# JakobHavtorn/benchmarking-lvms

Hardware: AMD Instinct MI355X
Metric: audio frames/sec training (VRNN, 16 kHz mu-law) (higher is better)
Workload: dtype f32

## Files before the change

benchmarking-lvms_amd/blvm/models/vrnn.py:

```python
import math
from types import SimpleNamespace
from typing import Optional, Union

import torch
import torch.nn as nn
import torch.nn.init as init

from blvm import _hip, ops
from blvm.data.transforms import StackTensor
from blvm.evaluation import BitsPerDimMetric, DeferredScalars, KLMetric, LatestMeanMetric, LLMetric, LossMetric
from blvm.models.base_model import BaseModel
from blvm.modules.convenience import View
from blvm.modules.distributions import (DiagonalGaussianDense, DiagonalGaussianMixtureDense,
                                        DiscretizedLogisticMixtureDense, mlp_log_prob)

LIKELIHOOD_HEADS = (DiscretizedLogisticMixtureDense, DiagonalGaussianMixtureDense, DiagonalGaussianDense)


class LazyNamespace(SimpleNamespace):

    def __init__(self, _lazy=None, **kwargs):
        super().__init__(**kwargs)
        object.__setattr__(self, "_lazy", dict(_lazy or {}))

# ... 121 lines not shown
            and self.condition_x_on_h
            and all(isinstance(m, (nn.Linear, nn.LeakyReLU, View, StackTensor)) for m in list(enc) + list(dec))
            and isinstance(dec[-2], nn.LeakyReLU)
        )
        if not ok:
            raise NotImplementedError(
                "libblvm_hip accelerates the VRNNAudio(likelihood='DMoL') structure (stacked-frame MLP encoder, MLP "
                "decoder, DMoL head, condition_h_on_x = condition_x_on_h = True); other compositions are not built yet"
            )
        return stack.n_frames, _linears(enc), _linears(dec), lik

    def forward(self, x: torch.Tensor, x_sl: torch.Tensor, beta: float = 1, free_nats: float = 0,
                h0: Optional[torch.Tensor] = None, eps: Optional[torch.Tensor] = None):
        S, enc_lin, dec_lin, lik = self._plan()
        if x.ndim == 3:
            x = x.squeeze(-1)
        dev = x.device
        B, T = x.shape
        x_sl_host = x_sl.detach().cpu().to(torch.int64)
        x_sl_dev = ops.upload_i32(x_sl_host, dev)
        y = x.detach().to(torch.float32).contiguous()
        Tp = (T + S - 1) // S
        stride = math.ceil(T / Tp)
        H, Z, R = self.h_dim, self.z_dim, self.r_dim

        xs = torch.nn.functional.pad(y, (0, Tp * S - T)) if Tp * S != T else y
        xs = xs.view(B, Tp, S).transpose(0, 1).contiguous().view(Tp * B, S)
        enc = ops.mlp(xs, enc_lin, ops.ACT_LEAKY, ops.LEAKY_SLOPE).view(Tp, B, -1)

        if eps is None:
            eps = torch.randn(Tp, B, Z, device=dev, dtype=torch.float32)
        widths = [(lin.in_features, lin.out_features) for lin in dec_lin]
        chained = len(dec_lin) == 3 and widths[0] == (H + R, widths[1][0]) and widths[1][1] == widths[1][0] == widths[2][0]
        fold = ops.DecoderFold(dec_lin, ops.LEAKY_SLOPE) if chained and all(lin.bias is not None for lin in dec_lin) else None
        decin, kld, kld_fn, mu_q, sd_q, mu_p, sd_p, z = self.vrnn_cell.sequence(enc, h0, eps, x_sl_dev, stride, free_nats, decoder=fold)
        given = fold.given if fold is not None else None

        dec, log_prob = mlp_log_prob(lik, decin[:Tp].view(Tp * B, H + R), dec_lin, ops.ACT_LEAKY, ops.LEAKY_SLOPE, y, x_sl_dev,
                                     ops.LAYOUT_TIME_MAJOR, B, T, Tp, S, given=given)

        n_frames = float(x_sl_host.sum())
        loss, elbo, sums4 = ops.elbo_assemble(log_prob, kld, kld_fn, beta, n_frames)
        kl = kld_fn

        sums = DeferredScalars(sums4)
        ln2 = math.log(2)
        metrics = [
            LossMetric(sums[0], weight_by=B),
            LLMetric(sums[1], name="elbo", reduce_by=B),
            LLMetric(sums[2], name="rec", reduce_by=B),
            KLMetric(sums[3], reduce_by=B),
            KLMetric(sums[3] / ln2, name="kl (bpt)", reduce_by=n_frames),
            BitsPerDimMetric(sums[1], reduce_by=n_frames),
            LatestMeanMetric(beta, name="beta"),
            LatestMeanMetric(free_nats, name="free_nats"),
        ]

        max_len = int(x_sl_host.max())
        F = lik.out_features

        def parameters():
            d = dec.detach().view(Tp, B, S, F).permute(1, 0, 2, 3).reshape(B, Tp * S, F)[:, :max_len]
            return lik(d.contiguous())

        lazy = dict(
            reconstructions_parameters=parameters,
            reconstructions=lambda ns: lik.sample(ns.reconstructions_parameters),
            reconstructions_mode=lambda ns: lik.mode(ns.reconstructions_parameters),
            seq_mask=lambda: (torch.arange(max_len, device=dev).unsqueeze(0) < x_sl_dev.unsqueeze(1)).to(torch.float64),
        )
        outputs = LazyNamespace(
            lazy,
# ... 141 lines not shown
```

benchmarking-lvms_amd/blvm/modules/distributions.py:

```python
import math

import torch
import torch.nn as nn

from .. import ops
from .convenience import AddConstant


class ConditionalDistribution(nn.Module):
    def reset_parameters(self):
        pass


class DiagonalGaussianDense(ConditionalDistribution):
    def __init__(self, x_dim, y_dim, initial_sd: float = 1, epsilon: float = 1e-6):
        super().__init__()
        self.x_dim, self.y_dim, self.initial_sd, self.epsilon = x_dim, y_dim, initial_sd, epsilon
        self.out_features = 2 * y_dim
        self.params = nn.Linear(x_dim, 2 * y_dim)
        beta = math.log(2) / (initial_sd - epsilon)
        self.sd_activation = nn.Sequential(nn.Softplus(beta=beta), AddConstant(epsilon)) if epsilon > 0 else nn.Softplus(beta=beta)
        self.reset_parameters()

    @property
# ... 11 lines not shown
        lead = x.shape[:-1]
        p = ops.mlp(x.reshape(-1, x.shape[-1]), [self.params], act=ops.ACT_NONE)
        mu, raw = p.view(*lead, -1).chunk(2, dim=-1)
        return mu, self.sd_activation(raw)

    def fused_log_prob(self, dec, y, x_sl_dev, layout, B, T, Tp, S, fused_linear: bool = True):
        if self.y_dim != 1:
            raise NotImplementedError("Gaussian likelihood head: y_dim must be 1 on the audio path")
        W, b = (self.params.weight, self.params.bias) if fused_linear else (None, None)
        return ops.gauss_log_prob(dec, W, b, y, x_sl_dev, layout, B, T, Tp, S, self.softplus_beta, self.epsilon)


class DiscretizedLogisticMixtureDense(ConditionalDistribution):
    def __init__(self, x_dim: int, y_dim: int, num_mix: int = 10, num_bins: int = 256, log_epsilon: float = -7.0):
        super().__init__()
        self.x_dim, self.y_dim, self.num_mix, self.num_bins, self.log_epsilon = x_dim, y_dim, num_mix, num_bins, log_epsilon
        self.out_features = num_mix * (2 * y_dim + 1)
        self.params = nn.Linear(x_dim, self.out_features)
        self.reset_parameters()

    def forward(self, x):
        if self.y_dim != 1:
            raise NotImplementedError("DMoL head: y_dim must be 1 on the audio path")
        lead = x.shape[:-1]
        p = ops.mlp(x.reshape(-1, x.shape[-1]), [self.params], act=ops.ACT_NONE).view(*lead, -1)
        logits = p[..., : self.num_mix]
        locs, log_scales = p[..., self.num_mix :].reshape(*lead, 1, 2 * self.num_mix).chunk(2, dim=-1)
        return logits, locs, log_scales.clamp(min=self.log_epsilon)

    def fused_log_prob(self, dec, y, x_sl_dev, layout, B, T, Tp, S, fused_linear: bool = True):
        W, b = (self.params.weight, self.params.bias) if fused_linear else (None, None)
        return ops.dmol_log_prob(dec, W, b, y, x_sl_dev, layout, B, T, Tp, S, self.num_mix, self.num_bins, self.log_epsilon)

    def fused_mlp_log_prob(self, x2d, layers, act, slope, y, x_sl_dev, layout, B, T, Tp, S, given=None):
        return ops.mlp_dmol_log_prob(x2d, layers, self.params.weight, self.params.bias, y, x_sl_dev, layout, B, T, Tp, S, act, slope,
                                     self.num_mix, self.num_bins, self.log_epsilon, given)

    @staticmethod
    def _pack(params):
        return torch.cat([params[0], params[1].squeeze(-2), params[2].squeeze(-2)], -1).contiguous()

    @torch.no_grad()
    def mode(self, params):
        return ops.mix_sample(self._pack(params), None, None, 0, self.log_epsilon).unsqueeze(-1)

    @torch.no_grad()
    def sample(self, params, eps: float = 1e-5, uniforms=None):
        logits = params[0]
        u = torch.empty_like(logits).uniform_(eps, 1.0 - eps) if uniforms is None else uniforms[0].to(logits)
        u2 = torch.empty(*logits.shape[:-1], device=logits.device).uniform_(1e-8, 1.0 - 1e-8) if uniforms is None else uniforms[1].to(logits)
        return ops.mix_sample(self._pack(params), u, u2, 0, self.log_epsilon).unsqueeze(-1)


class DiagonalGaussianMixtureDense(ConditionalDistribution):

    def __init__(self, x_dim, y_dim, num_mix: int, initial_sd: float = 1, epsilon: float = 1e-6):
        super().__init__()
        self.x_dim, self.y_dim, self.num_mix, self.initial_sd, self.epsilon = x_dim, y_dim, num_mix, initial_sd, epsilon
        self.out_features = num_mix * (2 * y_dim + 1)
        self.params = nn.Linear(x_dim, self.out_features)
        beta = self.softplus_beta
        self.sd_activation = nn.Sequential(nn.Softplus(beta=beta), AddConstant(epsilon)) if epsilon > 0 else nn.Softplus(beta=beta)
        self.reset_parameters()

    @property
    def softplus_beta(self) -> float:
        return math.log(2) / self.initial_sd if self.epsilon > 0 else math.log(2) / (self.initial_sd - self.epsilon)

    def forward(self, x):
# ... 27 lines not shown
    def __init__(self, x_dim, y_dim):
        super().__init__()
        ops.categorical_check_widths(x_dim, y_dim)
        self.x_dim, self.y_dim = x_dim, y_dim
        self.out_features = y_dim
        self.logits = nn.Linear(x_dim, y_dim)
        self.register_buffer("levels", torch.linspace(-1.0, 1.0, y_dim), persistent=False)
        self.reset_parameters()

    def forward(self, x):
        lead = x.shape[:-1]
        return ops.mlp(x.reshape(-1, x.shape[-1]), [self.logits], act=ops.ACT_NONE).view(*lead, -1)

    def fused_log_prob(self, dec, y, x_sl_dev, B, T, Tp, S):
        return ops.categorical_log_prob(dec, self.logits.weight, self.logits.bias, y, x_sl_dev, B, T, Tp, S)

    def log_prob(self, y, logits, reduce_dim=None):
        ll = (logits - logits.logsumexp(dim=-1, keepdim=True)).gather(-1, y.long().unsqueeze(-1)).squeeze(-1)
        return ll if reduce_dim is None else ll.sum(reduce_dim)

    @torch.no_grad()
    def mode(self, logits):
        return ops.categorical_sample(logits)

    @torch.no_grad()
    def sample(self, logits, uniforms=None):
        u = torch.rand(logits.shape[:-1], device=logits.device) if uniforms is None else uniforms
        return ops.categorical_sample(logits, u)

    def dequantize(self, k):
        return self.levels.to(k.device)[k.long()]


def mlp_log_prob(lik, x2d, layers, act, slope, y, x_sl_dev, layout, B, T, Tp, S, given=None):
    if isinstance(lik, DiscretizedLogisticMixtureDense):
        return lik.fused_mlp_log_prob(x2d, layers, act, slope, y, x_sl_dev, layout, B, T, Tp, S, given)
    dec = ops.mlp(x2d, layers, act, slope) if given is None else ops.mlp_given(x2d, layers, given, act, slope)
    return dec.detach(), lik.fused_log_prob(dec, y, x_sl_dev, layout, B, T, Tp, S)
```

benchmarking-lvms_amd/blvm/ops.py:

```python
import ctypes
from typing import List, Optional, Sequence

import torch

from . import _hip
from ._hip import VrnnWeights, check, load, ptr, stream_ptr

ACT_NONE, ACT_RELU, ACT_LEAKY = 0, 1, 2
LEAKY_SLOPE = 0.01

LAYOUT_BATCH_MAJOR, LAYOUT_TIME_MAJOR = 0, 1

seq_timer_hook = None


def _tick(tag):
    if seq_timer_hook is not None:
        seq_timer_hook(tag)


def _c_ints(v):
    return (ctypes.c_int * len(v))(*[int(i) for i in v])


# ... 265 lines not shown
            dW = torch.empty_like(W) if need_w else None
            db = torch.empty_like(b) if need_b else None
            ws = _dmol_workspace(dec.device, ws_floats) if (need_w or need_b) else None
            rc = lib.blvm_dmol_bwd_fused(ptr(dec), layout, ptr(W), ptr(b), ptr(y), ptr(x_sl_dev), ptr(g32), B, T, Tp, S, num_mix,
                                         num_bins, log_eps, act_slope, ptr(dz), ptr(dW), ptr(db), ptr(ws), stream_ptr())
            if rc == 0:
                return (dz if ctx.needs_input_grad[0] else None, dW, db) + (None,) * 11
            if rc != BLVM_NOT_APPLICABLE:
                check(rc, "blvm_dmol_bwd_fused")
        d_dec = torch.empty_like(dec)
        d_par = torch.empty_like(dec) if ctx.has_linear else None
        check(
            load().blvm_dmol_bwd(ptr(dec), layout, ptr(W), ptr(b), ptr(y), ptr(x_sl_dev), ptr(g32), B, T, Tp, S, num_mix,
                                 num_bins, log_eps, ptr(d_dec), ptr(d_par), stream_ptr()),
            "blvm_dmol_bwd",
        )
        n_frames = dec.numel() // F
        dW, db = _head_linear_grads(d_par, dec, W, b, F, n_frames, need_w, need_b)
        if act_slope >= 0.0 and ctx.needs_input_grad[0]:
            dz = torch.empty_like(d_dec)
            check(lib.blvm_act_bwd_f32(ptr(d_dec), ptr(dec), act_slope, ptr(dz), dz.numel(), stream_ptr()), "blvm_act_bwd_f32")
            d_dec = dz
        return (d_dec if ctx.needs_input_grad[0] else None, dW, db) + (None,) * 11


def mlp_given(x2d, layers, given, act: int = ACT_LEAKY, slope: float = LEAKY_SLOPE, head_gates: bool = False):
    params = []
    for lin in layers:
        params += [lin.weight, lin.bias]
    return _MLPGivenFunction.apply(x2d, act, slope, head_gates, tuple(given), *params)


def mlp_dmol_log_prob(x2d, layers, W, b, y, x_sl_dev, layout, B, T, Tp, S, act: int = ACT_LEAKY, slope: float = LEAKY_SLOPE,
                      num_mix=10, num_bins=256, log_eps=-7.0, given=None):
    if act == ACT_NONE or W is None:
        dec = mlp(x2d, layers, act, slope) if given is None else mlp_given(x2d, layers, given, act, slope)
        return dec.detach(), dmol_log_prob(dec, W, b, y, x_sl_dev, layout, B, T, Tp, S, num_mix, num_bins, log_eps)
    params = []
    for lin in layers:
        params += [lin.weight, lin.bias]
    dec = _MLPFunction.apply(x2d, act, slope, True, *params) if given is None else mlp_given(x2d, layers, given, act, slope, True)
    gate = slope if act == ACT_LEAKY else 0.0
    return dec.detach(), _DMoLFunction.apply(dec, W, b, y, x_sl_dev, layout, B, T, Tp, S, num_mix, num_bins, log_eps, gate)


def dmol_log_prob(dec, W, b, y, x_sl_dev, layout, B, T, Tp, S, num_mix=10, num_bins=256, log_eps=-7.0):
    return _DMoLFunction.apply(dec, W, b, y, x_sl_dev, layout, B, T, Tp, S, num_mix, num_bins, log_eps, -1.0)


class _GaussHeadFunction(torch.autograd.Function):

    @staticmethod
    def forward(ctx, dec, W, b, y, x_sl_dev, kind, layout, B, T, Tp, S, num_mix, sd_beta, sd_eps):
        dec, y = _f32c(dec), _f32c(y)
        W, b = (_f32c(W), _f32c(b)) if W is not None else (None, None)
        F = 3 * num_mix if kind == 1 else 2
        if dec.dim() != 2 or dec.shape[0] != B * Tp or dec.shape[1] != S * F:
            raise _hip.BlvmHipError(f"Gaussian head: activations must be [B*T'={B * Tp}, S*F={S * F}], got {tuple(dec.shape)}")
        if W is not None and tuple(W.shape) != (F, F):
            raise _hip.BlvmHipError(f"Gaussian head: fused head weight must be [{F},{F}], got {tuple(W.shape)}")
        if tuple(y.shape) != (B, T) or Tp * S < T:
            raise _hip.BlvmHipError(f"Gaussian head: targets must be [B={B}, T={T}] with T <= T'*S={Tp * S}, got {tuple(y.shape)}")
        log_prob = torch.zeros(B, device=dec.device, dtype=torch.float64)
        lib = load()
        if kind == 1:
            rc = lib.blvm_gmm_fwd(ptr(dec), layout, ptr(W), ptr(b), ptr(y), ptr(x_sl_dev), B, T, Tp, S, num_mix, sd_beta, sd_eps,
                                  ptr(log_prob), None, stream_ptr())
# ... 325 lines not shown
    keep = _decode_weight_ptrs(w, "enc", enc_lin, dec_lin, lik_lin)
    w.cell = ctypes.pointer(cw)
    x0, eps = _f32c(x0), _f32c(eps)
    h0 = _f32c(h0) if h0 is not None else None
    u = _f32c(u) if u is not None else None
    v = _f32c(v) if v is not None else None
    if whole_chip is None:
        whole_chip = B <= lib.blvm_pchain_max_batch()
    x = torch.empty(B, T, S, device=dev, dtype=torch.float32)
    hn = torch.empty(B, R, device=dev, dtype=torch.float32)
    if whole_chip:

        def call(t0, t1, state, xc, scratch):
            xs, hs = (x0, h0) if state is None else state
            uc, vc = (None, None) if u is None else (u[t0:t1], v[t0:t1])
            check(lib.blvm_vrnn_generate(ctypes.byref(w), ptr(xs), ptr(hs), ptr(eps[t0:t1]), ptr(uc), ptr(vc), t1 - t0, B, S, H, Z, R, num_mix,
                                         sd_eps, slope, log_eps, ptr(xc), ptr(hn), ptr(scratch), stream_ptr()), "blvm_vrnn_generate")

        _rollout(lambda n: lib.blvm_vrnn_generate_scratch_floats(n, B, S, H, Z, R), T, max_scratch_floats, "vrnn_decode", x, call,
                 lambda xc, t1: (xc[:, -1].contiguous(), hn.clone()))
        return x, hn
    scratch = torch.empty(lib.blvm_vrnn_decode_scratch_floats(S, H, Z, R), device=dev, dtype=torch.float32)
    check(lib.blvm_vrnn_decode(ctypes.byref(w), ptr(x0), ptr(h0), ptr(eps), ptr(u), ptr(v), T, B, S, H, Z, R, num_mix, sd_eps, slope,
                               log_eps, ptr(x), ptr(hn), ptr(scratch), stream_ptr()), "blvm_vrnn_decode")
    return x, hn


class _VRNNSeqFunction(torch.autograd.Function):

    @staticmethod
    def forward(ctx, enc, h0, eps, x_sl_dev, cfg, dec, *params):
        Tp, B, X, H, Z, R, residual, sd_eps, stride, fn_floor = cfg
        enc, eps = _f32c(enc), _f32c(eps)
        params = tuple(_f32c(p) for p in params)
        dev = enc.device
        lib = load()
        f32 = dict(device=dev, dtype=torch.float32)
        decin = torch.empty(Tp + 1, B, H + R, **f32)
        mu_q, sd_q, mu_p, sd_p, z = (torch.empty(Tp, B, Z, **f32) for _ in range(5))
        w = _pack_weights(params)
        if dec is None:
            reserve = torch.empty(lib.blvm_vrnn_reserve_floats(Tp, B, X, H, Z, R), **f32)
            _tick("fwd_begin")
            check(
                lib.blvm_vrnn_seq_fwd(w, ptr(enc), ptr(_f32c(h0)) if h0 is not None else None, ptr(eps), Tp, B, X, H, Z, R,
                                      int(residual), sd_eps, ptr(decin), ptr(mu_q), ptr(sd_q), ptr(mu_p), ptr(sd_p), ptr(z),
                                      ptr(reserve), stream_ptr()),
                "blvm_vrnn_seq_fwd",
            )
        else:
            keep = [_f32c(t.detach()) for lin in dec.layers for t in (lin.weight, lin.bias)]
            DH, SF = keep[0].shape[0], keep[4].shape[0]
            ys = [torch.empty(Tp * B, n, **f32) for n in (DH, DH, SF)]
            three = ctypes.c_void_p * 3
            dw, db, dy = three(*(ptr(t) for t in keep[0::2])), three(*(ptr(t) for t in keep[1::2])), three(*(ptr(t) for t in ys))
            reserve = torch.empty(lib.blvm_vrnn_fwd_reserve_floats(Tp, B, X, H, Z, R, DH, SF), **f32)
            folded = ctypes.c_int(0)
            _tick("fwd_begin")
            check(
                lib.blvm_vrnn_seq_fwd_dec(w, ptr(enc), ptr(_f32c(h0)) if h0 is not None else None, ptr(eps), Tp, B, X, H, Z, R,
                                          int(residual), sd_eps, ptr(decin), ptr(mu_q), ptr(sd_q), ptr(mu_p), ptr(sd_p), ptr(z),
                                          ptr(reserve), dw, db, dy, DH, SF, dec.slope, ctypes.byref(folded), stream_ptr()),
                "blvm_vrnn_seq_fwd_dec",
            )
            dec.given = tuple(ys[: folded.value]) if folded.value else None
        _tick("fwd_end")
        kld = torch.zeros(B, device=dev, dtype=torch.float64)
        kld_fn = torch.zeros(B, device=dev, dtype=torch.float64)
        check(
            lib.blvm_kl_fwd(ptr(mu_q), ptr(sd_q), ptr(mu_p), ptr(sd_p), LAYOUT_TIME_MAJOR, ptr(x_sl_dev), B, Tp, Z, stride,
                            fn_floor, ptr(kld), ptr(kld_fn), stream_ptr()),
            "blvm_kl_fwd",
        )
        ctx.cfg = cfg
        ctx.has_h0 = h0 is not None
        ctx.save_for_backward(enc, eps, x_sl_dev, decin, mu_q, sd_q, mu_p, sd_p, z, reserve, *params)
        ctx.mark_non_differentiable(mu_q, sd_q, mu_p, sd_p, z)
        ctx.set_materialize_grads(False)
        return decin, kld, kld_fn, mu_q, sd_q, mu_p, sd_p, z

    @staticmethod
    def backward(ctx, d_decin, g_kld, g_kld_fn, *_unused):
        Tp, B, X, H, Z, R, residual, sd_eps, stride, fn_floor = ctx.cfg
        enc, eps, x_sl_dev, decin, mu_q, sd_q, mu_p, sd_p, z, reserve, *params = ctx.saved_tensors
        dev = enc.device
        lib = load()
        f32 = dict(device=dev, dtype=torch.float32)
        d_decin = _f32c(d_decin) if d_decin is not None else torch.zeros_like(decin)
        c_raw = _grad_f32(g_kld) if g_kld is not None else None
        c_fn = _grad_f32(g_kld_fn) if g_kld_fn is not None else None
        grads = _zeros_like_many(params)
        d_enc = torch.empty_like(enc)
        d_h0 = torch.empty(B, R, **f32) if ctx.has_h0 else None
        ws = torch.empty(lib.blvm_vrnn_bwd_workspace_floats(Tp, B, X, H, Z, R), **f32)
        w, g = _pack_weights(params), _pack_weights(grads, _hip.VrnnGrads)
        _tick("bwd_begin")
        check(
            lib.blvm_vrnn_seq_bwd(w, ptr(enc), ptr(eps), ptr(decin), ptr(mu_q), ptr(sd_q), ptr(mu_p), ptr(sd_p), ptr(z),
                                  ptr(reserve), ptr(d_decin), ptr(x_sl_dev), ptr(c_raw), ptr(c_fn), stride, fn_floor, Tp, B,
                                  X, H, Z, R, int(residual), sd_eps, ptr(d_enc), ptr(d_h0), g, ptr(ws), stream_ptr()),
            "blvm_vrnn_seq_bwd",
        )
        _tick("bwd_end")
        return (d_enc, d_h0, None, None, None, None, *grads)


def vrnn_sequence(enc, h0, eps, x_sl_dev, params: Sequence[torch.Tensor], X, H, Z, R, residual_posterior, stride,
                  free_nats=0.0, sd_eps=1e-6, decoder=None):
    Tp, B, _ = enc.shape
    fn_floor = float(free_nats) / Z if free_nats else 0.0
    cfg = (Tp, B, X, H, Z, R, int(residual_posterior), float(sd_eps), int(stride), fn_floor)
    if decoder is None:
        return _VRNNSeqFunction.apply(enc, h0, eps, x_sl_dev, cfg, None, *params)
    decoder.given = None
    return _VRNNSeqFunction.apply(enc, h0, eps, x_sl_dev, cfg, decoder, *params)


class DecoderFold:

    def __init__(self, layers, slope: float = LEAKY_SLOPE):
        self.layers, self.slope, self.given = list(layers), float(slope), None




class _LSTMSeqFunction(torch.autograd.Function):
    @staticmethod
    def forward(ctx, inp, h0, c0, lens_dev, Wih, Whh, bih, bhh):
        inp, Wih, Whh, bih, bhh = (_f32c(t) for t in (inp, Wih, Whh, bih, bhh))
        T, B, I = inp.shape
        H = Whh.shape[1]
        lib = load()
        f32 = dict(device=inp.device, dtype=torch.float32)
        out = torch.empty(T, B, H, **f32)
        hn, cn = torch.empty(B, H, **f32), torch.empty(B, H, **f32)
        reserve = torch.empty(lib.blvm_lstm_reserve_floats(T, B, H), **f32)
        check(
            lib.blvm_lstm_seq_fwd(ptr(Wih), ptr(Whh), ptr(bih), ptr(bhh), ptr(inp), ptr(_f32c(h0)) if h0 is not None else None,
                                  ptr(_f32c(c0)) if c0 is not None else None, ptr(lens_dev), T, B, I, H, ptr(out), ptr(hn), ptr(cn),
                                  ptr(reserve), stream_ptr()),
            "blvm_lstm_seq_fwd",
        )
        ctx.dims = (T, B, I, H)
        ctx.has_state = (h0 is not None, c0 is not None)
        ctx.save_for_backward(inp, Wih, Whh, reserve)
        ctx.mark_non_differentiable(hn, cn)
        return out, hn, cn

    @staticmethod
    def backward(ctx, d_out, _dhn, _dcn):
        T, B, I, H = ctx.dims
        inp, Wih, Whh, reserve = ctx.saved_tensors
        lib = load()
        f32 = dict(device=inp.device, dtype=torch.float32)
# ... 1273 lines not shown
```

benchmarking-lvms_amd/csrc/pchain.h:

```cpp
#pragma once
#include <algorithm>
#include <cstdlib>
#include <functional>

#include "common.h"
#include "decode_tiles.h"

namespace blvm {
namespace pchain {

constexpr unsigned SENTINEL = 0xFFFFFFFFu;
constexpr unsigned SPIN_LIMIT = 1u << 22;

typedef unsigned u32x4 __attribute__((ext_vector_type(4)));
typedef __amdgpu_buffer_rsrc_t rsrc_t;
constexpr int AUX_SC1 = 16;
#ifndef PCHAIN_POLL_AUX
#define PCHAIN_POLL_AUX AUX_SC1
#endif
#ifndef PCHAIN_STORE_AUX
#define PCHAIN_STORE_AUX AUX_SC1
#endif
__device__ __forceinline__ rsrc_t make_rsrc(const void* base) {
  const unsigned long long u = reinterpret_cast<unsigned long long>(base);
// ... 400 lines not shown
  int ld;
  bool rm_sc1;
  float* x16;
  int n16;
  float* x16b = nullptr;
  int n16b = 0;
};
__device__ __forceinline__ Out out_rm(float* p, int ld, bool sc1 = false) { return Out{p, ld, sc1, nullptr, 0}; }
__device__ __forceinline__ Out out_both(float* p, int ld, float* x16, int n16, bool sc1 = false) { return Out{p, ld, sc1, x16, n16}; }
__device__ __forceinline__ void put_rm(const Out& o, int row, int col, float x) {
  if (o.rm != nullptr) {
    if (o.rm_sc1) st_sc1(make_rsrc(o.rm), 4u * ((unsigned)row * (unsigned)o.ld + (unsigned)col), x);
    else o.rm[(size_t)row * o.ld + col] = x;
  }
}
__device__ __forceinline__ void put_t16(const Out& o, int r0, int c0, int row, int col, float x) {
  const int rr = row - r0, cc = col - c0;
  const unsigned in_block = (unsigned)((rr + 16 * ((cc & 15) >> 2)) * 4 + (cc & 3));
  if (o.x16 != nullptr) st_sc1(make_rsrc(o.x16), 4u * ((((unsigned)(r0 >> 4) * (unsigned)o.n16 + (unsigned)((c0 + cc) >> 4)) << 8) + in_block), x);
  if (o.x16b != nullptr) st_sc1(make_rsrc(o.x16b), 4u * ((((unsigned)(r0 >> 4) * (unsigned)o.n16b + (unsigned)((c0 + cc) >> 4)) << 8) + in_block), x);
}
__device__ __forceinline__ void put(const Out& o, int r0, int c0, int row, int col, float x) {
  put_t16(o, r0, c0, row, col, x);
  put_rm(o, row, col, x);
}


struct LinLate {
  const float *bias, *add, *gate;
  int ldadd, ldgate;
  bool add_polled, relu;
  float slope;
  Out out;
};
template <int NW, int OT, class Late, class WS = WMem, class PC = PaceOff>
__device__ __forceinline__ void tile_lin_late(const float* A, int lda, bool a_polled, const float* W, int K, Late& late, int r0, int c0, int B,
                                              float* red, Poll& pl, const float* A2 = nullptr, const float* A3 = nullptr, int w_width = 0,
                                              const WS& ws = WS(), const PC& pace = PC()) {
  const int t = threadIdx.x & 255;
  const int row = r0 + (t >> 4), col = c0 + (t & 15);
  const bool own = threadIdx.x < 256 && row < B;
  const int rowc = row < B ? row : r0;
#ifdef PCHAIN_TPROF
  const unsigned long long t0 = wall_clock64();
  pl.t_first = 0; pl.polls = 0;
#endif
  float e_bias = 0.f, e_gate = 1.f, e_add = 0.f;
  LinLate L;
  auto prefetch = [&]() {
    L = late();
    if (L.bias) e_bias = L.bias[col];
    if (L.gate) e_gate = L.gate[(size_t)rowc * L.ldgate + col];
    if (L.add && !L.add_polled) e_add = L.add[(size_t)rowc * L.ldadd + col];
  };
  f32x4 acc[1] = {{0.f, 0.f, 0.f, 0.f}};
  if (A2 != nullptr) {
    const float* const As[3] = {A, A2, A3};
    const float* const Ws[1] = {W};
    const int la[3] = {0, 0, 0}, cs[1] = {c0};
    tile_product<NW, OT, 3, 1, MapSum>(ws, As, la, true, r0, B, Ws, cs, K, acc, pl, prefetch, lda, w_width, pace);
  } else {
    const float* const As[1] = {A};
    const float* const Ws[1] = {W};
    const int la[1] = {lda}, cs[1] = {c0};
    tile_product<NW, OT, 1, 1, MapSame>(ws, As, la, a_polled, r0, B, Ws, cs, K, acc, pl, prefetch, a_polled ? lda : 0, w_width, pace);
  }
  float v[1];
  reduce_tiles<1, NW>(acc, red, v);
#ifdef PCHAIN_TPROF
  if (a_polled && pl.nap == 1) {
    const unsigned long long t3 = wall_clock64();
    pl.tp[0] += 1; pl.tp[1] += pl.t_first - t0; pl.tp[2] += pl.t_ok - pl.t_first; pl.tp[3] += t3 - pl.t_ok; pl.tp[4] += pl.polls;
    if (pl.t_end != 0) pl.tp[6] += t0 - pl.t_end;
  }
#endif
  if (threadIdx.x >= 256) return;
  if (L.add && L.add_polled) {
    const rsrc_t rs[1] = {make_rsrc(L.add)};
    const unsigned os[1] = {4u * ((unsigned)rowc * (unsigned)L.ldadd + (unsigned)col)};
    float ws[1];
    poll_words<1>(rs, os, ws, own, pl);
    e_add = ws[0];
  }
  if (!own) return;
  float x = v[0] + e_bias + e_add;
  if (L.relu) x = x > 0.f ? x : x * L.slope;
  if (L.gate) x = e_gate > 0.f ? x : x * L.slope;
  put(L.out, r0, c0, row, col, x);
#ifdef PCHAIN_TPROF
  if (a_polled && pl.nap == 1) { pl.t_end = wall_clock64(); pl.t_st = pl.t_end; }
#endif
}
template <int NW, int OT = OP_F32>
__device__ __forceinline__ void tile_lin(const float* A, int lda, bool a_polled, const float* W, int K, const float* bias,
                                         const float* add, int ldadd, bool add_polled, const float* gate, int ldgate, bool relu,
                                         float slope, const Out& out, int r0, int c0, int B, float* red, Poll& pl) {
  auto late = [&]() { return LinLate{bias, add, gate, ldadd, ldgate, add_polled, relu, slope, out}; };
  tile_lin_late<NW, OT>(A, lda, a_polled, W, K, late, r0, c0, B, red, pl);
}

struct HeadOut {
  float *mu_p, *sd_p, *mu_q, *sd_q, *raw_p, *raw_q, *muq_raw;
  Out z;
};
template <int NW, int OT = OP_F32, class WS = WMem, class PC = PaceOff>
__device__ __forceinline__ void tile_head(const float* P, const float* Q, bool polled, const float* Wp, const float* bp, const float* Wq,
                                          const float* bq, const float* eps, const HeadOut& o, int H, int Z, int residual, float beta,
                                          float inv_beta, float sd_eps, int r0, int c0, int B, float* red, Poll& pl, const WS& ws = WS(),
                                          const PC& pace = PC()) {
  const int t = threadIdx.x & 255;
  const int row = r0 + (t >> 4), col = c0 + (t & 15);
  const bool own = threadIdx.x < 256 && row < B;
  const size_t oc = (size_t)(row < B ? row : r0) * Z + col;
  float b0 = 0.f, b1 = 0.f, b2 = 0.f, b3 = 0.f, e = 0.f;
  auto prefetch = [&]() { b0 = bp[col]; b1 = bp[Z + col]; b2 = bq[col]; b3 = bq[Z + col]; e = eps[oc]; };
  f32x4 acc[4];
#pragma unroll
  for (int g = 0; g < 4; ++g) acc[g] = (f32x4){0.f, 0.f, 0.f, 0.f};
// ... 535 lines not shown
      }
#pragma unroll
      for (int j = 0; j < 4; ++j)
        if (wave * 4 + j < F) outp[lane * 32 + wave * 4 + j] = acc[j];
    }
  }
  __syncthreads();
  if (wave == 0) {
    const int rr = lane >> 2, ss = lane & 3, row = r0 + rr, smp = s0 + ss;
    if (row < B && smp < S) {
      const float* p = outp + lane * 32;
      const size_t f = (size_t)row * S + smp;
      const int best = mix_pick(p, num_mix, u != nullptr ? u + f * num_mix : nullptr);
      float x = p[num_mix + best];
      if (v != nullptr) x = logistic_draw(x, p[2 * num_mix + best], v[f], log_eps);
      put(xo, r0, s0 & ~15, row, smp, x);
    } else if (row < B) {
      put_t16(xo, r0, s0 & ~15, row, smp, 0.f);
    }
  }
  __syncthreads();
}

enum Kind : int { K_LIN = 0, K_HEAD = 1, K_GRU = 2, K_DZ = 3, K_GRUB = 4, K_DMOLS = 5, K_GRUS = 6, K_GRUSB = 7, K_LSTMS = 8, K_LSTMSB = 9, K_LINSEQ = 10, K_LSTM = 11 };
enum DescFlag : int {
  DF_RELU = 1,
  DF_A_PLAIN = 2,
  DF_ADD_POLLED = 4,
  DF_RM_SC1 = 8,
  DF_GENTLE = 16,
  DF_CANARY = 32,
  DF_A_SUM3 = 64,
  DF_SEQ_GATE = 128,
};
enum : int { LD_OUT = 3, N16_OUT = 0, N16_OUTB = 1 };
enum : int { LIN_A, LIN_W, LIN_BIAS, LIN_ADD, LIN_GATE, LIN_ORM, LIN_O16, LIN_O16B, LIN_A2, LIN_A3, LIN_LD_A = 0, LIN_LD_ADD = 1, LIN_LD_GATE = 2,
             LIN_I_W_WIDTH = 0, LIN_F_SLOPE = 0 };
enum : int { LINSEQ_A0 = 0, LINSEQ_W = 1, LINSEQ_AUX = 5, LINSEQ_ORM = 9, LINSEQ_O16 = 13, LINSEQ_ADD0 = 17, LINSEQ_LD_ORM = 0,
             LINSEQ_I_LD_ADD0 = 0, LINSEQ_I_N = 1, LINSEQ_I_LD_GATE = 2, LINSEQ_I_K0 = 3, LINSEQ_F_SLOPE = 0 };
enum : int { HEAD_P16, HEAD_Q16, HEAD_WP, HEAD_BP, HEAD_WQ, HEAD_BQ, HEAD_EPS, HEAD_MU_P, HEAD_SD_P, HEAD_MU_Q, HEAD_SD_Q, HEAD_RAW_P, HEAD_RAW_Q,
             HEAD_MUQ_RAW, HEAD_Z, HEAD_Z16, HEAD_Z16B, HEAD_I_Z = 0, HEAD_I_RESIDUAL = 1, HEAD_F_BETA = 0, HEAD_F_INV_BETA = 1, HEAD_F_SD_EPS = 2 };
enum : int { GRU_X16, GRU_WIH, GRU_XG, GRU_GH, GRU_HPREV, GRU_HRM, GRU_H16, GRU_RG, GRU_UG, GRU_NG, GRU_BIH, GRU_H16B, GRU_LD_HPREV = 0, GRU_I_R = 0 };
enum : int { DZ_D16, DZ_WT, DZ_D2_16, DZ_WT2, DZ_ADD, DZ_MU_Q, DZ_SD_Q, DZ_MU_P, DZ_SD_P, DZ_EPS, DZ_RAW_Q, DZ_RAW_P, DZ_MUQ_RAW, DZ_X_SL, DZ_C_RAW,
             DZ_C_FN, DZ_DQH, DZ_DQH16, DZ_DPH, DZ_DPH16, DZ_LD_ADD = 1, DZ_I_Z = 0, DZ_I_RESIDUAL = 1, DZ_I_STRIDE = 2, DZ_I_T0 = 3,
             DZ_F_FN_FLOOR = 0, DZ_F_BETA = 1, DZ_F_SD_EPS = 2, DZ_F_GEMM_FROM = 3 };
enum : int { GRUB_D0_16, GRUB_D1_16, GRUB_W0, GRUB_W1, GRUB_G_IN, GRUB_RG, GRUB_UG, GRUB_NG, GRUB_GH, GRUB_HPREV, GRUB_DD, GRUB_DGI, GRUB_DGI16,
             GRUB_DGH, GRUB_DGH16, GRUB_GA, GRUB_G_OUT, GRUB_G_ADD, GRUB_LD_H = 0, GRUB_LD_GADD = 1, GRUB_I_R = 0, GRUB_I_GEMM_FROM = 1,
             GRUB_I_GATES_TO = 2, GRUB_I_GIN_FROM = 3 };
enum : int { DMOLS_DEC, DMOLS_W, DMOLS_B, DMOLS_U, DMOLS_V, DMOLS_X, DMOLS_X16, DMOLS_LD_DEC = 0, DMOLS_I_S = 0, DMOLS_I_F = 1, DMOLS_I_NMIX = 2,
             DMOLS_F_LOG_EPS = 0 };
enum : int { GRUS_H16, GRUS_WHH, GRUS_BHH, GRUS_XG, GRUS_LENS, GRUS_HPREV, GRUS_HNEXT, GRUS_HNEXT16, GRUS_OUT, GRUS_RG, GRUS_UG, GRUS_NG, GRUS_GHN,
             GRUS_I_R = 0, GRUS_I_REVERSE = 1, GRUS_I_OUT_TS = 2, GRUS_I_OUT_LD = 3 };
enum : int { GRUSB_DGH16_IN, GRUSB_WHHT, GRUSB_DOUT, GRUSB_RG, GRUSB_UG, GRUSB_NG, GRUSB_GHN, GRUSB_HPREV, GRUSB_LENS, GRUSB_G, GRUSB_DGI, GRUSB_DGH,
             GRUSB_DGH16, GRUSB_DH0, GRUSB_N16_T = 1, GRUSB_I_R = 0, GRUSB_I_REVERSE = 1, GRUSB_I_OUT_TS = 2, GRUSB_I_OUT_LD = 3 };
enum : int { LSTMS_H16, LSTMS_WHH, LSTMS_BHH, LSTMS_XG, LSTMS_LENS, LSTMS_HPREV, LSTMS_HNEXT, LSTMS_HNEXT16, LSTMS_CPREV, LSTMS_CNEXT, LSTMS_OUT,
             LSTMS_GATES, LSTMS_I_H = 0 };
enum : int { LSTMSB_DG16_IN, LSTMSB_WHHT, LSTMSB_DOUT, LSTMSB_GATES, LSTMSB_CS, LSTMSB_DC, LSTMSB_DG, LSTMSB_DG16, LSTMSB_DH0, LSTMSB_N16_T = 1, LSTMSB_I_H = 0 };
enum : int { LSTM_X16, LSTM_WIH, LSTM_BIH, LSTM_GH, LSTM_CPREV, LSTM_CNEXT, LSTM_HRM, LSTM_H16, LSTM_H16B, LSTM_I_H = 0 };
constexpr int kMaxDesc = 24, kMaxPtr = 20;
struct Desc {
  int kind, ct, wg0, nwg, flags, K, s_begin, s_end;
  int ld[4];
  int n16[2];
  int i[4];
  float f[4];
  unsigned char sidx[kMaxPtr];
  const float* p[kMaxPtr];
};
struct Program {
  int ot = OP_F32;
// ... 129 lines not shown
```

benchmarking-lvms_amd/csrc/pchain.hip:

```cpp
#include <algorithm>
#include <mutex>

#include "common.h"
#include "pchain.h"
#include "pchain_rt.h"

namespace blvm {
namespace {
using namespace pchain;

constexpr int kDescWords = 128;
enum { RD_KIND = 0, RD_CT, RD_WG0, RD_NWG, RD_FLAGS, RD_K, RD_SBEGIN, RD_SEND, RD_LD = 8, RD_N16 = 12, RD_I = 14, RD_F = 18, RD_P = 24, RD_ST = 64,
       RD_NT = 84, RD_TILE = 85 };
constexpr int kMaxTilesPerWg = kDescWords - RD_TILE;
struct Hdr {
  int ndesc, s0, S, B, xcd, prof_wg, lds_products;
  Ctl ctl;
  unsigned long long* prof;
};

constexpr int kResolveChunk = 12;
struct ProgramPart {
  int ndesc, first;
  long stride[16];
// ... 115 lines not shown
  for (int s = a.s0; s < a.S; ++s) {
    for (unsigned m = mine; m != 0; m &= m - 1) {
      const int i = __builtin_ctz(m);
#ifdef PCHAIN_TPROF2
      const unsigned long long tq0 = wall_clock64();
      if (tq_end) tq[2] += tq0 - tq_end;
#endif
      const unsigned rest = m & (m - 1);
      const int nx_i = __builtin_ctz(rest != 0 ? rest : mine), nx_s = rest != 0 ? s : s + 1;
      const int kind = d.w<RD_KIND>(), flags = d.w<RD_FLAGS>(), K = d.w<RD_K>();
      const bool active = s >= d.w<RD_SBEGIN>() && s < d.w<RD_SEND>();
#ifdef PCHAIN_TPROF2
      const unsigned long long tqa = wall_clock64();
      tq[3] += tqa - tq0;
#endif
      if (!active || (kind != K_LIN && kind != K_LINSEQ)) nx.fetch(ltab, nx_i, nx_s);
      if (active) {
        const int nt = d.w<RD_NT>();
        pl.nap = (flags & DF_GENTLE) ? 16 : 1;
        pl.code = ((unsigned)s << 4) | (unsigned)i;
        switch (kind) {
          case K_LIN: {
            const bool a_polled = !(flags & DF_A_PLAIN);
            const float *A = d.p<LIN_A>(s), *W = d.base<LIN_W>();
            const float *A2 = (flags & DF_A_SUM3) ? d.p<LIN_A2>(s) : nullptr, *A3 = (flags & DF_A_SUM3) ? d.p<LIN_A3>(s) : nullptr;
            const int ld0 = d.w<RD_LD + LIN_LD_A>(), w_width = d.w<RD_I + LIN_I_W_WIDTH>();
#ifdef PCHAIN_TPROF2
            const unsigned long long tqb = wall_clock64();
            tq[4] += tqb - tqa;
#endif
            auto late = [&]() {
              __builtin_amdgcn_sched_barrier(0);
              nx.fetch(ltab, nx_i, nx_s);
              return LinLate{d.base<LIN_BIAS>(), d.p<LIN_ADD>(s), d.p<LIN_GATE>(s), d.w<RD_LD + LIN_LD_ADD>(), d.w<RD_LD + LIN_LD_GATE>(), (flags & DF_ADD_POLLED) != 0,
                             (flags & DF_RELU) != 0, d.f<LIN_F_SLOPE>(), Out{d.m<LIN_ORM>(s), d.w<RD_LD + LD_OUT>(), (flags & DF_RM_SC1) != 0, d.m<LIN_O16>(s),
                                                                             d.w<RD_N16 + N16_OUT>(), d.m<LIN_O16B>(s), d.w<RD_N16 + N16_OUTB>()}};
            };
            for (int tk = 0; tk < nt; ++tk) {
              const int trc = d.tile(tk), tr0 = trc & 0xffff, tc0 = (trc >> 16) * 16;
              if ((flags & DF_CANARY) && a_polled) canary_wait(A, tr0, K, pl, ld0);
#ifdef PCHAIN_TPROF2
              const unsigned long long tq1 = wall_clock64();
              tq[0] += tq1 - tq0;
#endif
              tile_lin_late<NW, OT>(A, ld0, a_polled, W, K, late, tr0, tc0, B, red(), pl, A2, A3, w_width);
#ifdef PCHAIN_TPROF2
              tq_end = wall_clock64();
              tq[1] += tq_end - tq1;
#endif
            }
            if (nt == 0) nx.fetch(ltab, nx_i, nx_s);
          } break;
          case K_LINSEQ: {
            const int n = d.w<RD_I + LINSEQ_I_N>();
            const bool gated = (flags & DF_SEQ_GATE) != 0;
            const float* A = d.p<LINSEQ_A0>(s);
            const int K0 = d.w<RD_I + LINSEQ_I_K0>();
            for (int lq = 0; lq < n; ++lq) {
              int li = lq;
              asm volatile("" : "+s"(li));
              pl.code = ((unsigned)s << 4) | (unsigned)i | ((unsigned)li << 28);
              const float* W = d.basedyn(LINSEQ_W + li);
              const int Kl = (li == 0 && K0 != 0) ? K0 : K;
              auto late = [&]() {
                __builtin_amdgcn_sched_barrier(0);
                if (li == 0) nx.fetch(ltab, nx_i, nx_s);
                const float* aux = d.pdyn(LINSEQ_AUX + li);
                const float* add0 = li == 0 ? d.p<LINSEQ_ADD0>(s) : nullptr;
                return LinLate{gated ? nullptr : aux, add0, gated ? aux : nullptr, d.w<RD_I + LINSEQ_I_LD_ADD0>(), d.w<RD_I + LINSEQ_I_LD_GATE>(), false,
// ... 381 lines not shown
  Hdr h{prog.ndesc, prog.s_first, prog.S, prog.B, prog.xcd, prog.prof_wg, prog.lds_products, prog.ctl, prog.prof};
  const int nw = prog.rt_group > 1 ? 8 : 16;
  const size_t lds_fixed = sizeof(int) * kDescWords * pchain::kMaxDesc + 32 * sizeof(unsigned long long);
  const size_t lds = lds_fixed + sizeof(float) * 2 * (size_t)prog.lds_products * nw * 256;
  constexpr int kMaxProducts = 8;
  static std::mutex attr_mu;
  static int attr_dev[7] = {-1, -1, -1, -1, -1, -1, -1};
  static int occ_blocks[7][kMaxProducts + 1];
  const size_t lds_max = lds_fixed + sizeof(float) * 2 * (prog.rt_group > 1 ? 8 : 4) * (size_t)nw * 256;
  BLVM_REQUIRE(prog.lds_products >= 1 && lds <= lds_max, "pchain: %d products per tile do not fit the reduction scratch", prog.lds_products);
  auto go = [&](auto kernel, int slot, int threads) -> int {
    {
      std::lock_guard<std::mutex> lock(attr_mu);
      int* const occ = occ_blocks[slot];
      if (attr_dev[slot] != dev) {
        BLVM_HIP(hipFuncSetAttribute(reinterpret_cast<const void*>(kernel), hipFuncAttributeMaxDynamicSharedMemorySize, (int)lds_max));
        attr_dev[slot] = dev;
        std::fill(occ, occ + kMaxProducts + 1, 0);
      }
      if (occ[prog.lds_products] == 0) BLVM_HIP(hipOccupancyMaxActiveBlocksPerMultiprocessor(&occ[prog.lds_products], kernel, threads, lds));
      BLVM_REQUIRE((long)occ[prog.lds_products] * cus >= grid,
                   "pchain: %d workgroups of %d threads + %zu B LDS are not co-resident (%d per CU x %d CUs)", grid, threads, lds, occ[prog.lds_products], cus);
    }
    hipLaunchKernelGGL(kernel, dim3(grid), dim3(threads), lds, stream, (const int*)tab, h);
    return BLVM_OK;
  };
  BLVM_REQUIRE(prog.rt_group == 1 || prog.rt_group == 2, "pchain: row groups of %d row tiles are not built", prog.rt_group);
  if (prog.rt_group > 1) {
    for (int i = 0; i < prog.ndesc; ++i) {
      const int k = prog.d[i].kind;
      BLVM_REQUIRE(k == pchain::K_LIN || k == pchain::K_LINSEQ || k == pchain::K_HEAD || k == pchain::K_GRU || k == pchain::K_DZ || k == pchain::K_GRUB,
                   "pchain: tile kind %d has no row-group form", k);
      BLVM_REQUIRE(k != pchain::K_DZ || prog.d[i].p[2] == nullptr, "pchain: the row-group dz tile is the single-product form");
    }
    BLVM_REQUIRE(prog.ot == OP_F32, "pchain: row groups multiply fp32 operands only");
    BLVM_TRY(go(&pchain_rt_kernel<8, OP_F32, 2>, 2, 512));
    BLVM_CHECK_LAUNCH("pchain_launch (row groups)");
    return BLVM_OK;
  }
  bool roll = false;
  for (int i = 0; i < prog.ndesc; ++i) roll |= prog.d[i].kind == pchain::K_LSTM;
  if (roll) {
    for (int i = 0; i < prog.ndesc; ++i) {
      const int k = prog.d[i].kind;
      BLVM_REQUIRE(k == pchain::K_LIN || k == pchain::K_LINSEQ || k == pchain::K_LSTM || k == pchain::K_DMOLS, "pchain: tile kind %d is not part of the roll-out kernel", k);
    }
    BLVM_TRY(prog.ot == OP_BF16  ? go(&pchain_kernel<16, OP_BF16, true>, 5, 1024)
             : prog.ot == OP_F16 ? go(&pchain_kernel<16, OP_F16, true>, 6, 1024)
                                 : go(&pchain_kernel<16, OP_F32, true>, 4, 1024));
    BLVM_CHECK_LAUNCH("pchain_launch (roll-out)");
    return BLVM_OK;
  }
  BLVM_TRY(prog.ot == OP_BF16  ? go(&pchain_kernel<16, OP_BF16>, 1, 1024)
           : prog.ot == OP_F16 ? go(&pchain_kernel<16, OP_F16>, 3, 1024)
                               : go(&pchain_kernel<16, OP_F32>, 0, 1024));
  BLVM_CHECK_LAUNCH("pchain_launch");
  return BLVM_OK;
}

}

extern "C" int blvm_pchain_chain_probe(const float* W16, const float* bias, float* x16, float* xs, int B, int N, int L, int nwg, void* stream_) {
  using namespace blvm;
  using namespace blvm::pchain;
  hipStream_t s = static_cast<hipStream_t>(stream_);
  BLVM_REQUIRE(W16 && bias && x16 && xs && B > 0 && N > 0 && N % 16 == 0 && L > 0, "pchain_chain_probe: bad arguments");
  const int rt = (B + 15) / 16;
  const long x = (long)rt * 16 * N, sN = (long)B * N;
  Builder bld;
  bld.begin(OP_F32, L, B, 1, false, 1);
  static const int run = [] { const char* e = getenv("BLVM_PCHAIN_PROBE_RUN"); return e ? atoi(e) : 1; }();
  const int nw = nwg > 0 ? nwg : range_for((N / 16) * rt, device_cus() & ~7);
  if (run >= 2 && run <= 4 && L % run == 0) {
    bld.p.S = L / run;
// ... 16 lines not shown
```

benchmarking-lvms_amd/csrc/vrnn.hip:

```cpp
#include <vector>
#include <stdlib.h>

#include <algorithm>

#include "common.h"
#include "pchain.h"
#include "vrnn_static.h"

namespace blvm {
namespace {

#include "stages.h"


template <int NW>
__global__ __launch_bounds__(NW * 64) void gru_stage_kernel(const float* decin_t, const float* Wih, const float* xg,
                                                            const float* gh, int B, int H, int R, float* decin_next,
                                                            float* rg, float* ug, float* ng) {
  __shared__ float red[3 * NW * 256];
  const int r0 = blockIdx.y * 16, c0 = blockIdx.x * 16, wave = threadIdx.x >> 6;
  const int ldd = H + R;
  const int t = threadIdx.x & 255;
  const int row = r0 + (t >> 4), col = c0 + (t & 15);
  const bool own = threadIdx.x < 256 && row < B;
// ... 123 lines not shown
  tmp.XQ = ar.take(n * H);
  tmp.XG = ar.take(n * 3 * R);
  tmp.RAWQ = ar.take(n * Z); tmp.RAWP = ar.take(n * Z);
  tmp.Wp[0] = ar.take((size_t)H * R); tmp.Wq[0] = ar.take((size_t)H * R);
  for (int i = 1; i < 3; ++i) { tmp.Wp[i] = ar.take((size_t)H * H); tmp.Wq[i] = ar.take((size_t)H * H); }
  tmp.Wph = ar.take((size_t)2 * Z * H); tmp.Wqh = ar.take((size_t)2 * Z * H);
  tmp.Wf[0] = ar.take((size_t)H * Z);
  for (int i = 1; i < 4; ++i) tmp.Wf[i] = ar.take((size_t)H * H);
  tmp.Wih = ar.take((size_t)3 * R * H); tmp.Whh = ar.take((size_t)3 * R * R);
  tmp.H16 = nullptr;
  if (B <= kPchainCarveMaxB || B <= vrnn_rt_max_b()) {
    const size_t rows = (size_t)((B + 15) / 16) * 16, m = (size_t)Tp * rows;
    tmp.H16 = ar.take((m + rows) * R);
    for (int i = 0; i < 3; ++i) tmp.P16[i] = ar.take(m * H);
    for (int i = 0; i < 3; ++i) tmp.Q16[i] = ar.take(m * H);
    tmp.Z16 = ar.take(m * Z);
    for (int i = 0; i < 3; ++i) tmp.FZ16[i] = ar.take(m * H);
    tmp.PHI16 = ar.take(m * H);
    tmp.Y116 = tmp.Y216 = tmp.Y1P = nullptr;
    if (SF > 0) { tmp.Y116 = ar.take(m * H); tmp.Y216 = ar.take(m * H); tmp.Y1P = ar.take(n * H); }
    tmp.x16_bytes = ar.bytes_from(tmp.H16);
    if (SF > 0) { tmp.Wd[0] = ar.take((size_t)H * (H + R)); tmp.Wd[1] = ar.take((size_t)H * H); tmp.Wd[2] = ar.take((size_t)SF * H); }
  }
  if (r) *r = tmp;
  return ar.floats();
}

struct BwdWs {
  float *pT[3], *phT, *qT[3], *qhT, *fT[4], *wihT, *whhT;
  float *DGI, *DGH, *DPHI[4], *DQH, *DPH, *DP[3], *DQ[3], *G;
  float *GA, *GB, *DP16[3], *DQ16[3], *DGI16, *DGH16, *DPHI16[4], *DPH16, *DQH16, *DPHI16b, *DPHI16c;
  size_t x16_bytes;
  float *DPHI3b, *DPHI3c;
};

size_t carve_ws(float* base, int Tp, int B, int X, int H, int Z, int R, BwdWs* w) {
  (void)X;
  const size_t n = (size_t)Tp * B;
  Arena ar{base};
  BwdWs t;
  t.pT[0] = ar.take((size_t)R * H); t.pT[1] = ar.take((size_t)H * H); t.pT[2] = ar.take((size_t)H * H);
  t.phT = ar.take((size_t)H * 2 * Z);
  t.qT[0] = ar.take((size_t)R * H); t.qT[1] = ar.take((size_t)H * H); t.qT[2] = ar.take((size_t)H * H);
  t.qhT = ar.take((size_t)H * 2 * Z);
  t.fT[0] = ar.take((size_t)Z * H);
  for (int i = 1; i < 4; ++i) t.fT[i] = ar.take((size_t)H * H);
  t.wihT = ar.take((size_t)H * 3 * R);
  t.whhT = ar.take((size_t)R * 3 * R);
  t.DGI = ar.take(n * 3 * R); t.DGH = ar.take(n * 3 * R);
  for (int i = 0; i < 4; ++i) t.DPHI[i] = ar.take(n * H);
  t.DQH = ar.take(n * 2 * Z); t.DPH = ar.take(n * 2 * Z);
  for (int i = 0; i < 3; ++i) t.DP[i] = ar.take(n * H);
  for (int i = 0; i < 3; ++i) t.DQ[i] = ar.take(n * H);
  t.G = ar.take((size_t)B * R);
  t.GA = nullptr;
  if (B <= kPchainCarveMaxB || B <= vrnn_rt_max_b()) {
    const size_t m = (size_t)Tp * ((B + 15) / 16) * 16;
    t.GA = ar.take(n * R); t.GB = ar.take(n * R);
    for (int i = 0; i < 3; ++i) { t.DP16[i] = ar.take(m * H); t.DQ16[i] = ar.take(m * H); }
    t.DGI16 = ar.take(m * 3 * R); t.DGH16 = ar.take(m * 3 * R);
    for (int i = 0; i < 4; ++i) t.DPHI16[i] = ar.take(m * H);
    t.DPH16 = ar.take(m * 2 * Z); t.DQH16 = ar.take(m * 2 * Z);
    t.DPHI16b = ar.take(m * H); t.DPHI16c = ar.take(m * H);
    t.x16_bytes = ar.bytes_from(t.GA);
    t.DPHI3b = ar.take(n * H); t.DPHI3c = ar.take(n * H);
  }
  if (w) *w = t;
  return ar.floats();
}

__global__ __launch_bounds__(256) void add3_kernel(float4* __restrict__ a, const float4* __restrict__ b, const float4* __restrict__ c, size_t n4) {
  for (size_t i = (size_t)blockIdx.x * 256 + threadIdx.x; i < n4; i += (size_t)gridDim.x * 256) {
    float4 x = a[i];
    const float4 y = b[i], z = c[i];
    x.x += y.x + z.x; x.y += y.y + z.y; x.z += y.z + z.z; x.w += y.w + z.w;
    a[i] = x;
  }
}

inline bool pchain_split3() {
  static int v = [] {
    const char* e = getenv("BLVM_PCHAIN_SPLIT3");
    return e ? atoi(e) : 1;
  }();
  return v != 0;
}

struct VrnnDecoder {
  const float *w[3], *b[3];
  float* y[3];
};
int g_dec_fold = [] { const char* e = getenv("BLVM_VRNN_DEC_FOLD"); const int v = e ? atoi(e) : 1; return v >= 0 && v <= 2 ? v : 1; }();
long g_dec_folded = 0;
int dec_ct(int layers, int SF) { return layers == 3 ? SF / 16 : layers == 2 ? 1 : 0; }
int vrnn_dec_folds(int B, int H, int Z, int R, int DH, int SF) {
  if (!g_dec_fold || !vrnn_persistent(B) || device_cus() < 32 || operand_16bit() || pchain_optype(B) != OP_F32) return 0;
  if (B > 64 || vrnn_row_groups(B) || Z != H || DH != H || SF <= 0 || SF % 16 != 0) return 0;
  const int tl = (B + 15) / 16, layers = g_dec_fold == 2 ? 2 : 3;
  const bool fits = pchain::vrnn_fwd_deal(H / 16, Z / 16, R / 16, tl, device_cus() & ~7, vrnn_shared_deal(false, tl), dec_ct(layers, SF)).dec[0].nwg > 0;
  return fits ? layers : 0;
}

int check_dims(int Tp, int B, int X, int H, int Z, int R) {
  BLVM_REQUIRE(Tp > 0 && B > 0, "vrnn: bad Tp=%d B=%d", Tp, B);
  BLVM_REQUIRE(X > 0 && H > 0 && Z > 0 && R > 0 && X % 16 == 0 && H % 16 == 0 && Z % 16 == 0 && R % 16 == 0,
               "vrnn: X,H,Z,R must be positive multiples of 16 (got %d,%d,%d,%d)", X, H, Z, R);
  BLVM_REQUIRE(B < 65536 && H < 65536 && R < 65536, "vrnn: B, H and R must be below 65536 (packed kernel arguments)");
  return BLVM_OK;
}

}
}

using namespace blvm;

extern "C" size_t blvm_vrnn_reserve_floats(int Tp, int B, int X, int H, int Z, int R) {
  (void)X;
  return carve_reserve(nullptr, Tp, B, H, Z, R, nullptr);
}
extern "C" size_t blvm_vrnn_fwd_reserve_floats(int Tp, int B, int X, int H, int Z, int R, int DH, int SF) {
  (void)X;
  return carve_reserve(nullptr, Tp, B, H, Z, R, nullptr, vrnn_dec_folds(B, H, Z, R, DH, SF) ? SF : 0);
}
extern "C" int blvm_vrnn_dec_fold(int mode) {
  if (mode == -2) return (int)std::min<long>(g_dec_folded, 0x7fffffffL);
  const int was = g_dec_fold;
  if (mode >= 0) g_dec_fold = mode <= 2 ? mode : 1;
  return was;
}

extern "C" size_t blvm_vrnn_bwd_workspace_floats(int Tp, int B, int X, int H, int Z, int R) {
  return carve_ws(nullptr, Tp, B, X, H, Z, R, nullptr);
}

static int vrnn_seq_fwd_impl(const BlvmVrnnWeights* w, const float* enc, const float* h0, const float* eps,
                             int Tp, int B, int X, int H, int Z, int R, int residual_posterior, float sd_eps,
                             float* decin, float* mu_q, float* sd_q, float* mu_p, float* sd_p, float* z,
                             float* reserve, hipStream_t s, const VrnnDecoder* dec = nullptr, int DH = 0, int SF = 0,
                             float dec_slope = 0.f, int* folded = nullptr) {
  BLVM_TRY(check_dims(Tp, B, X, H, Z, R));
  BLVM_REQUIRE(w && enc && eps && decin && mu_q && sd_q && mu_p && sd_p && z && reserve, "vrnn_fwd: null pointer");
  BLVM_REQUIRE(aligned16(enc) && aligned16(decin) && aligned16(reserve) && aligned16(z),
               "vrnn_fwd: buffers must be 16-byte aligned");
  if (folded) *folded = 0;
  const int fold = dec != nullptr ? vrnn_dec_folds(B, H, Z, R, DH, SF) : 0;
  Reserve rs;
  carve_reserve(reserve, Tp, B, H, Z, R, &rs, fold ? SF : 0);
  const size_t n = (size_t)Tp * B;
  const int ldd = H + R;
  const float beta = softplus_beta_of(sd_eps);

  BLVM_TRY(gemm_f32(0, 0, (int)n, H, X, enc, X, w->post_w[0] + R, R + X, rs.XQ, H, w->post_b[0], 0, 0.f, nullptr, 0, 0, 1, s));
  BLVM_TRY(gemm_f32(0, 0, (int)n, 3 * R, X, enc, X, w->gru_wih, X + H, rs.XG, 3 * R, w->gru_bih, 0, 0.f, nullptr, 0, 0, 1, s));

  T16PackScope pack_scope(pchain_optype(B), s);
  BLVM_TRY(t16_pack_rows(w->prior_w[0], R, H, R, rs.Wp[0], s));
  BLVM_TRY(t16_pack_rows(w->post_w[0], R + X, H, R, rs.Wq[0], s));
  for (int l = 1; l < 3; ++l) {
    BLVM_TRY(t16_pack_rows(w->prior_w[l], H, H, H, rs.Wp[l], s));
    BLVM_TRY(t16_pack_rows(w->post_w[l], H, H, H, rs.Wq[l], s));
  }
  BLVM_TRY(t16_pack_rows(w->prior_hw, H, 2 * Z, H, rs.Wph, s));
  BLVM_TRY(t16_pack_rows(w->post_hw, H, 2 * Z, H, rs.Wqh, s));
  BLVM_TRY(t16_pack_rows(w->phi_w[0], Z, H, Z, rs.Wf[0], s));
  for (int l = 1; l < 4; ++l) BLVM_TRY(t16_pack_rows(w->phi_w[l], H, H, H, rs.Wf[l], s));
// ... 155 lines not shown
  BLVM_CHECK_LAUNCH("vrnn_seq_fwd");
  return BLVM_OK;
}

extern "C" int blvm_vrnn_seq_fwd(const BlvmVrnnWeights* w, const float* enc, const float* h0, const float* eps,
                                 int Tp, int B, int X, int H, int Z, int R, int residual_posterior, float sd_eps,
                                 float* decin, float* mu_q, float* sd_q, float* mu_p, float* sd_p, float* z,
                                 float* reserve, void* stream_) {
  return vrnn_seq_fwd_impl(w, enc, h0, eps, Tp, B, X, H, Z, R, residual_posterior, sd_eps, decin, mu_q, sd_q, mu_p, sd_p, z, reserve,
                           static_cast<hipStream_t>(stream_));
}

extern "C" int blvm_vrnn_seq_fwd_dec(const BlvmVrnnWeights* w, const float* enc, const float* h0, const float* eps,
                                     int Tp, int B, int X, int H, int Z, int R, int residual_posterior, float sd_eps,
                                     float* decin, float* mu_q, float* sd_q, float* mu_p, float* sd_p, float* z,
                                     float* reserve, const float* const* dec_w, const float* const* dec_b, float* const* dec_y,
                                     int DH, int SF, float slope, int* folded, void* stream_) {
  BLVM_REQUIRE(dec_w && dec_b && dec_y && folded, "vrnn_seq_fwd_dec: null pointer");
  VrnnDecoder d;
  for (int l = 0; l < 3; ++l) {
    d.w[l] = dec_w[l]; d.b[l] = dec_b[l]; d.y[l] = dec_y[l];
    BLVM_REQUIRE(d.w[l] && d.b[l] && d.y[l] && aligned16(d.y[l]), "vrnn_seq_fwd_dec: decoder layer %d: null or unaligned pointer", l);
  }
  BLVM_REQUIRE(DH > 0 && SF > 0, "vrnn_seq_fwd_dec: bad decoder widths %d, %d", DH, SF);
  return vrnn_seq_fwd_impl(w, enc, h0, eps, Tp, B, X, H, Z, R, residual_posterior, sd_eps, decin, mu_q, sd_q, mu_p, sd_p, z, reserve,
                           static_cast<hipStream_t>(stream_), &d, DH, SF, slope, folded);
}

static int vrnn_seq_bwd_impl(const BlvmVrnnWeights* w, const float* enc, const float* eps, const float* decin,
                             const float* mu_q, const float* sd_q, const float* mu_p, const float* sd_p,
                             const float* z, const float* reserve, const float* d_decin, const int32_t* x_sl,
                             const float* c_raw, const float* c_fn, int stride, float fn_floor, int Tp, int B, int X, int H, int Z,
                             int R, int residual_posterior, float sd_eps, float* d_enc, float* d_h0,
                             const BlvmVrnnGrads* gr, float* workspace, hipStream_t s) {
  BLVM_TRY(check_dims(Tp, B, X, H, Z, R));
  BLVM_REQUIRE(w && enc && eps && decin && mu_q && sd_q && mu_p && sd_p && z && reserve && d_decin && workspace && gr,
               "vrnn_bwd: null pointer");
  BLVM_REQUIRE((c_fn == nullptr && c_raw == nullptr) || x_sl != nullptr, "vrnn_bwd: KL coefficients need x_sl");
  BLVM_REQUIRE(aligned16(workspace) && aligned16(reserve) && aligned16(d_decin), "vrnn_bwd: buffers must be 16-byte aligned");
  Reserve rs;
  carve_reserve(const_cast<float*>(reserve), Tp, B, H, Z, R, &rs);
  BwdWs ws;
  carve_ws(workspace, Tp, B, X, H, Z, R, &ws);
  const size_t n = (size_t)Tp * B;
  const int ldd = H + R;
  const float beta = softplus_beta_of(sd_eps);

  T16PackScope pack_scope(pchain_optype(B), s);
  BLVM_TRY(t16_pack_transposed(w->prior_w[0], R, H, R, ws.pT[0], s));
  BLVM_TRY(t16_pack_transposed(w->prior_w[1], H, H, H, ws.pT[1], s));
  BLVM_TRY(t16_pack_transposed(w->prior_w[2], H, H, H, ws.pT[2], s));
  BLVM_TRY(t16_pack_transposed(w->prior_hw, H, 2 * Z, H, ws.phT, s));
  BLVM_TRY(t16_pack_transposed(w->post_w[0], R + X, H, R, ws.qT[0], s));
  BLVM_TRY(t16_pack_transposed(w->post_w[1], H, H, H, ws.qT[1], s));
  BLVM_TRY(t16_pack_transposed(w->post_w[2], H, H, H, ws.qT[2], s));
  BLVM_TRY(t16_pack_transposed(w->post_hw, H, 2 * Z, H, ws.qhT, s));
  BLVM_TRY(t16_pack_transposed(w->phi_w[0], Z, H, Z, ws.fT[0], s));
  for (int i = 1; i < 4; ++i) BLVM_TRY(t16_pack_transposed(w->phi_w[i], H, H, H, ws.fT[i], s));
  BLVM_TRY(t16_pack_transposed(w->gru_wih + X, X + H, 3 * R, H, ws.wihT, s));
  BLVM_TRY(t16_pack_transposed(w->gru_whh, R, 3 * R, R, ws.whhT, s));
  BLVM_TRY(pack_scope.flush());

  BLVM_HIP(hipMemsetAsync(ws.G, 0, sizeof(float) * (size_t)B * R, s));
  const int rt = (B + 15) / 16;

  auto launch_dh = [&](int t_gemm, int s_gates) {
    DhArgs d;
    d.has_gemm = t_gemm >= 0; d.has_gates = s_gates >= 0;
    d.DP0 = d.has_gemm ? ws.DP[0] + (size_t)t_gemm * B * H : nullptr;
    d.DQ0 = d.has_gemm ? ws.DQ[0] + (size_t)t_gemm * B * H : nullptr;
    d.WpT = ws.pT[0]; d.WqT = ws.qT[0]; d.G = ws.G;
    const size_t sg = d.has_gates ? (size_t)s_gates : 0;
    d.rg = rs.RG + sg * B * R; d.ug = rs.UG + sg * B * R; d.ng = rs.NG + sg * B * R;
    d.gh = rs.GHb + sg * B * 3 * R;
    d.decin_s = decin + sg * B * ldd; d.ddecin_s = d_decin + sg * B * ldd;
    d.dgi = ws.DGI + sg * B * 3 * R; d.dgh = ws.DGH + sg * B * 3 * R;
    d.B = B; d.H = H; d.R = R;
    {
      const int nw = pick_nw(H, 2);
      const dim3 grid(R / 16, rt);
      const unsigned b_h = (unsigned)B | ((unsigned)H << 16), has = (d.has_gemm ? 1u : 0u) | (d.has_gates ? 2u : 0u);
      LAUNCH_NW(dh_stage_kernel<NW_>, nw, grid, s, d.DP0, d.DQ0, d.WpT, d.WqT, d.G, b_h, R, has, d);
    }
  };

  const float* hprev_all = decin + H;
  auto batched = [&]() -> int {
    if (d_enc) {
      BLVM_TRY(gemm_f32(0, 1, (int)n, X, H, ws.DQ[0], H, w->post_w[0] + R, R + X, d_enc, X, nullptr, 0, 0.f, nullptr, 0, 0, 1, s));
      BLVM_TRY(gemm_f32(0, 1, (int)n, X, 3 * R, ws.DGI, 3 * R, w->gru_wih, X + H, d_enc, X, nullptr, 0, 0.f, nullptr, 0, 1, 1, s));
    }
    {
      WgradGroup grp;
      auto job = [&](const float* D, int ldd_, int n_out, const float* Act, int lda, int k_in, float* dW, int ldw, float* db = nullptr) {
        grp.add(D, ldd_, n_out, Act, lda, k_in, dW, ldw, db);
      };
      job(ws.DGI, 3 * R, 3 * R, enc, X, X, gr->gru_wih, X + H, gr->gru_bih);
      job(ws.DGI, 3 * R, 3 * R, decin, ldd, H, gr->gru_wih ? gr->gru_wih + X : nullptr, X + H);
      job(ws.DGH, 3 * R, 3 * R, hprev_all, ldd, R, gr->gru_whh, R, gr->gru_bhh);
      job(ws.DPHI[0], H, H, z, Z, Z, gr->phi_w[0], Z, gr->phi_b[0]);
      for (int l = 1; l < 4; ++l) job(ws.DPHI[l], H, H, rs.FZ[l - 1], H, H, gr->phi_w[l], H, gr->phi_b[l]);
      job(ws.DPH, 2 * Z, 2 * Z, rs.P[2], H, H, gr->prior_hw, H, gr->prior_hb);
      job(ws.DQH, 2 * Z, 2 * Z, rs.Q[2], H, H, gr->post_hw, H, gr->post_hb);
      for (int l = 2; l >= 1; --l) {
        job(ws.DP[l], H, H, rs.P[l - 1], H, H, gr->prior_w[l], H, gr->prior_b[l]);
        job(ws.DQ[l], H, H, rs.Q[l - 1], H, H, gr->post_w[l], H, gr->post_b[l]);
      }
      job(ws.DP[0], H, H, hprev_all, ldd, R, gr->prior_w[0], R, gr->prior_b[0]);
      job(ws.DQ[0], H, H, hprev_all, ldd, R, gr->post_w[0], R + X);
      job(ws.DQ[0], H, H, enc, X, X, gr->post_w[0] ? gr->post_w[0] + R : nullptr, R + X, gr->post_b[0]);
      BLVM_TRY(grp.run(n, s));
    }
    return BLVM_OK;
  };
  if (vrnn_persistent(B) && device_cus() >= 32) {
    using namespace pchain;
    const int ctH = H / 16, ctZ = Z / 16, ctR = R / 16, cus = device_cus() & ~7, T = Tp;
    const long sH = (long)B * H, sZ = (long)B * Z, sR = (long)B * R, s3R = 3 * sR, s2Z = 2 * sZ, sD = (long)B * ldd;
    const long xH = (long)rt * 16 * H, x2Z = (long)rt * 16 * 2 * Z, x3R = (long)rt * 16 * 3 * R;
    const bool groups = vrnn_row_groups(B);
    const int RTG = groups ? vrnn_rt(B) : 1;
    const int tl = (rt + RTG - 1) / RTG;
    const bool shared = vrnn_shared_deal(groups, tl);
    const VrnnBwdDeal dl = vrnn_bwd_deal(ctH, ctZ, ctR, tl, cus, shared, pchain_split3());
    Builder bld;
    bld.begin(pchain_optype(B), T + 1, B, groups ? 8 : 2, true, dl.g);
    bld.p.rt_group = RTG;
    auto last = [&](const float* base, long step) { return rev(base, step, T - 1); };
    {
      Operands o;
      o.p[GRUB_D0_16] = rev(ws.DP16[0], xH, T); o.p[GRUB_D1_16] = rev(ws.DQ16[0], xH, T); o.p[GRUB_W0] = ws.pT[0]; o.p[GRUB_W1] = ws.qT[0];
      o.p[GRUB_G_IN] = rev(ws.GB, sR, T); o.p[GRUB_RG] = last(rs.RG, sR); o.p[GRUB_UG] = last(rs.UG, sR); o.p[GRUB_NG] = last(rs.NG, sR);
      o.p[GRUB_GH] = last(rs.GHb, s3R); o.p[GRUB_HPREV] = last(decin + H, sD); o.p[GRUB_DD] = last(d_decin + H, sD); o.p[GRUB_DGI] = last(ws.DGI, s3R);
      o.p[GRUB_DGI16] = last(ws.DGI16, x3R); o.p[GRUB_DGH] = last(ws.DGH, s3R); o.p[GRUB_DGH16] = last(ws.DGH16, x3R); o.p[GRUB_GA] = last(ws.GA, sR);
      o.p[GRUB_G_OUT] = d_h0 ? d_h0 : ws.G; o.ld[GRUB_LD_H] = ldd; o.ld[LD_OUT] = 3 * R; o.n16[N16_OUT] = 3 * ctR; o.i[GRUB_I_R] = R; o.i[GRUB_I_GEMM_FROM] = 1;
      o.i[GRUB_I_GATES_TO] = T; o.i[GRUB_I_GIN_FROM] = 1;
      add_desc(bld, K_GRUB, ctR, dl.grub.wg0, dl.grub.nwg, H, 0, 0, T + 1, o);
    }
    const bool split3 = dl.split3;
    Operands o;
    o.p[LIN_GATE] = last(decin, sD); o.ld[LIN_LD_ADD] = ldd; o.ld[LIN_LD_GATE] = ldd; o.ld[LD_OUT] = H; o.n16[N16_OUT] = ctH;
    if (split3) {
      const size_t wthird = (size_t)ctR * 256 / (bld.p.ot != OP_F32 ? 2 : 1);
      float* const orm[3] = {ws.DPHI[3], ws.DPHI3b, ws.DPHI3c};
      float* const o16[3] = {ws.DPHI16[3], ws.DPHI16b, ws.DPHI16c};
      o.ld[LIN_LD_A] = 3 * R; o.i[LIN_I_W_WIDTH] = 3 * R;
      for (int part = 0; part < 3; ++part) {
        o.p[LIN_A] = last(ws.DGI16 + (size_t)part * ctR * 256, x3R); o.p[LIN_W] = ws.wihT + part * wthird; o.p[LIN_ADD] = part == 0 ? last(d_decin, sD) : Ptr();
        o.p[LIN_ORM] = last(orm[part], sH); o.p[LIN_O16] = last(o16[part], xH);
        add_desc(bld, K_LIN, ctH, dl.part[part].wg0, dl.part[part].nwg, R, 0, 0, T, o);
      }
    } else {
      o.p[LIN_A] = last(ws.DGI16, x3R); o.p[LIN_W] = ws.wihT; o.p[LIN_ADD] = last(d_decin, sD); o.p[LIN_ORM] = last(ws.DPHI[3], sH);
      o.p[LIN_O16] = last(ws.DPHI16[3], xH);
      add_desc(bld, K_LIN, ctH, dl.dphi.wg0, dl.dphi.nwg, 3 * R, 0, 0, T, o);
    }
    Operands gb;
    gb.p[LIN_A] = last(ws.DGH16, x3R); gb.p[LIN_W] = ws.whhT; gb.p[LIN_ADD] = last(ws.GA, sR); gb.ld[LIN_LD_ADD] = R; gb.p[LIN_ORM] = last(ws.GB, sR); gb.ld[LD_OUT] = R;
    add_desc(bld, K_LIN, ctR, dl.gb.wg0, dl.gb.nwg, 3 * R, DF_ADD_POLLED | DF_RM_SC1 | DF_GENTLE | ((pchain_tune() & 16) ? DF_CANARY : 0), 0, T, gb);
    auto blink = [&](const float* W, const float* gate, float* orm, float* o16) { return rev_link(W, gate, orm, o16, T - 1, sH, H, xH); };
    const SeqLink lf[3] = {blink(ws.fT[3], rs.FZ[2], ws.DPHI[2], ws.DPHI16[2]), blink(ws.fT[2], rs.FZ[1], ws.DPHI[1], ws.DPHI16[1]),
                           blink(ws.fT[1], rs.FZ[0], ws.DPHI[0], ws.DPHI16[0])};
    if (split3) {
      Operands o3;
      o3.p[LIN_A] = last(ws.DPHI16[3], xH); o3.p[LIN_W] = ws.fT[3]; o3.p[LIN_GATE] = last(rs.FZ[2], sH); o3.ld[LIN_LD_GATE] = H; o3.p[LIN_ORM] = last(ws.DPHI[2], sH);
      o3.ld[LD_OUT] = H; o3.p[LIN_O16] = last(ws.DPHI16[2], xH); o3.n16[N16_OUT] = ctH; o3.p[LIN_A2] = last(ws.DPHI16b, xH); o3.p[LIN_A3] = last(ws.DPHI16c, xH);
      add_desc(bld, K_LIN, ctH, dl.wide_h.wg0, dl.wide_h.nwg, H, DF_A_SUM3, 0, T, o3);
    }
    add_linseq(bld, ctH, dl.wide_h.wg0, dl.wide_h.nwg, H, false, true, 0, T, last(ws.DPHI16[split3 ? 2 : 3], xH), split3 ? 2 : 3, lf + (split3 ? 1 : 0), -sH,
               -xH, ctH, 0.f, H);
    {
      Operands z;
      z.p[DZ_D16] = last(ws.DPHI16[0], xH); z.p[DZ_WT] = ws.fT[0]; z.p[DZ_MU_Q] = last(mu_q, sZ); z.p[DZ_SD_Q] = last(sd_q, sZ); z.p[DZ_MU_P] = last(mu_p, sZ);
      z.p[DZ_SD_P] = last(sd_p, sZ); z.p[DZ_EPS] = last(eps, sZ); z.p[DZ_RAW_Q] = last(rs.RAWQ, sZ); z.p[DZ_RAW_P] = last(rs.RAWP, sZ); z.p[DZ_X_SL] = x_sl;
      z.p[DZ_C_RAW] = c_raw; z.p[DZ_C_FN] = c_fn; z.p[DZ_DQH] = last(ws.DQH, s2Z); z.p[DZ_DQH16] = last(ws.DQH16, x2Z); z.p[DZ_DPH] = last(ws.DPH, s2Z);
      z.p[DZ_DPH16] = last(ws.DPH16, x2Z); z.ld[LD_OUT] = 2 * Z; z.n16[N16_OUT] = 2 * ctZ; z.i[DZ_I_Z] = Z; z.i[DZ_I_RESIDUAL] = residual_posterior;
      z.i[DZ_I_STRIDE] = stride; z.i[DZ_I_T0] = T - 1; z.f[DZ_F_FN_FLOOR] = fn_floor; z.f[DZ_F_BETA] = beta; z.f[DZ_F_SD_EPS] = sd_eps;
      add_desc(bld, K_DZ, ctZ, dl.dz.wg0, dl.dz.nwg, H, 0, 0, T, z);
    }
    {
      const SeqLink lp[3] = {blink(ws.phT, rs.P[2], ws.DP[2], ws.DP16[2]), blink(ws.pT[2], rs.P[1], ws.DP[1], ws.DP16[1]), blink(ws.pT[1], rs.P[0], ws.DP[0], ws.DP16[0])};
      const SeqLink lq[3] = {blink(ws.qhT, rs.Q[2], ws.DQ[2], ws.DQ16[2]), blink(ws.qT[2], rs.Q[1], ws.DQ[1], ws.DQ16[1]), blink(ws.qT[1], rs.Q[0], ws.DQ[0], ws.DQ16[0])};
      add_linseq(bld, ctH, dl.prior.wg0, dl.prior.nwg, H, false, true, 0, T, last(ws.DPH16, x2Z), 3, lp, -sH, -xH, ctH, 0.f, H, 2 * Z);
      add_linseq(bld, ctH, dl.post.wg0, dl.post.nwg, H, false, true, 0, T, last(ws.DQH16, x2Z), 3, lq, -sH, -xH, ctH, 0.f, H, 2 * Z);
    }
    ArmPlan plan;
    plan.fill(ws.GA, ws.x16_bytes);
    if (!groups) {
      plan.add(arm_rm(ws.GA, R, B, T, true)); plan.add(arm_rm(ws.GB, R, B, T, true));
      for (int i = 0; i < 3; ++i) { plan.add(arm_t16(ws.DP16[i], H, rt, T, true)); plan.add(arm_t16(ws.DQ16[i], H, rt, T, true)); }
      plan.add(arm_t16(ws.DGI16, 3 * R, rt, T, true)); plan.add(arm_t16(ws.DGH16, 3 * R, rt, T, true));
      for (int i = 0; i < 4; ++i) plan.add(arm_t16(ws.DPHI16[i], H, rt, T, true));
      plan.add(arm_t16(ws.DPH16, 2 * Z, rt, T, true)); plan.add(arm_t16(ws.DQH16, 2 * Z, rt, T, true));
      plan.add(arm_t16(ws.DPHI16b, H, rt, T, true)); plan.add(arm_t16(ws.DPHI16c, H, rt, T, true));
    }
    BLVM_TRY(vrnn_launch(bld, false, "vrnn_bwd", s, plan, []() -> int { return BLVM_OK; }));
    if (split3) {
      const size_t n4 = n * H / 4;
      hipLaunchKernelGGL(add3_kernel, dim3((unsigned)std::min<size_t>((n4 + 255) / 256, 2048)), dim3(256), 0, s, reinterpret_cast<float4*>(ws.DPHI[3]),
                         reinterpret_cast<const float4*>(ws.DPHI3b), reinterpret_cast<const float4*>(ws.DPHI3c), n4);
    }
    return batched();
  }

  launch_dh(-1, Tp - 1);
  for (int t = Tp - 1; t >= 0; --t) {
    const size_t oH = (size_t)t * B * H, oZ = (size_t)t * B * Z, o3R = (size_t)t * B * 3 * R, o2Z = (size_t)t * B * 2 * Z;
    const float* dec_t = decin + (size_t)t * B * ldd;
    const float* ddec_t = d_decin + (size_t)t * B * ldd;
    LinLaunch a;
    a.B = B;
    a.nseg = 2;
    a.seg[0] = seg(ws.DGI + o3R, 3 * R, ws.wihT, 3 * R, nullptr, ddec_t, ldd, dec_t, ldd, ws.DPHI[3] + oH, H, H, 3 * R, 0);
    a.seg[1] = seg(ws.DGH + o3R, 3 * R, ws.whhT, 3 * R, nullptr, ws.G, R, nullptr, 0, ws.G, R, R, 3 * R, 0);
    launch_lin(a, s);
    a.nseg = 1;
    for (int l = 3; l >= 1; --l) {
      a.seg[0] = seg(ws.DPHI[l] + oH, H, ws.fT[l], H, nullptr, nullptr, 0, rs.FZ[l - 1] + oH, H, ws.DPHI[l - 1] + oH, H, H, H, 0);
      launch_lin(a, s);
    }
    DzArgs d;
    d.D = ws.DPHI[0] + oH; d.WT = ws.fT[0]; d.D2 = nullptr; d.WT2 = nullptr; d.dz_add = nullptr; d.ld_add = 0; d.has_gemm = 1;
    d.mu_q = mu_q + oZ; d.sd_q = sd_q + oZ; d.mu_p = mu_p + oZ; d.sd_p = sd_p + oZ; d.eps = eps + oZ;
    d.raw_q = rs.RAWQ + oZ; d.raw_p = rs.RAWP + oZ;
    d.x_sl = x_sl; d.c_raw = c_raw; d.c_fn = c_fn;
    d.dqh = ws.DQH + o2Z; d.dph = ws.DPH + o2Z;
    d.B = B; d.H = H; d.Z = Z; d.residual = residual_posterior; d.t = t; d.stride = stride;
    d.fn_floor = fn_floor; d.beta = beta; d.sd_eps = sd_eps; d.muq_raw = nullptr;
    launch_dz(d, pick_nw(H, 1), dim3(Z / 16, rt), s);
    a.nseg = 2;
    a.seg[0] = seg(ws.DPH + o2Z, 2 * Z, ws.phT, 2 * Z, nullptr, nullptr, 0, rs.P[2] + oH, H, ws.DP[2] + oH, H, H, 2 * Z, 0);
    a.seg[1] = seg(ws.DQH + o2Z, 2 * Z, ws.qhT, 2 * Z, nullptr, nullptr, 0, rs.Q[2] + oH, H, ws.DQ[2] + oH, H, H, 2 * Z, 0);
    launch_lin(a, s);
    for (int l = 2; l >= 1; --l) {
      a.seg[0] = seg(ws.DP[l] + oH, H, ws.pT[l], H, nullptr, nullptr, 0, rs.P[l - 1] + oH, H, ws.DP[l - 1] + oH, H, H, H, 0);
      a.seg[1] = seg(ws.DQ[l] + oH, H, ws.qT[l], H, nullptr, nullptr, 0, rs.Q[l - 1] + oH, H, ws.DQ[l - 1] + oH, H, H, H, 0);
      launch_lin(a, s);
    }
    launch_dh(t, t - 1);
  }
  BLVM_CHECK_LAUNCH("vrnn_seq_bwd");
  if (d_h0) BLVM_HIP(hipMemcpyAsync(d_h0, ws.G, sizeof(float) * (size_t)B * R, hipMemcpyDeviceToDevice, s));

  return batched();
}

extern "C" int blvm_vrnn_seq_bwd(const BlvmVrnnWeights* w, const float* enc, const float* eps, const float* decin,
                                 const float* mu_q, const float* sd_q, const float* mu_p, const float* sd_p,
                                 const float* z, const float* reserve, const float* d_decin, const int32_t* x_sl,
                                 const float* c_raw, const float* c_fn, int stride, float fn_floor, int Tp, int B, int X, int H, int Z,
                                 int R, int residual_posterior, float sd_eps, float* d_enc, float* d_h0,
                                 const BlvmVrnnGrads* gr, float* workspace, void* stream_) {
  return vrnn_seq_bwd_impl(w, enc, eps, decin, mu_q, sd_q, mu_p, sd_p, z, reserve, d_decin, x_sl, c_raw, c_fn, stride, fn_floor, Tp, B, X,
                           H, Z, R, residual_posterior, sd_eps, d_enc, d_h0, gr, workspace, static_cast<hipStream_t>(stream_));
}
```

benchmarking-lvms_amd/csrc/vrnn_static.h:

```cpp
#pragma once
#include <algorithm>
#include <initializer_list>

#include "pchain.h"

namespace blvm {
namespace pchain {

struct LinkRange {
  int ct, wg0, nwg;
};
constexpr int kMaxTiles = 8;
struct VrnnFwdDeal {
  int def_n, half, g, spare;
  LinkRange hproj, prior, post, head, phi, gru, dec[4];
};
inline VrnnFwdDeal vrnn_fwd_deal(int ctH, int ctZ, int ctR, int tl, int cus, bool shared, int ctD = 0) {
  VrnnFwdDeal d;
  d.def_n = shared ? 0 : range_for(3 * ctR * tl, std::min(cus / 4, 64));
  d.half = range_for(ctH * tl, (cus - d.def_n) / 2);
  d.g = 2 * d.half;
  const int wide = shared ? d.half : d.g;
  d.hproj = shared ? LinkRange{3 * ctR, d.half, d.half} : LinkRange{3 * ctR, d.g, d.def_n};
  d.prior = LinkRange{ctH, 0, d.half};
  d.post = LinkRange{ctH, d.half, d.half};
  d.head = LinkRange{ctZ, 0, range_for(ctZ * tl, wide)};
  d.phi = LinkRange{ctH, 0, range_for(ctH * tl, wide)};
  d.gru = LinkRange{ctR, 0, range_for(ctR * tl, d.g)};
  d.spare = shared ? 0 : cus - d.g - d.def_n;
  for (LinkRange& r : d.dec) r = LinkRange{0, 0, 0};
  if (ctD > 0 && d.spare >= 8) {
    const int w0 = d.g + d.def_n, n12 = range_for(ctH * tl, d.spare), n3 = range_for(ctD * tl, d.spare);
    bool fits = true;
    for (bool xcd : {false, true})
      fits = fits && tiles_per_workgroup(tl, ctH, n12, xcd) <= 1 && tiles_per_workgroup(tl, ctD, n3, xcd) <= kMaxTiles;
    if (fits) {
      d.dec[0] = d.dec[1] = d.dec[2] = LinkRange{ctH, w0, n12};
      d.dec[3] = LinkRange{ctD, w0, n3};
    }
  }
  return d;
}
struct VrnnBwdDeal {
  int def_n, half, g, spare;
  bool split3;
  LinkRange grub, part[3], dphi, gb, wide_h, dz, prior, post;
};
inline VrnnBwdDeal vrnn_bwd_deal(int ctH, int ctZ, int ctR, int tl, int cus, bool shared, bool allow_split3) {
  VrnnBwdDeal d;
  d.def_n = shared ? 0 : range_for(ctR * tl, std::min(cus / 4, 64));
  d.half = range_for(ctH * tl, (cus - d.def_n) / 2);
  d.g = 2 * d.half;
  const int wide = shared ? d.half : d.g;
  d.spare = cus - d.g - d.def_n;
  d.split3 = !shared && d.spare >= 8 && d.half >= 8 && allow_split3;
  d.grub = LinkRange{ctR, 0, range_for(ctR * tl, d.g)};
  d.part[0] = LinkRange{ctH, 0, range_for(ctH * tl, d.half)};
  d.part[1] = LinkRange{ctH, d.half, range_for(ctH * tl, d.half)};
  d.part[2] = LinkRange{ctH, d.g + d.def_n, d.split3 ? range_for(ctH * tl, d.spare) : 0};
  d.dphi = LinkRange{ctH, 0, range_for(ctH * tl, wide)};
  d.gb = shared ? LinkRange{ctR, d.half, d.half} : LinkRange{ctR, d.g, d.def_n};
  d.wide_h = LinkRange{ctH, 0, range_for(ctH * tl, wide)};
  d.dz = LinkRange{ctZ, 0, range_for(ctZ * tl, wide)};
  d.prior = LinkRange{ctH, 0, d.half};
  d.post = LinkRange{ctH, d.half, d.half};
  return d;
}

constexpr std::initializer_list<int> kFwdResident = {1, 2, 3, 4, 5};
constexpr std::initializer_list<int> kBwdResident = {0, 1, 2, 3, 5, 6, 7, 8, 9};
constexpr int kFwdDesc = 6, kFwdDecDesc = 10;
constexpr std::initializer_list<int> kFwdDecResident = {6, 7, 8};
inline bool one_tile_each(const Program& p, std::initializer_list<int> links, bool xcd) {
  for (int i : links)
    if (tiles_per_workgroup((p.B + 15) / 16, p.d[i].ct, p.d[i].nwg, xcd) > 1) return false;
  return true;
}
inline bool one_tile_each(const Program& p, std::initializer_list<int> links) { return one_tile_each(p, links, p.xcd != 0); }

enum Place {
  kPlaceProgram = 0,
  kPlacePlain = 1,
  kPlaceLocal = 2,
};
constexpr int kPlaceSpan = 128;
__host__ __device__ __forceinline__ int place_wg(int p) { return p < kPlaceSpan ? 64 * ((p & 7) >> 2) + 4 * (p >> 3) + (p & 3) : p; }
inline bool place_local_applies(const Program& p, int prior, int post, int grid) {
  if ((p.B + 15) / 16 != 4 || grid < kPlaceSpan) return false;
  if (p.d[prior].wg0 != 0 || p.d[prior].nwg != 64 || p.d[post].wg0 != 64 || p.d[post].nwg != 64) return false;
  for (int i = 0; i < p.ndesc; ++i) {
    const int lo = p.d[i].wg0, hi = lo + p.d[i].nwg;
    const bool kept = (lo == 0 && (hi == 64 || hi == kPlaceSpan)) || (lo == 64 && hi == kPlaceSpan) || lo >= kPlaceSpan;
    if (!kept) return false;
  }
  return true;
}
inline int place_for(int want, int fallback, const Program& p, int prior, int post, int grid) {
  if (want == kPlaceLocal) return place_local_applies(p, prior, post, grid) ? kPlaceLocal : (fallback == kPlacePlain ? kPlacePlain : kPlaceProgram);
  return want == kPlacePlain ? kPlacePlain : kPlaceProgram;
}
inline bool place_xcd(int place, const Program& p) { return place == kPlaceProgram && p.xcd != 0; }
inline int grid_of(const Program& p) {
  int g = 0;
  for (int i = 0; i < p.ndesc; ++i) g = std::max(g, p.d[i].wg0 + p.d[i].nwg);
  return g;
// ... 39 lines not shown
  for (int c = cand0; c < cand0 + ncand; ++c) {
    TileIter it(c, d.wg0, d.nwg, rt, d.ct, xcd);
    if (!it.valid() || it.r0() != mine.r0()) continue;
    ++*n;
    if (c < w) ++*k;
  }
  return true;
}
inline int arm_operand_slot(int kind) {
  switch (kind) {
    case K_LIN: return LIN_A;
    case K_LINSEQ: return LINSEQ_A0;
    case K_HEAD: return HEAD_P16;
    case K_GRU: return GRU_X16;
    case K_GRUB: return GRUB_D0_16;
    case K_DZ: return DZ_D16;
    default: return -1;
  }
}
inline bool arm_applies(const Program& p, const ArmTable& t, int link, std::initializer_list<int> idle, int cand0, int ncand, bool xcd) {
  const int rt = (p.B + 15) / 16;
  if (t.n <= 0 || t.n > kArmMax || ncand <= 0 || ncand > kArmCandidates || p.S <= kArmAhead || p.rt_group != 1) return false;
  for (int i = 0; i < t.n; ++i) {
    const ArmEntry& e = t.e[i];
    const long span = e.step < 0 ? -(long)e.step : e.step;
    if (e.base == nullptr || (reinterpret_cast<unsigned long long>(e.base) & 15) != 0 || e.step % 4 != 0 || e.tile % 4 != 0) return false;
    if (e.n4 <= 0 || e.n4_last <= 0 || e.n4_last > e.n4 || 4L * e.n4 > e.tile || (long)(rt - 1) * e.tile + 4L * e.n4_last > span) return false;
    if (e.nslabs < p.S - 1 || e.nslabs > p.S + 1) return false;
  }
  for (int i = 0; i < p.ndesc; ++i) {
    const Desc& d = p.d[i];
    const int slot = arm_operand_slot(d.kind);
    if (slot < 0 || d.p[slot] == nullptr || p.stride[d.sidx[slot]] == 0) return false;
    bool inside = false;
    for (int k = 0; k < t.n && !inside; ++k) {
      const ArmEntry& e = t.e[k];
      const long span = e.step < 0 ? -(long)e.step : e.step;
      const float* lo = e.step < 0 ? e.base - (long)(e.nslabs - 1) * span : e.base;
      inside = d.p[slot] >= lo && d.p[slot] <= lo + (long)e.nslabs * span;
    }
    if (!inside) return false;
  }
  const Desc& d = p.d[link];
  int armers[4] = {0, 0, 0, 0};
  if (rt > 4) return false;
  for (int w = cand0; w < cand0 + ncand; ++w) {
    int tiles = 0, r = 0;
    for (TileIter it(w, d.wg0, d.nwg, rt, d.ct, xcd); it.valid(); it.next()) { ++tiles; r = it.r0() / 16; }
    if (tiles > 1) return false;
    if (tiles == 1) ++armers[r];
    for (int i : idle)
      if (TileIter(w, p.d[i].wg0, p.d[i].nwg, rt, p.d[i].ct, xcd).valid()) return false;
  }
  for (int r = 0; r < rt; ++r)
    if (armers[r] == 0 || (armers[r] & (armers[r] - 1)) != 0) return false;
  return true;
}

}
}
```

benchmarking-lvms_amd/csrc/vrnn_static.hip:

```cpp
#include <algorithm>
#include <mutex>

#include "common.h"
#include "pchain.h"
#include "vrnn_static.h"

namespace blvm {
namespace {
using namespace pchain;

struct SPtr {
  float* base;
  int stride;
  __device__ __forceinline__ float* at(int s) const { return base + (long)s * stride; }
};

__device__ __forceinline__ int placed_wg(int place) { return place == kPlaceLocal ? place_wg((int)blockIdx.x) : (int)blockIdx.x; }
__device__ __forceinline__ int tile_lanes(int w, int wg0, int nwg, int rt, int ct, bool xcd) {
  TileIter it(w, wg0, nwg, rt, ct, xcd);
  const int lane = threadIdx.x & 63;
  it.j += lane * it.step;
  return (lane < kMaxTiles && it.valid()) ? (it.r0() | (it.c() << 16)) : -1;
}
__device__ __forceinline__ int tile_count(int lanes) { return __popcll(__ballot(lanes >= 0)); }

constexpr int kAnatBase = 128, kAnatRole = 512, kAnatSlots = 48;
#ifdef PCHAIN_TPROF
__device__ __forceinline__ void anat_begin(unsigned* tab) {
  for (int i = threadIdx.x; i < kAnatSlots * 8; i += blockDim.x) tab[i] = 0u;
  __syncthreads();
}
__device__ __forceinline__ void anat_arm(Poll& pl) { pl.rpolls = 0; pl.t_st = 0; }
__device__ __forceinline__ void anat_note(unsigned* tab, int slot, const Poll& pl) {
  const unsigned long long now = wall_clock64();
  if ((threadIdx.x & 63) == 0 && pl.rpolls != 0) {
    unsigned* q = tab + (slot * 2 + (threadIdx.x < 256 ? 0 : 1)) * 4;
    atomicAdd(q, 1u); atomicAdd(q + 1, pl.rpolls); atomicAdd(q + 2, (unsigned)(pl.t_ok - pl.t_issue));
    atomicAdd(q + 3, (unsigned)((pl.t_st != 0 ? pl.t_st : now) - pl.t_ok));
  }
}
__device__ __forceinline__ void anat_end(const unsigned* tab, unsigned long long* prof, int role, bool chosen) {
  __syncthreads();
  if (prof != nullptr && chosen)
    for (int i = threadIdx.x; i < kAnatSlots * 8; i += blockDim.x) prof[kAnatBase + role * kAnatRole + i] = tab[i];
}
#define ANAT(x) x
#else
#define ANAT(x)
#endif

struct LinChainArgs {
  SPtr a16, orm, o16;
  const float *W, *bias;
  int ldo, n16, B, s0, S, wg0, nwg, ct, xcd, place;
  Ctl ctl;
  int pace_early, pace_epi;
  ANAT(unsigned long long* prof;)
};
template <class PC>
// ... 121 lines not shown
template <int NW>
__device__ __forceinline__ void load_head(Res<kH, 4>& r, const HeadArgs& q, int tiles, int nt) {
  if (nt == 0) return;
  const int c0 = tile_c0(tiles);
  const float* const Ws[4] = {q.Wp, q.Wp, q.Wq, q.Wq};
  const int cs[4] = {c0, q.Z + c0, c0, q.Z + c0};
  load_w<NW, OP_F32, 4, 1>(r.w, Ws, cs, kH);
}
template <int NW>
__device__ __forceinline__ void load_gru(Res<kH, 3>& r, const GruArgs& q, int tiles, int nt) {
  if (nt == 0) return;
  const int c0 = tile_c0(tiles);
  const float* const Ws[3] = {q.Wih, q.Wih, q.Wih};
  const int cs[3] = {c0, q.R + c0, 2 * q.R + c0};
  load_w<NW, OP_F32, 3, 1>(r.w, Ws, cs, kH);
}
template <int NW>
__device__ __forceinline__ void load_grub(Res<kH, 2>& r, const GrubArgs& q, int tiles, int nt) {
  if (nt == 0) return;
  const int c0 = tile_c0(tiles);
  const float* const Ws[2] = {q.W0, q.W1};
  const int cs[2] = {c0, c0};
  load_w<NW, OP_F32, 2, 1>(r.w, Ws, cs, kH);
}

#ifndef VRNN_PACE_EARLY
#define VRNN_PACE_EARLY 8
#endif
#ifndef VRNN_PACE_EPI
#define VRNN_PACE_EPI 4
#endif
typedef PaceK<VRNN_PACE_EARLY, VRNN_PACE_EPI> Paced;

template <int NW, int K, int FLAGS, class PC = PaceOff, bool ROW_ONCE = false, class WS>
__device__ __forceinline__ void visit_lin(const LinArgs& q, const Deal& d, int s, int tiles, int nt, Walk& wk, const WS& ws) {
  if (nt == 0 || s < d.s_begin || s >= d.s_end) return;
  constexpr bool sum3 = (FLAGS & DF_A_SUM3) != 0;
  wk.at(d, s, (FLAGS & DF_GENTLE) != 0);
  const float* A = q.a.at(s);
  const float* A2 = sum3 ? q.a2.at(s) : nullptr;
  const float* A3 = sum3 ? q.a3.at(s) : nullptr;
  auto late = [&]() {
    return LinLate{q.bias, q.add.at(s), q.gate.at(s), q.ld1, q.ld2, (FLAGS & DF_ADD_POLLED) != 0, (FLAGS & DF_RELU) != 0, q.slope,
                   Out{q.orm.at(s), q.ld3, (FLAGS & DF_RM_SC1) != 0, q.o16.at(s), q.n16, q.o16b.at(s), q.n16b}};
  };
  int seen_r0 = -1;
  for (int tk = 0; tk < (WS::resident ? 1 : nt); ++tk) {
    const int trc = __builtin_amdgcn_readlane(tiles, tk), tr0 = trc & 0xffff, tc0 = (trc >> 16) * 16;
    if constexpr ((FLAGS & DF_CANARY) != 0) {
      if (!ROW_ONCE || tr0 != seen_r0) canary_wait(A, tr0, K, wk.pl, q.ld0);
      seen_r0 = tr0;
    }
    ANAT(anat_arm(wk.pl);)
    tile_lin_late<NW, OP_F32>(A, q.ld0, true, q.W, K, late, tr0, tc0, wk.B, wk.red(), wk.pl, A2, A3, q.w_width, ws, PC());
    ANAT(anat_note(wk.anat, 4 * d.idx, wk.pl);)
  }
}

template <int NW, int N, int K0, int K, bool GATED, class P0 = PaceOff>
__device__ __forceinline__ void visit_run(const SeqArgs& q, const Deal& d, int s, int tiles, int nt, Walk& wk, const RunRes<N, K0, K>& rr) {
  if (nt == 0 || s < d.s_begin || s >= d.s_end) return;
  const int trc = __builtin_amdgcn_readlane(tiles, 0), tr0 = trc & 0xffff, tc0 = (trc >> 16) * 16;
  const float* A = q.a0.at(s);
#pragma unroll
  for (int li = 0; li < N; ++li) {
    wk.at(d, s, false, (unsigned)li);
    auto late = [&]() {
      const float* aux = q.aux[li].at(s);
      return LinLate{GATED ? nullptr : aux, li == 0 ? q.add0.at(s) : nullptr, GATED ? aux : nullptr, q.ldadd0, q.ldgate, false, !GATED, q.slope,
                     Out{q.orm[li].at(s), q.ld[li], false, q.o16[li].at(s), q.n16}};
    };
    ANAT(anat_arm(wk.pl);)
    if (li == 0) tile_lin_late<NW, OP_F32>(A, 0, true, q.W[li], K0, late, tr0, tc0, wk.B, wk.red(), wk.pl, nullptr, nullptr, 0, rr.first, P0());
    else tile_lin_late<NW, OP_F32>(A, 0, true, q.W[li], K, late, tr0, tc0, wk.B, wk.red(), wk.pl, nullptr, nullptr, 0, rr.rest[li > 0 ? li - 1 : 0], Paced());
    ANAT(anat_note(wk.anat, 4 * d.idx + li, wk.pl);)
    A = q.o16[li].at(s);
  }
}

template <int NW, class PC = PaceOff>
__device__ __forceinline__ void visit_head(const HeadArgs& q, const Deal& d, int s, int tiles, int nt, Walk& wk, const Res<kH, 4>& ws) {
  if (nt == 0 || s < d.s_begin || s >= d.s_end) return;
  wk.at(d, s, false);
  const HeadOut o{q.mu_p.at(s), q.sd_p.at(s), q.mu_q.at(s), q.sd_q.at(s), q.raw_p.at(s), q.raw_q.at(s), q.muq_raw.at(s),
                  Out{q.z.at(s), q.ld3, false, q.z16.at(s), q.n16, q.z16b.at(s), q.n16b}};
  const int trc = __builtin_amdgcn_readlane(tiles, 0);
  ANAT(anat_arm(wk.pl);)
// ... 161 lines not shown
    visit_lin<NW, kH, kDecFlags>(kargs<FwdArgs>().dec[2], kargs<FwdArgs>().deal[8], s, t8, n8, wk, w2);
    visit_lin<NW, kH, kDecFlags, PaceOff, true>(kargs<FwdArgs>().dec[3], kargs<FwdArgs>().deal[9], s, t9, n9, wk, WMem());
  }
}

template <int NW>
__global__ __launch_bounds__(NW * 64, 1) void vrnn_static_fwd_kernel(FwdArgs a) {
  extern __shared__ __attribute__((aligned(16))) float lds_red[];
  const int w = placed_wg(a.place), rt = (a.B + 15) / 16;
  const bool xcd = a.place == kPlaceProgram && a.xcd != 0;
  Walk wk{lds_red, lds_red + kFwdProducts * NW * 256, 0, a.B, Poll{a.ctl, 0u, false, 1}};
  ANAT(__shared__ unsigned anat[kAnatSlots * 8]; anat_begin(anat); wk.anat = anat;)
  if (a.ndec != 0 && w >= a.deal[6].wg0) {
    fwd_dec<NW>(a, w, rt, xcd, wk);
    return;
  }
  if (w >= a.deal[0].wg0) {
    const int t0 = tile_lanes(w, a.deal[0].wg0, a.deal[0].nwg, rt, a.deal[0].ct, xcd), n0 = tile_count(t0);
    if (n0 == 0) return;
    for (int s = a.s0; s < a.S; ++s) visit_lin<NW, kR, DF_RM_SC1 | DF_GENTLE | DF_CANARY>(kargs<FwdArgs>().hproj, kargs<FwdArgs>().deal[0], s, t0, n0, wk, WMem());
    return;
  }
  if (w < a.deal[2].wg0) fwd_half<NW, 0>(a, w, rt, xcd, wk);
  else if (a.arm.n != 0) fwd_post_arming<NW>(a, w, rt, xcd, wk);
  else fwd_half<NW, 1>(a, w, rt, xcd, wk);
}

struct BwdArgs {
  GrubArgs grub;
  LinArgs part[3], gb, sum;
  SeqArgs phi;
  DzArgs dz;
  SeqArgs run[2];
  Deal deal[10];
  int B, s0, S, xcd, place;
  Ctl ctl;
  ArmTable arm;
  ANAT(unsigned long long* prof;)
};

template <int NW, int HALF>
__device__ __forceinline__ void bwd_half(const BwdArgs& a, int w, int rt, bool xcd, Walk& wk) {
  const int t0 = tile_lanes(w, a.deal[0].wg0, a.deal[0].nwg, rt, a.deal[0].ct, xcd), n0 = tile_count(t0);
  const int t1 = tile_lanes(w, a.deal[1 + HALF].wg0, a.deal[1 + HALF].nwg, rt, a.deal[1 + HALF].ct, xcd), n1 = tile_count(t1);
  const int t5 = tile_lanes(w, a.deal[5].wg0, a.deal[5].nwg, rt, a.deal[5].ct, xcd), n5 = tile_count(t5);
  const int t6 = tile_lanes(w, a.deal[6].wg0, a.deal[6].nwg, rt, a.deal[6].ct, xcd), n6 = tile_count(t6);
  const int t7 = tile_lanes(w, a.deal[7].wg0, a.deal[7].nwg, rt, a.deal[7].ct, xcd), n7 = tile_count(t7);
  const int t8 = tile_lanes(w, a.deal[8 + HALF].wg0, a.deal[8 + HALF].nwg, rt, a.deal[8 + HALF].ct, xcd), n8 = tile_count(t8);
  Res<kH, 2> grub;
  Res<kR> part;
  Res<kH> sum, dz;
  RunRes<2, kH, kH> phi;
  RunRes<3, 2 * kH, kH> run;
  load_grub<NW>(grub, kargs<BwdArgs>().grub, t0, n0);
  load_lin<NW, kR>(part, kargs<BwdArgs>().part[HALF].W, kargs<BwdArgs>().part[HALF].w_width, t1, n1);
  load_lin<NW, kH>(sum, kargs<BwdArgs>().sum.W, kH, t5, n5);
  load_run<NW>(phi, kargs<BwdArgs>().phi, t6, n6);
  load_lin<NW, kH>(dz, kargs<BwdArgs>().dz.WT, kH, t7, n7);
  load_run<NW>(run, kargs<BwdArgs>().run[HALF], t8, n8);
  for (int s = a.s0; s < a.S; ++s) {
    visit_grub<NW, Paced>(kargs<BwdArgs>().grub, kargs<BwdArgs>().deal[0], s, t0, n0, wk, grub);
    visit_lin<NW, kR, 0, Paced>(kargs<BwdArgs>().part[HALF], kargs<BwdArgs>().deal[1 + HALF], s, t1, n1, wk, part);
    visit_lin<NW, kH, DF_A_SUM3, Paced>(kargs<BwdArgs>().sum, kargs<BwdArgs>().deal[5], s, t5, n5, wk, sum);
    visit_run<NW, 2, kH, kH, true, Paced>(kargs<BwdArgs>().phi, kargs<BwdArgs>().deal[6], s, t6, n6, wk, phi);
    visit_dz<NW, Paced>(kargs<BwdArgs>().dz, kargs<BwdArgs>().deal[7], s, t7, n7, wk, dz);
    if constexpr (HALF == 0) visit_run<NW, 3, 2 * kH, kH, true, Paced>(kargs<BwdArgs>().run[HALF], kargs<BwdArgs>().deal[8 + HALF], s, t8, n8, wk, run);
    else visit_run<NW, 3, 2 * kH, kH, true>(kargs<BwdArgs>().run[HALF], kargs<BwdArgs>().deal[8 + HALF], s, t8, n8, wk, run);
  }
  ANAT(anat_end(wk.anat, kargs<BwdArgs>().prof, 2 + HALF, w == kargs<BwdArgs>().deal[1 + HALF].wg0);)
}

template <int NW>
__global__ __launch_bounds__(NW * 64, 1) void vrnn_static_bwd_kernel(BwdArgs a) {
  extern __shared__ __attribute__((aligned(16))) float lds_red[];
  const int w = placed_wg(a.place), rt = (a.B + 15) / 16;
  const bool xcd = a.place == kPlaceProgram && a.xcd != 0;
  Walk wk{lds_red, lds_red + kBwdProducts * NW * 256, 0, a.B, Poll{a.ctl, 0u, false, 1}};
  ANAT(__shared__ unsigned anat[kAnatSlots * 8]; anat_begin(anat); wk.anat = anat;)
  if (w >= a.deal[3].wg0) {
    const int t = tile_lanes(w, a.deal[3].wg0, a.deal[3].nwg, rt, a.deal[3].ct, xcd), n = tile_count(t);
    if (n == 0) return;
    Res<kR> part;
    load_lin<NW, kR>(part, kargs<BwdArgs>().part[2].W, kargs<BwdArgs>().part[2].w_width, t, n);
    const Armer armer = arm_rank_dev(w, a.deal[3], a.deal[3].wg0, a.deal[3].nwg, rt, xcd, t, n, a.arm.n);
    for (int s = a.s0; s < a.S; ++s) {
      visit_lin<NW, kR, 0>(kargs<BwdArgs>().part[2], kargs<BwdArgs>().deal[3], s, t, n, wk, part);
      arm_ahead<NW>(kargs<BwdArgs>().arm, s + kArmAhead, rt, armer);
    }
    ANAT(anat_end(wk.anat, kargs<BwdArgs>().prof, 4, w == kargs<BwdArgs>().deal[3].wg0);)
    return;
  }
  if (w >= a.deal[4].wg0) {
    const int t = tile_lanes(w, a.deal[4].wg0, a.deal[4].nwg, rt, a.deal[4].ct, xcd), n = tile_count(t);
    if (n == 0) return;
    for (int s = a.s0; s < a.S; ++s)
      visit_lin<NW, 3 * kR, DF_ADD_POLLED | DF_RM_SC1 | DF_GENTLE | DF_CANARY>(kargs<BwdArgs>().gb, kargs<BwdArgs>().deal[4], s, t, n, wk, WMem());
    return;
  }
  if (w < a.deal[2].wg0) bwd_half<NW, 0>(a, w, rt, xcd, wk);
  else bwd_half<NW, 1>(a, w, rt, xcd, wk);
}

int static_place_fallback() { return (pchain_tune() & 32) ? kPlacePlain : kPlaceProgram; }
int static_place_wanted() { return (pchain_tune() & 64) ? kPlaceLocal : static_place_fallback(); }

bool int_strides(const Program& p) {
  for (long v : p.stride)
    if (v < -2147483647L || v > 2147483647L) return false;
  return true;
}
SPtr sptr(const Program& p, const Desc& d, int k) { return SPtr{const_cast<float*>(d.p[k]), (int)p.stride[d.sidx[k]]}; }

template <class Kern>
int static_go(Kern kernel, int slot, int grid, size_t lds, const char* what) {
  static std::mutex mu;
  static int attr_dev[3] = {-1, -1, -1}, occ[3] = {0, 0, 0};
  int dev = 0, cus = 0;
  BLVM_HIP(hipGetDevice(&dev));
  BLVM_HIP(hipDeviceGetAttribute(&cus, hipDeviceAttributeMultiprocessorCount, dev));
  {
    std::lock_guard<std::mutex> lock(mu);
    if (attr_dev[slot] != dev) {
      BLVM_HIP(hipFuncSetAttribute(reinterpret_cast<const void*>(kernel), hipFuncAttributeMaxDynamicSharedMemorySize, (int)lds));
      BLVM_HIP(hipOccupancyMaxActiveBlocksPerMultiprocessor(&occ[slot], kernel, 1024, lds));
      attr_dev[slot] = dev;
    }
    BLVM_REQUIRE((long)occ[slot] * cus >= grid, "%s: %d workgroups are not co-resident (%d per CU x %d CUs)", what, grid, occ[slot], cus);
  }
  return BLVM_OK;
// ... 119 lines not shown
    }
    if (!one_tile_each(p, kFwdDecResident, place_xcd(place, p))) return 1;
  }
  FwdArgs a{};
  a.hproj = lin_args(p, d[0]);
  a.run[0] = seq_args(p, d[1]); a.run[1] = seq_args(p, d[2]); a.phi = seq_args(p, d[4]);
  const Desc &h = d[3], &g = d[5];
  a.head = HeadArgs{sp(p, h, HEAD_P16), sp(p, h, HEAD_Q16), sp(p, h, HEAD_EPS), sp(p, h, HEAD_MU_P), sp(p, h, HEAD_SD_P), sp(p, h, HEAD_MU_Q),
                    sp(p, h, HEAD_SD_Q), sp(p, h, HEAD_RAW_P), sp(p, h, HEAD_RAW_Q), sp(p, h, HEAD_MUQ_RAW), sp(p, h, HEAD_Z), sp(p, h, HEAD_Z16),
                    sp(p, h, HEAD_Z16B), h.p[HEAD_WP], h.p[HEAD_BP], h.p[HEAD_WQ], h.p[HEAD_BQ], h.ld[LD_OUT], h.n16[N16_OUT], h.n16[N16_OUTB],
                    h.i[HEAD_I_Z], h.i[HEAD_I_RESIDUAL], h.f[HEAD_F_BETA], h.f[HEAD_F_INV_BETA], h.f[HEAD_F_SD_EPS]};
  a.gru = GruArgs{sp(p, g, GRU_X16), sp(p, g, GRU_XG), sp(p, g, GRU_GH), sp(p, g, GRU_HPREV), sp(p, g, GRU_HRM), sp(p, g, GRU_H16), sp(p, g, GRU_H16B),
                  sp(p, g, GRU_RG), sp(p, g, GRU_UG), sp(p, g, GRU_NG), g.p[GRU_WIH], g.p[GRU_BIH], g.ld[GRU_LD_HPREV], g.ld[LD_OUT], g.n16[N16_OUT],
                  g.n16[N16_OUTB], g.i[GRU_I_R]};
  a.ndec = dec ? p.ndesc - kFwdDesc : 0;
  for (int k = 0; k < a.ndec; ++k) a.dec[k] = lin_args(p, d[6 + k]);
  int grid = 0;
  for (int i = 0; i < p.ndesc; ++i) { a.deal[i] = deal_of(d[i], i); grid = std::max(grid, d[i].wg0 + d[i].nwg); }
  a.B = p.B; a.s0 = p.s_first; a.S = S; a.xcd = p.xcd; a.place = place; a.ctl = p.ctl;
  ANAT(a.prof = pchain_profile_buffer();)
  BLVM_TRY(arm_or_fill(p, plan, 5, {3, 4}, half, gentle - half, place_xcd(place, p), stream, &a.arm));
  BLVM_TRY(pre());
  const size_t lds = sizeof(float) * 2 * kFwdProducts * 16 * 256;
  BLVM_TRY(static_go(&vrnn_static_fwd_kernel<16>, 0, grid, lds, "vrnn_static_fwd"));
  hipLaunchKernelGGL(vrnn_static_fwd_kernel<16>, dim3(grid), dim3(1024), lds, stream, a);
  BLVM_CHECK_LAUNCH("vrnn_static_fwd");
  ++g_static_launches;
  if (a.arm.n != 0) ++g_armed_launches;
  return BLVM_OK;
}

int vrnn_static_bwd(const Program& p, hipStream_t stream, const ArmPlan& plan, const std::function<int()>& pre) {
  int place = kPlaceProgram;
  if (vrnn_static_check(p, 10, kBwdProducts, 8, 9, &place)) return 1;
  const Desc* d = p.d;
  const int S = p.S;
  for (int i = 0; i < 10; ++i)
    if (d[i].s_begin != 0 || d[i].s_end != (i == 0 ? S : S - 1)) return 1;
  if (!shaped(d[0], K_GRUB, 0, kH) || !shaped(d[1], K_LIN, 0, kR) || !shaped(d[2], K_LIN, 0, kR) || !shaped(d[3], K_LIN, 0, kR) ||
      !shaped(d[4], K_LIN, DF_ADD_POLLED | DF_RM_SC1 | DF_GENTLE | DF_CANARY, 3 * kR) || !shaped(d[5], K_LIN, DF_A_SUM3, kH) ||
      !shaped(d[6], K_LINSEQ, DF_SEQ_GATE, kH) || !shaped(d[7], K_DZ, 0, kH) || !shaped(d[8], K_LINSEQ, DF_SEQ_GATE, kH) ||
      !shaped(d[9], K_LINSEQ, DF_SEQ_GATE, kH))
    return 1;
  if (!run(d[6], 2, 0) || !run(d[8], 3, 2 * kH) || !run(d[9], 3, 2 * kH)) return 1;
  if (!one_tile_each(p, kBwdResident, place_xcd(place, p)) || d[7].p[DZ_D2_16] != nullptr) return 1;
  const int half = d[2].wg0, gentle = d[4].wg0, spare = d[3].wg0;
  if (!within(d[1], 0, half) || !within(d[8], 0, half) || !within(d[2], half, gentle) || !within(d[9], half, gentle) || !within(d[4], gentle, spare) ||
      d[3].nwg <= 0)
    return 1;
  for (int i : {0, 5, 6, 7})
    if (!within(d[i], 0, gentle)) return 1;
  BwdArgs a{};
  const Desc& g = d[0];
  a.grub = GrubArgs{sp(p, g, GRUB_D0_16), sp(p, g, GRUB_D1_16), sp(p, g, GRUB_G_IN), sp(p, g, GRUB_RG), sp(p, g, GRUB_UG), sp(p, g, GRUB_NG), sp(p, g, GRUB_GH),
                    sp(p, g, GRUB_HPREV), sp(p, g, GRUB_DD), sp(p, g, GRUB_DGI), sp(p, g, GRUB_DGI16), sp(p, g, GRUB_DGH), sp(p, g, GRUB_DGH16), sp(p, g, GRUB_GA),
                    sp(p, g, GRUB_G_ADD), g.p[GRUB_W0], g.p[GRUB_W1], g.p[GRUB_G_OUT], g.ld[GRUB_LD_H], g.ld[GRUB_LD_GADD], g.ld[LD_OUT], g.n16[N16_OUT],
                    g.i[GRUB_I_R], g.i[GRUB_I_GEMM_FROM], g.i[GRUB_I_GATES_TO], g.i[GRUB_I_GIN_FROM]};
  for (int k = 0; k < 3; ++k) a.part[k] = lin_args(p, d[1 + k]);
  a.gb = lin_args(p, d[4]); a.sum = lin_args(p, d[5]);
  a.phi = seq_args(p, d[6]); a.run[0] = seq_args(p, d[8]); a.run[1] = seq_args(p, d[9]);
  const Desc& z = d[7];
  a.dz = DzArgs{sp(p, z, DZ_D16), sp(p, z, DZ_ADD), sp(p, z, DZ_MU_Q), sp(p, z, DZ_SD_Q), sp(p, z, DZ_MU_P), sp(p, z, DZ_SD_P),
                sp(p, z, DZ_EPS), sp(p, z, DZ_RAW_Q), sp(p, z, DZ_RAW_P), sp(p, z, DZ_MUQ_RAW), sp(p, z, DZ_DQH), sp(p, z, DZ_DQH16), sp(p, z, DZ_DPH),
                sp(p, z, DZ_DPH16), z.p[DZ_WT], z.p[DZ_C_RAW], z.p[DZ_C_FN], reinterpret_cast<const int32_t*>(z.p[DZ_X_SL]), z.ld[DZ_LD_ADD],
                z.ld[LD_OUT], z.n16[N16_OUT], z.i[DZ_I_Z], z.i[DZ_I_RESIDUAL], z.i[DZ_I_STRIDE], z.i[DZ_I_T0], (int)z.f[DZ_F_GEMM_FROM], z.f[DZ_F_FN_FLOOR],
                z.f[DZ_F_BETA], z.f[DZ_F_SD_EPS]};
  int grid = 0;
  for (int i = 0; i < 10; ++i) { a.deal[i] = deal_of(d[i], i); grid = std::max(grid, d[i].wg0 + d[i].nwg); }
  a.B = p.B; a.s0 = p.s_first; a.S = S; a.xcd = p.xcd; a.place = place; a.ctl = p.ctl;
  ANAT(a.prof = pchain_profile_buffer();)
  BLVM_TRY(arm_or_fill(p, plan, 3, {}, spare, d[3].nwg, place_xcd(place, p), stream, &a.arm));
  BLVM_TRY(pre());
  const size_t lds = sizeof(float) * 2 * kBwdProducts * 16 * 256;
  BLVM_TRY(static_go(&vrnn_static_bwd_kernel<16>, 1, grid, lds, "vrnn_static_bwd"));
  hipLaunchKernelGGL(vrnn_static_bwd_kernel<16>, dim3(grid), dim3(1024), lds, stream, a);
  BLVM_CHECK_LAUNCH("vrnn_static_bwd");
  ++g_static_launches;
  if (a.arm.n != 0) ++g_armed_launches;
  return BLVM_OK;
}

}

int vrnn_launch(pchain::Builder& bld, bool forward, const char* who, hipStream_t stream, const pchain::ArmPlan& plan, const std::function<int()>& pre) {
  BLVM_TRY(pchain_prepare(bld, who));
  const int rc = forward ? vrnn_static_fwd(bld.p, stream, plan, pre) : vrnn_static_bwd(bld.p, stream, plan, pre);
  if (rc != 1) return rc;
  BLVM_TRY(full_fill(plan, stream));
  BLVM_TRY(pre());
  return pchain_run(bld.p, stream);
}

}

extern "C" int blvm_pchain_static(int mode) {
  if (mode == -2) return (int)std::min<long>(blvm::g_static_launches, 0x7fffffffL);
  if (mode == -3) return (int)std::min<long>(blvm::g_armed_launches, 0x7fffffffL);
  const int was = blvm::g_static;
  if (mode >= 0) blvm::g_static = mode != 0;
  return was;
}
// ... 35 lines not shown
```

include/blvm_hip.h:

```cpp
#ifndef BLVM_HIP_H
#define BLVM_HIP_H

#include <stddef.h>
#include <stdint.h>

#ifdef __cplusplus
extern "C" {
#endif

#define BLVM_OK 0
#define BLVM_EINVAL (-1)
#define BLVM_ELAUNCH (-2)
#define BLVM_ENOSUP (-3)
#define BLVM_NOT_APPLICABLE 1

int blvm_version(void);
const char* blvm_last_error(void);
int blvm_device_ok(void);
int blvm_async_errors(unsigned* last_code);
int blvm_async_errors_take(unsigned* last_code);
int blvm_pchain_configure(int max_batch, int waves);
int blvm_pchain_max_batch(void);
#define BLVM_DTYPE_F32 0
#define BLVM_DTYPE_BF16 1
// ... 129 lines not shown
} BlvmVrnnDecodeWeights;
size_t blvm_vrnn_decode_scratch_floats(int S, int H, int Z, int R);
int blvm_vrnn_decode(const BlvmVrnnDecodeWeights* w, const float* x0, const float* h0, const float* eps, const float* u,
                     const float* v, int T, int B, int S, int H, int Z, int R, int num_mix, float sd_eps, float slope,
                     float log_eps, float* x_out, float* h_out, float* scratch, void* stream);

size_t blvm_vrnn_generate_scratch_floats(int T, int B, int S, int H, int Z, int R);
int blvm_vrnn_generate(const BlvmVrnnDecodeWeights* w, const float* x0, const float* h0, const float* eps, const float* u,
                       const float* v, int T, int B, int S, int H, int Z, int R, int num_mix, float sd_eps, float slope,
                       float log_eps, float* x_out, float* h_out, float* scratch, void* stream);

size_t blvm_vrnn_reserve_floats(int Tp, int B, int X, int H, int Z, int R);
size_t blvm_vrnn_bwd_workspace_floats(int Tp, int B, int X, int H, int Z, int R);

int blvm_vrnn_seq_fwd(const BlvmVrnnWeights* w, const float* enc, const float* h0, const float* eps, int Tp, int B,
                      int X, int H, int Z, int R, int residual_posterior, float sd_eps, float* decin,
                      float* mu_q, float* sd_q, float* mu_p, float* sd_p, float* z, float* reserve, void* stream);

size_t blvm_vrnn_fwd_reserve_floats(int Tp, int B, int X, int H, int Z, int R, int DH, int SF);
int blvm_vrnn_seq_fwd_dec(const BlvmVrnnWeights* w, const float* enc, const float* h0, const float* eps, int Tp, int B,
                          int X, int H, int Z, int R, int residual_posterior, float sd_eps, float* decin,
                          float* mu_q, float* sd_q, float* mu_p, float* sd_p, float* z, float* reserve,
                          const float* const* dec_w, const float* const* dec_b, float* const* dec_y, int DH, int SF, float slope,
                          int* folded, void* stream);
int blvm_vrnn_dec_fold(int mode);

int blvm_vrnn_seq_bwd(const BlvmVrnnWeights* w, const float* enc, const float* eps, const float* decin,
                      const float* mu_q, const float* sd_q, const float* mu_p, const float* sd_p, const float* z,
                      const float* reserve, const float* d_decin, const int32_t* x_sl, const float* c_raw,
                      const float* c_fn, int stride, float fn_floor, int Tp, int B, int X, int H, int Z, int R,
                      int residual_posterior, float sd_eps, float* d_enc, float* d_h0, const BlvmVrnnGrads* grads,
                      float* workspace, void* stream);

size_t blvm_lstm_reserve_floats(int T, int B, int H);
size_t blvm_lstm_bwd_workspace_floats(int T, int B, int H);
int blvm_lstm_seq_fwd(const float* Wih, const float* Whh, const float* bih, const float* bhh, const float* in,
                      const float* h0, const float* c0, const int32_t* lens, int T, int B, int I, int H, float* out,
                      float* hn, float* cn, float* reserve, void* stream);
int blvm_lstm_seq_bwd(const float* Wih, const float* Whh, const float* in, const float* reserve, const float* d_out,
                      int T, int B, int I, int H, float* d_in, float* d_h0, float* d_c0, float* dWih, float* dWhh,
                      float* dbih, float* dbhh, float* workspace, void* stream);

size_t blvm_lstm_bidir_reserve_floats(int T, int B, int H);
size_t blvm_lstm_bidir_bwd_workspace_floats(int T, int B, int H);
int blvm_lstm_bidir_fwd(const float* Wih_f, const float* Whh_f, const float* bih_f, const float* bhh_f,
                        const float* Wih_r, const float* Whh_r, const float* bih_r, const float* bhh_r, const float* in,
                        const int32_t* lens, int T, int B, int I, int H, float* out, float* reserve, void* stream);
int blvm_lstm_bidir_bwd(const float* Wih_f, const float* Whh_f, const float* Wih_r, const float* Whh_r, const float* in,
                        const int32_t* lens, const float* reserve, const float* d_out, int T, int B, int I, int H,
                        float* d_in, float* dWih_f, float* dWhh_f, float* dbih_f, float* dbhh_f, float* dWih_r,
                        float* dWhh_r, float* dbih_r, float* dbhh_r, float* workspace, void* stream);
int blvm_lstm_bidir_applies(int T, int B, int H);
int blvm_lstm_bidir_path_counts(unsigned long long out[2]);

size_t blvm_gru_reserve_floats(int T, int B, int R);
size_t blvm_gru_bwd_workspace_floats(int T, int B, int R);
int blvm_gru_seq_fwd(const float* Wih, const float* Whh, const float* bih, const float* bhh, const float* in,
                     int ld_in, const float* h0, const int32_t* lens, int reverse, int T, int B, int I, int R,
                     float* out, long long out_ts, int out_ld, float* hn, float* reserve, void* stream);
int blvm_gru_seq_bwd(const float* Wih, const float* Whh, const float* in, int ld_in, const int32_t* lens, int reverse,
                     const float* reserve, const float* d_out, long long out_ts, int out_ld, int T, int B, int I,
                     int R, float* d_in, int ld_din, int accumulate_din, float* d_h0, float* dWih, float* dWhh,
                     float* dbih, float* dbhh, float* workspace, void* stream);

typedef struct BlvmSrnnWeights {
  const float *prior_w[3], *prior_b[3];
// ... 178 lines not shown
```

Measured before the change: 92.89 million.

## Fold decoder MLP backward into persistent VRNN backward kernel via spare leader workgroups

The forward VRNN sequence now also returns the final decoder activation, so the DMoL head consumes it directly. The backward pass then runs the decoder-MLP input-gradient GEMMs inside the persistent VRNN backward chain on spare workgroups (bwd_spare_leader), feeding a second polled add into the gate-gradient linear. This overlaps the decoder backward with the recurrent backward instead of running separate GEMMs first. Weight gradients are computed afterwards in a grouped wgrad call. A fallback path issues the GEMMs separately when the fold is unavailable. The change adds considerable complexity and new polling paths, which risks stalls or mismatched descriptors.

```diff
diff --git a/benchmarking-lvms_amd/blvm/models/vrnn.py b/benchmarking-lvms_amd/blvm/models/vrnn.py
--- a/benchmarking-lvms_amd/blvm/models/vrnn.py
+++ b/benchmarking-lvms_amd/blvm/models/vrnn.py
@@ -177,12 +177,13 @@
             eps = torch.randn(Tp, B, Z, device=dev, dtype=torch.float32)
         widths = [(lin.in_features, lin.out_features) for lin in dec_lin]
         chained = len(dec_lin) == 3 and widths[0] == (H + R, widths[1][0]) and widths[1][1] == widths[1][0] == widths[2][0]
-        fold = ops.DecoderFold(dec_lin, ops.LEAKY_SLOPE) if chained and all(lin.bias is not None for lin in dec_lin) else None
+        gates = isinstance(lik, DiscretizedLogisticMixtureDense) and lik.params is not None
+        fold = ops.DecoderFold(dec_lin, ops.LEAKY_SLOPE, gates) if chained and all(lin.bias is not None for lin in dec_lin) else None
         decin, kld, kld_fn, mu_q, sd_q, mu_p, sd_p, z = self.vrnn_cell.sequence(enc, h0, eps, x_sl_dev, stride, free_nats, decoder=fold)
-        given = fold.given if fold is not None else None
+        given, dec_node = (fold.given, fold.dec) if fold is not None else (None, None)
 
         dec, log_prob = mlp_log_prob(lik, decin[:Tp].view(Tp * B, H + R), dec_lin, ops.ACT_LEAKY, ops.LEAKY_SLOPE, y, x_sl_dev,
-                                     ops.LAYOUT_TIME_MAJOR, B, T, Tp, S, given=given)
+                                     ops.LAYOUT_TIME_MAJOR, B, T, Tp, S, given=given, dec_node=dec_node)
 
         n_frames = float(x_sl_host.sum())
         loss, elbo, sums4 = ops.elbo_assemble(log_prob, kld, kld_fn, beta, n_frames)
diff --git a/benchmarking-lvms_amd/blvm/modules/distributions.py b/benchmarking-lvms_amd/blvm/modules/distributions.py
--- a/benchmarking-lvms_amd/blvm/modules/distributions.py
+++ b/benchmarking-lvms_amd/blvm/modules/distributions.py
@@ -67,9 +67,9 @@
         W, b = (self.params.weight, self.params.bias) if fused_linear else (None, None)
         return ops.dmol_log_prob(dec, W, b, y, x_sl_dev, layout, B, T, Tp, S, self.num_mix, self.num_bins, self.log_epsilon)
 
-    def fused_mlp_log_prob(self, x2d, layers, act, slope, y, x_sl_dev, layout, B, T, Tp, S, given=None):
+    def fused_mlp_log_prob(self, x2d, layers, act, slope, y, x_sl_dev, layout, B, T, Tp, S, given=None, dec_node=None):
         return ops.mlp_dmol_log_prob(x2d, layers, self.params.weight, self.params.bias, y, x_sl_dev, layout, B, T, Tp, S, act, slope,
-                                     self.num_mix, self.num_bins, self.log_epsilon, given)
+                                     self.num_mix, self.num_bins, self.log_epsilon, given, dec_node)
 
     @staticmethod
     def _pack(params):
@@ -163,8 +163,10 @@
         return self.levels.to(k.device)[k.long()]
 
 
-def mlp_log_prob(lik, x2d, layers, act, slope, y, x_sl_dev, layout, B, T, Tp, S, given=None):
+def mlp_log_prob(lik, x2d, layers, act, slope, y, x_sl_dev, layout, B, T, Tp, S, given=None, dec_node=None):
     if isinstance(lik, DiscretizedLogisticMixtureDense):
-        return lik.fused_mlp_log_prob(x2d, layers, act, slope, y, x_sl_dev, layout, B, T, Tp, S, given)
+        return lik.fused_mlp_log_prob(x2d, layers, act, slope, y, x_sl_dev, layout, B, T, Tp, S, given, dec_node)
+    if dec_node is not None:
+        raise ops._hip.BlvmHipError("mlp_log_prob: only the fused DMoL head takes a decoder output with head gates")
     dec = ops.mlp(x2d, layers, act, slope) if given is None else ops.mlp_given(x2d, layers, given, act, slope)
     return dec.detach(), lik.fused_log_prob(dec, y, x_sl_dev, layout, B, T, Tp, S)
diff --git a/benchmarking-lvms_amd/blvm/ops.py b/benchmarking-lvms_amd/blvm/ops.py
--- a/benchmarking-lvms_amd/blvm/ops.py
+++ b/benchmarking-lvms_amd/blvm/ops.py
@@ -321,7 +321,11 @@
 
 
 def mlp_dmol_log_prob(x2d, layers, W, b, y, x_sl_dev, layout, B, T, Tp, S, act: int = ACT_LEAKY, slope: float = LEAKY_SLOPE,
-                      num_mix=10, num_bins=256, log_eps=-7.0, given=None):
+                      num_mix=10, num_bins=256, log_eps=-7.0, given=None, dec_node=None):
+    if dec_node is not None:
+        if act != ACT_LEAKY or W is None:
+            raise _hip.BlvmHipError("mlp_dmol_log_prob: a decoder output with head gates needs the leaky ReLU and the fused head Linear")
+        return dec_node.detach(), _DMoLFunction.apply(dec_node, W, b, y, x_sl_dev, layout, B, T, Tp, S, num_mix, num_bins, log_eps, slope)
     if act == ACT_NONE or W is None:
         dec = mlp(x2d, layers, act, slope) if given is None else mlp_given(x2d, layers, given, act, slope)
         return dec.detach(), dmol_log_prob(dec, W, b, y, x_sl_dev, layout, B, T, Tp, S, num_mix, num_bins, log_eps)
@@ -713,7 +717,7 @@
     def forward(ctx, enc, h0, eps, x_sl_dev, cfg, dec, *params):
         Tp, B, X, H, Z, R, residual, sd_eps, stride, fn_floor = cfg
         enc, eps = _f32c(enc), _f32c(eps)
-        params = tuple(_f32c(p) for p in params)
+        params, dparams = tuple(_f32c(p) for p in params[:28]), tuple(_f32c(p) for p in params[28:])
         dev = enc.device
         lib = load()
         f32 = dict(device=dev, dtype=torch.float32)
@@ -745,6 +749,7 @@
                 "blvm_vrnn_seq_fwd_dec",
             )
             dec.given = tuple(ys[: folded.value]) if folded.value else None
+        joint = dec is not None and len(dparams) == 6 and dec.given is not None and len(dec.given) == 3
         _tick("fwd_end")
         kld = torch.zeros(B, device=dev, dtype=torch.float64)
         kld_fn = torch.zeros(B, device=dev, dtype=torch.float64)
@@ -755,21 +760,74 @@
         )
         ctx.cfg = cfg
         ctx.has_h0 = h0 is not None
-        ctx.save_for_backward(enc, eps, x_sl_dev, decin, mu_q, sd_q, mu_p, sd_p, z, reserve, *params)
+        ctx.joint, ctx.n_dpar, ctx.dec_slope = joint, len(dparams), dec.slope if joint else 0.0
+        ctx.save_for_backward(enc, eps, x_sl_dev, decin, mu_q, sd_q, mu_p, sd_p, z, reserve, *params, *((*dparams, ys[0], ys[1]) if joint else ()))
         ctx.mark_non_differentiable(mu_q, sd_q, mu_p, sd_p, z)
         ctx.set_materialize_grads(False)
-        return decin, kld, kld_fn, mu_q, sd_q, mu_p, sd_p, z
-
-    @staticmethod
-    def backward(ctx, d_decin, g_kld, g_kld_fn, *_unused):
+        return decin, kld, kld_fn, mu_q, sd_q, mu_p, sd_p, z, (ys[2] if joint else None)
+
+    @staticmethod
+    def backward(ctx, d_decin, g_kld, g_kld_fn, *rest):
         Tp, B, X, H, Z, R, residual, sd_eps, stride, fn_floor = ctx.cfg
         enc, eps, x_sl_dev, decin, mu_q, sd_q, mu_p, sd_p, z, reserve, *params = ctx.saved_tensors
         dev = enc.device
         lib = load()
         f32 = dict(device=dev, dtype=torch.float32)
-        d_decin = _f32c(d_decin) if d_decin is not None else torch.zeros_like(decin)
         c_raw = _grad_f32(g_kld) if g_kld is not None else None
         c_fn = _grad_f32(g_kld_fn) if g_kld_fn is not None else None
+        d_dec = rest[5] if ctx.joint else None
+        dgrads = (None,) * ctx.n_dpar
+        if d_dec is not None:
+            params, (W1, b1, W2, b2, W3, b3, y1, y2) = params[:28], params[28:]
+            dz3, M, DH, SF, slope = _f32c(d_dec), Tp * B, W2.shape[0], W3.shape[0], ctx.dec_slope
+            dy2, dy1 = torch.empty(M, DH, **f32), torch.empty(M, DH, **f32)
+            grads = _zeros_like_many(params)
+            d_enc = torch.empty_like(enc)
+            d_h0 = torch.empty(B, R, **f32) if ctx.has_h0 else None
+            w, g = _pack_weights(params), _pack_weights(grads, _hip.VrnnGrads)
+            folded = ctypes.c_int(0)
+            if d_decin is None:
+                ws = torch.empty(lib.blvm_vrnn_bwd_dec_workspace_floats(Tp, B, X, H, Z, R, DH, SF), **f32)
+                dw = (ctypes.c_void_p * 3)(ptr(W1), ptr(W2), ptr(W3))
+                _tick("bwd_begin")
+                check(
+                    lib.blvm_vrnn_seq_bwd_dec(w, ptr(enc), ptr(eps), ptr(decin), ptr(mu_q), ptr(sd_q), ptr(mu_p), ptr(sd_p), ptr(z),
+                                              ptr(reserve), ptr(x_sl_dev), ptr(c_raw), ptr(c_fn), stride, fn_floor, Tp, B, X, H, Z, R,
+                                              int(residual), sd_eps, ptr(d_enc), ptr(d_h0), g, ptr(ws), ptr(dz3), ptr(y1), ptr(y2), dw,
+                                              ptr(dy2), ptr(dy1), DH, SF, slope, ctypes.byref(folded), stream_ptr()),
+                    "blvm_vrnn_seq_bwd_dec",
+                )
+            if not folded.value:
+                gemm(0, 1, M, DH, SF, dz3, SF, W3, DH, dy2, DH, slope=slope, gate=y2, ldg=DH)
+                gemm(0, 1, M, DH, DH, dy2, DH, W2, DH, dy1, DH, slope=slope, gate=y1, ldg=DH)
+                dx = torch.empty(M, H + R, **f32)
+                gemm(0, 1, M, H + R, DH, dy1, DH, W1, H + R, dx, H + R, slope=slope)
+                dd = torch.zeros_like(decin)
+                dd[:Tp] = dx.view(Tp, B, H + R)
+                if d_decin is not None:
+                    dd = dd + _f32c(d_decin)
+                ws = torch.empty(lib.blvm_vrnn_bwd_workspace_floats(Tp, B, X, H, Z, R), **f32)
+                _tick("bwd_begin")
+                check(
+                    lib.blvm_vrnn_seq_bwd(w, ptr(enc), ptr(eps), ptr(decin), ptr(mu_q), ptr(sd_q), ptr(mu_p), ptr(sd_p), ptr(z),
+                                          ptr(reserve), ptr(dd), ptr(x_sl_dev), ptr(c_raw), ptr(c_fn), stride, fn_floor, Tp, B,
+                                          X, H, Z, R, int(residual), sd_eps, ptr(d_enc), ptr(d_h0), g, ptr(ws), stream_ptr()),
+                    "blvm_vrnn_seq_bwd",
+                )
+            _tick("bwd_end")
+            dpar = (W1, b1, W2, b2, W3, b3)
+            want = [ctx.needs_input_grad[6 + 28 + i] for i in range(6)]
+            sizes = [(dpar[i].numel() + 3) // 4 * 4 if want[i] else 0 for i in range(6)]
+            flat = torch.zeros(sum(sizes), **f32)
+            views, off = [], 0
+            for i in range(6):
+                views.append(flat[off : off + dpar[i].numel()].view(dpar[i].shape) if want[i] else None)
+                off += sizes[i]
+            x2d = decin[:Tp].view(M, H + R)
+            wgrad_group([(dz3, y2, views[4], views[5]), (dy2, y1, views[2], views[3]), (dy1, x2d, views[0], views[1])], M)
+            return (d_enc, d_h0, None, None, None, None, *grads, *views)
+        params = params[:28]
+        d_decin = _f32c(d_decin) if d_decin is not None else torch.zeros_like(decin)
         grads = _zeros_like_many(params)
         d_enc = torch.empty_like(enc)
         d_h0 = torch.empty(B, R, **f32) if ctx.has_h0 else None
@@ -783,7 +841,7 @@
             "blvm_vrnn_seq_bwd",
         )
         _tick("bwd_end")
-        return (d_enc, d_h0, None, None, None, None, *grads)
+        return (d_enc, d_h0, None, None, None, None, *grads, *dgrads)
 
 
 def vrnn_sequence(enc, h0, eps, x_sl_dev, params: Sequence[torch.Tensor], X, H, Z, R, residual_posterior, stride,
@@ -792,15 +850,19 @@
     fn_floor = float(free_nats) / Z if free_nats else 0.0
     cfg = (Tp, B, X, H, Z, R, int(residual_posterior), float(sd_eps), int(stride), fn_floor)
     if decoder is None:
-        return _VRNNSeqFunction.apply(enc, h0, eps, x_sl_dev, cfg, None, *params)
-    decoder.given = None
-    return _VRNNSeqFunction.apply(enc, h0, eps, x_sl_dev, cfg, decoder, *params)
+        return _VRNNSeqFunction.apply(enc, h0, eps, x_sl_dev, cfg, None, *params)[:8]
+    decoder.given = decoder.dec = None
+    dparams = ()
+    if decoder.head_gates and load().blvm_vrnn_dec_bwd_fold(-1):
+        dparams = tuple(t for lin in decoder.layers for t in (lin.weight, lin.bias))
+    *out, decoder.dec = _VRNNSeqFunction.apply(enc, h0, eps, x_sl_dev, cfg, decoder, *params, *dparams)
+    return tuple(out)
 
 
 class DecoderFold:
 
-    def __init__(self, layers, slope: float = LEAKY_SLOPE):
-        self.layers, self.slope, self.given = list(layers), float(slope), None
+    def __init__(self, layers, slope: float = LEAKY_SLOPE, head_gates: bool = False):
+        self.layers, self.slope, self.given, self.head_gates, self.dec = list(layers), float(slope), None, bool(head_gates), None
 
 
 
diff --git a/benchmarking-lvms_amd/csrc/pchain.h b/benchmarking-lvms_amd/csrc/pchain.h
--- a/benchmarking-lvms_amd/csrc/pchain.h
+++ b/benchmarking-lvms_amd/csrc/pchain.h
@@ -456,6 +456,9 @@
   bool add_polled, relu;
   float slope;
   Out out;
+  bool add_early = false;
+  const float* add2 = nullptr;
+  int ldadd2 = 0;
 };
 template <int NW, int OT, class Late, class WS = WMem, class PC = PaceOff>
 __device__ __forceinline__ void tile_lin_late(const float* A, int lda, bool a_polled, const float* W, int K, Late& late, int r0, int c0, int B,
@@ -476,6 +479,7 @@
     if (L.bias) e_bias = L.bias[col];
     if (L.gate) e_gate = L.gate[(size_t)rowc * L.ldgate + col];
     if (L.add && !L.add_polled) e_add = L.add[(size_t)rowc * L.ldadd + col];
+    if (L.add && L.add_polled && L.add_early) e_add = ld_sc1(make_rsrc(L.add), 4u * ((unsigned)rowc * (unsigned)L.ldadd + (unsigned)col));
   };
   f32x4 acc[1] = {{0.f, 0.f, 0.f, 0.f}};
   if (A2 != nullptr) {
@@ -499,15 +503,24 @@
   }
 #endif
   if (threadIdx.x >= 256) return;
-  if (L.add && L.add_polled) {
+  if (L.add && L.add_polled && (!L.add_early || __any(own && is_sentinel(e_add)))) {
     const rsrc_t rs[1] = {make_rsrc(L.add)};
     const unsigned os[1] = {4u * ((unsigned)rowc * (unsigned)L.ldadd + (unsigned)col)};
     float ws[1];
     poll_words<1>(rs, os, ws, own, pl);
     e_add = ws[0];
   }
+  float e_add2 = 0.f;
+  if (L.add2) {
+    const rsrc_t rs[1] = {make_rsrc(L.add2)};
+    const unsigned os[1] = {4u * ((unsigned)rowc * (unsigned)L.ldadd2 + (unsigned)col)};
+    float ws[1];
+    poll_words<1>(rs, os, ws, own, pl);
+    e_add2 = ws[0];
+  }
   if (!own) return;
   float x = v[0] + e_bias + e_add;
+  if (L.add2) x += e_add2;
   if (L.relu) x = x > 0.f ? x : x * L.slope;
   if (L.gate) x = e_gate > 0.f ? x : x * L.slope;
   put(L.out, r0, c0, row, col, x);
@@ -1109,10 +1122,12 @@
   DF_CANARY = 32,
   DF_A_SUM3 = 64,
   DF_SEQ_GATE = 128,
+  DF_ADD_EARLY = 256,
+  DF_ADD2_POLLED = 512,
 };
 enum : int { LD_OUT = 3, N16_OUT = 0, N16_OUTB = 1 };
-enum : int { LIN_A, LIN_W, LIN_BIAS, LIN_ADD, LIN_GATE, LIN_ORM, LIN_O16, LIN_O16B, LIN_A2, LIN_A3, LIN_LD_A = 0, LIN_LD_ADD = 1, LIN_LD_GATE = 2,
-             LIN_I_W_WIDTH = 0, LIN_F_SLOPE = 0 };
+enum : int { LIN_A, LIN_W, LIN_BIAS, LIN_ADD, LIN_GATE, LIN_ORM, LIN_O16, LIN_O16B, LIN_A2, LIN_A3, LIN_ADD2, LIN_LD_A = 0, LIN_LD_ADD = 1, LIN_LD_GATE = 2,
+             LIN_I_W_WIDTH = 0, LIN_I_LD_ADD2 = 1, LIN_F_SLOPE = 0 };
 enum : int { LINSEQ_A0 = 0, LINSEQ_W = 1, LINSEQ_AUX = 5, LINSEQ_ORM = 9, LINSEQ_O16 = 13, LINSEQ_ADD0 = 17, LINSEQ_LD_ORM = 0,
              LINSEQ_I_LD_ADD0 = 0, LINSEQ_I_N = 1, LINSEQ_I_LD_GATE = 2, LINSEQ_I_K0 = 3, LINSEQ_F_SLOPE = 0 };
 enum : int { HEAD_P16, HEAD_Q16, HEAD_WP, HEAD_BP, HEAD_WQ, HEAD_BQ, HEAD_EPS, HEAD_MU_P, HEAD_SD_P, HEAD_MU_Q, HEAD_SD_Q, HEAD_RAW_P, HEAD_RAW_Q,
diff --git a/benchmarking-lvms_amd/csrc/pchain.hip b/benchmarking-lvms_amd/csrc/pchain.hip
--- a/benchmarking-lvms_amd/csrc/pchain.hip
+++ b/benchmarking-lvms_amd/csrc/pchain.hip
@@ -171,9 +171,15 @@
             auto late = [&]() {
               __builtin_amdgcn_sched_barrier(0);
               nx.fetch(ltab, nx_i, nx_s);
-              return LinLate{d.base<LIN_BIAS>(), d.p<LIN_ADD>(s), d.p<LIN_GATE>(s), d.w<RD_LD + LIN_LD_ADD>(), d.w<RD_LD + LIN_LD_GATE>(), (flags & DF_ADD_POLLED) != 0,
-                             (flags & DF_RELU) != 0, d.f<LIN_F_SLOPE>(), Out{d.m<LIN_ORM>(s), d.w<RD_LD + LD_OUT>(), (flags & DF_RM_SC1) != 0, d.m<LIN_O16>(s),
-                                                                             d.w<RD_N16 + N16_OUT>(), d.m<LIN_O16B>(s), d.w<RD_N16 + N16_OUTB>()}};
+              if constexpr (OT == OP_F32 && !ROLL)
+                return LinLate{d.base<LIN_BIAS>(), d.p<LIN_ADD>(s), d.p<LIN_GATE>(s), d.w<RD_LD + LIN_LD_ADD>(), d.w<RD_LD + LIN_LD_GATE>(), (flags & DF_ADD_POLLED) != 0,
+                               (flags & DF_RELU) != 0, d.f<LIN_F_SLOPE>(), Out{d.m<LIN_ORM>(s), d.w<RD_LD + LD_OUT>(), (flags & DF_RM_SC1) != 0, d.m<LIN_O16>(s),
+                                                                               d.w<RD_N16 + N16_OUT>(), d.m<LIN_O16B>(s), d.w<RD_N16 + N16_OUTB>()},
+                               (flags & DF_ADD_EARLY) != 0, (flags & DF_ADD2_POLLED) ? d.p<LIN_ADD2>(s) : nullptr, d.w<RD_I + LIN_I_LD_ADD2>()};
+              else
+                return LinLate{d.base<LIN_BIAS>(), d.p<LIN_ADD>(s), d.p<LIN_GATE>(s), d.w<RD_LD + LIN_LD_ADD>(), d.w<RD_LD + LIN_LD_GATE>(), (flags & DF_ADD_POLLED) != 0,
+                               (flags & DF_RELU) != 0, d.f<LIN_F_SLOPE>(), Out{d.m<LIN_ORM>(s), d.w<RD_LD + LD_OUT>(), (flags & DF_RM_SC1) != 0, d.m<LIN_O16>(s),
+                                                                               d.w<RD_N16 + N16_OUT>(), d.m<LIN_O16B>(s), d.w<RD_N16 + N16_OUTB>()}};
             };
             for (int tk = 0; tk < nt; ++tk) {
               const int trc = d.tile(tk), tr0 = trc & 0xffff, tc0 = (trc >> 16) * 16;
@@ -621,6 +627,8 @@
       BLVM_REQUIRE(k == pchain::K_LIN || k == pchain::K_LINSEQ || k == pchain::K_HEAD || k == pchain::K_GRU || k == pchain::K_DZ || k == pchain::K_GRUB,
                    "pchain: tile kind %d has no row-group form", k);
       BLVM_REQUIRE(k != pchain::K_DZ || prog.d[i].p[2] == nullptr, "pchain: the row-group dz tile is the single-product form");
+      BLVM_REQUIRE(k != pchain::K_LIN || (prog.d[i].flags & (pchain::DF_ADD_EARLY | pchain::DF_ADD2_POLLED)) == 0,
+                   "pchain: the row-group linear tile has one addend, polled behind its product");
     }
     BLVM_REQUIRE(prog.ot == OP_F32, "pchain: row groups multiply fp32 operands only");
     BLVM_TRY(go(&pchain_rt_kernel<8, OP_F32, 2>, 2, 512));
@@ -629,6 +637,9 @@
   }
   bool roll = false;
   for (int i = 0; i < prog.ndesc; ++i) roll |= prog.d[i].kind == pchain::K_LSTM;
+  for (int i = 0; i < prog.ndesc; ++i)
+    BLVM_REQUIRE(prog.d[i].kind != pchain::K_LIN || (prog.d[i].flags & (pchain::DF_ADD_EARLY | pchain::DF_ADD2_POLLED)) == 0 || (prog.ot == OP_F32 && !roll),
+                 "pchain: an early or a second polled addend runs in the fp32 training kernel only");
   if (roll) {
     for (int i = 0; i < prog.ndesc; ++i) {
       const int k = prog.d[i].kind;
diff --git a/benchmarking-lvms_amd/csrc/vrnn.hip b/benchmarking-lvms_amd/csrc/vrnn.hip
--- a/benchmarking-lvms_amd/csrc/vrnn.hip
+++ b/benchmarking-lvms_amd/csrc/vrnn.hip
@@ -179,9 +179,10 @@
   float *GA, *GB, *DP16[3], *DQ16[3], *DGI16, *DGH16, *DPHI16[4], *DPH16, *DQH16, *DPHI16b, *DPHI16c;
   size_t x16_bytes;
   float *DPHI3b, *DPHI3c;
+  float *DY216, *DY116, *DD, *dT[3];
 };
 
-size_t carve_ws(float* base, int Tp, int B, int X, int H, int Z, int R, BwdWs* w) {
+size_t carve_ws(float* base, int Tp, int B, int X, int H, int Z, int R, BwdWs* w, int SF = 0) {
   (void)X;
   const size_t n = (size_t)Tp * B;
   Arena ar{base};
@@ -209,8 +210,11 @@
     for (int i = 0; i < 4; ++i) t.DPHI16[i] = ar.take(m * H);
     t.DPH16 = ar.take(m * 2 * Z); t.DQH16 = ar.take(m * 2 * Z);
     t.DPHI16b = ar.take(m * H); t.DPHI16c = ar.take(m * H);
+    t.DY216 = t.DY116 = t.DD = nullptr;
+    if (SF > 0) { t.DY216 = ar.take(m * H); t.DY116 = ar.take(m * H); t.DD = ar.take(n * (H + R)); }
     t.x16_bytes = ar.bytes_from(t.GA);
     t.DPHI3b = ar.take(n * H); t.DPHI3c = ar.take(n * H);
+    if (SF > 0) { t.dT[0] = ar.take((size_t)(H + R) * H); t.dT[1] = ar.take((size_t)H * H); t.dT[2] = ar.take((size_t)H * SF); }
   }
   if (w) *w = t;
   return ar.floats();
@@ -248,6 +252,24 @@
   return fits ? layers : 0;
 }
 
+struct VrnnDecBwd {
+  const float *dz3, *y1, *y2, *w[3];
+  float *dy2, *dy1;
+  int DH, SF;
+  float slope;
+};
+int g_dec_bwd_fold = [] { const char* e = getenv("BLVM_VRNN_DEC_BWD_FOLD"); return e ? (atoi(e) != 0 ? 1 : 0) : 1; }();
+long g_dec_bwd_folded = 0;
+bool vrnn_dec_bwd_folds(int Tp, int B, int H, int Z, int R, int DH, int SF) {
+  if (!g_dec_bwd_fold || !vrnn_persistent(B) || device_cus() < 32 || operand_16bit() || pchain_optype(B) != OP_F32) return false;
+  if (B > 64 || vrnn_row_groups(B) || Z != H || DH != H || H != 256 || R != 512 || SF <= 0 || SF % 16 != 0) return false;
+  if (Tp + 1 <= pchain::kArmAhead || Tp <= pchain::kBdecAhead) return false;
+  const int tl = (B + 15) / 16;
+  if (vrnn_shared_deal(false, tl)) return false;
+  const pchain::VrnnBwdDeal dl = pchain::vrnn_bwd_deal(H / 16, Z / 16, R / 16, tl, device_cus() & ~7, false, pchain_split3(), (H + R) / 16);
+  return dl.split3 && dl.bdec[0].nwg > 0;
+}
+
 int check_dims(int Tp, int B, int X, int H, int Z, int R) {
   BLVM_REQUIRE(Tp > 0 && B > 0, "vrnn: bad Tp=%d B=%d", Tp, B);
   BLVM_REQUIRE(X > 0 && H > 0 && Z > 0 && R > 0 && X % 16 == 0 && H % 16 == 0 && Z % 16 == 0 && R % 16 == 0,
@@ -278,6 +300,15 @@
 
 extern "C" size_t blvm_vrnn_bwd_workspace_floats(int Tp, int B, int X, int H, int Z, int R) {
   return carve_ws(nullptr, Tp, B, X, H, Z, R, nullptr);
+}
+extern "C" size_t blvm_vrnn_bwd_dec_workspace_floats(int Tp, int B, int X, int H, int Z, int R, int DH, int SF) {
+  return carve_ws(nullptr, Tp, B, X, H, Z, R, nullptr, vrnn_dec_bwd_folds(Tp, B, H, Z, R, DH, SF) ? SF : 0);
+}
+extern "C" int blvm_vrnn_dec_bwd_fold(int mode) {
+  if (mode == -2) return (int)std::min<long>(g_dec_bwd_folded, 0x7fffffffL);
+  const int was = g_dec_bwd_fold;
+  if (mode >= 0) g_dec_bwd_fold = mode != 0;
+  return was;
 }
 
 static int vrnn_seq_fwd_impl(const BlvmVrnnWeights* w, const float* enc, const float* h0, const float* eps,
@@ -499,16 +530,16 @@
                              const float* z, const float* reserve, const float* d_decin, const int32_t* x_sl,
                              const float* c_raw, const float* c_fn, int stride, float fn_floor, int Tp, int B, int X, int H, int Z,
                              int R, int residual_posterior, float sd_eps, float* d_enc, float* d_h0,
-                             const BlvmVrnnGrads* gr, float* workspace, hipStream_t s) {
+                             const BlvmVrnnGrads* gr, float* workspace, hipStream_t s, const VrnnDecBwd* dec = nullptr) {
   BLVM_TRY(check_dims(Tp, B, X, H, Z, R));
-  BLVM_REQUIRE(w && enc && eps && decin && mu_q && sd_q && mu_p && sd_p && z && reserve && d_decin && workspace && gr,
+  BLVM_REQUIRE(w && enc && eps && decin && mu_q && sd_q && mu_p && sd_p && z && reserve && (d_decin || dec) && workspace && gr,
                "vrnn_bwd: null pointer");
   BLVM_REQUIRE((c_fn == nullptr && c_raw == nullptr) || x_sl != nullptr, "vrnn_bwd: KL coefficients need x_sl");
   BLVM_REQUIRE(aligned16(workspace) && aligned16(reserve) && aligned16(d_decin), "vrnn_bwd: buffers must be 16-byte aligned");
   Reserve rs;
   carve_reserve(const_cast<float*>(reserve), Tp, B, H, Z, R, &rs);
   BwdWs ws;
-  carve_ws(workspace, Tp, B, X, H, Z, R, &ws);
+  carve_ws(workspace, Tp, B, X, H, Z, R, &ws, dec ? dec->SF : 0);
   const size_t n = (size_t)Tp * B;
   const int ldd = H + R;
   const float beta = softplus_beta_of(sd_eps);
@@ -526,6 +557,11 @@
   for (int i = 1; i < 4; ++i) BLVM_TRY(t16_pack_transposed(w->phi_w[i], H, H, H, ws.fT[i], s));
   BLVM_TRY(t16_pack_transposed(w->gru_wih + X, X + H, 3 * R, H, ws.wihT, s));
   BLVM_TRY(t16_pack_transposed(w->gru_whh, R, 3 * R, R, ws.whhT, s));
+  if (dec) {
+    BLVM_TRY(t16_pack_transposed(dec->w[0], H + R, H, H + R, ws.dT[0], s));
+    BLVM_TRY(t16_pack_transposed(dec->w[1], H, H, H, ws.dT[1], s));
+    BLVM_TRY(t16_pack_transposed(dec->w[2], H, dec->SF, H, ws.dT[2], s));
+  }
   BLVM_TRY(pack_scope.flush());
 
   BLVM_HIP(hipMemsetAsync(ws.G, 0, sizeof(float) * (size_t)B * R, s));
@@ -589,7 +625,8 @@
     const int RTG = groups ? vrnn_rt(B) : 1;
     const int tl = (rt + RTG - 1) / RTG;
     const bool shared = vrnn_shared_deal(groups, tl);
-    const VrnnBwdDeal dl = vrnn_bwd_deal(ctH, ctZ, ctR, tl, cus, shared, pchain_split3());
+    const VrnnBwdDeal dl = vrnn_bwd_deal(ctH, ctZ, ctR, tl, cus, shared, pchain_split3(), dec ? (H + R) / 16 : 0);
+    BLVM_REQUIRE(!dec || (dl.split3 && dl.bdec[0].nwg > 0 && !groups), "vrnn_bwd: the deal has no decoder leader range");
     Builder bld;
     bld.begin(pchain_optype(B), T + 1, B, groups ? 8 : 2, true, dl.g);
     bld.p.rt_group = RTG;
@@ -598,7 +635,7 @@
       Operands o;
       o.p[GRUB_D0_16] = rev(ws.DP16[0], xH, T); o.p[GRUB_D1_16] = rev(ws.DQ16[0], xH, T); o.p[GRUB_W0] = ws.pT[0]; o.p[GRUB_W1] = ws.qT[0];
       o.p[GRUB_G_IN] = rev(ws.GB, sR, T); o.p[GRUB_RG] = last(rs.RG, sR); o.p[GRUB_UG] = last(rs.UG, sR); o.p[GRUB_NG] = last(rs.NG, sR);
-      o.p[GRUB_GH] = last(rs.GHb, s3R); o.p[GRUB_HPREV] = last(decin + H, sD); o.p[GRUB_DD] = last(d_decin + H, sD); o.p[GRUB_DGI] = last(ws.DGI, s3R);
+      o.p[GRUB_GH] = last(rs.GHb, s3R); o.p[GRUB_HPREV] = last(decin + H, sD); o.p[GRUB_DD] = dec ? Ptr() : last(d_decin + H, sD); o.p[GRUB_DGI] = last(ws.DGI, s3R);
       o.p[GRUB_DGI16] = last(ws.DGI16, x3R); o.p[GRUB_DGH] = last(ws.DGH, s3R); o.p[GRUB_DGH16] = last(ws.DGH16, x3R); o.p[GRUB_GA] = last(ws.GA, sR);
       o.p[GRUB_G_OUT] = d_h0 ? d_h0 : ws.G; o.ld[GRUB_LD_H] = ldd; o.ld[LD_OUT] = 3 * R; o.n16[N16_OUT] = 3 * ctR; o.i[GRUB_I_R] = R; o.i[GRUB_I_GEMM_FROM] = 1;
       o.i[GRUB_I_GATES_TO] = T; o.i[GRUB_I_GIN_FROM] = 1;
@@ -613,9 +650,10 @@
       float* const o16[3] = {ws.DPHI16[3], ws.DPHI16b, ws.DPHI16c};
       o.ld[LIN_LD_A] = 3 * R; o.i[LIN_I_W_WIDTH] = 3 * R;
       for (int part = 0; part < 3; ++part) {
-        o.p[LIN_A] = last(ws.DGI16 + (size_t)part * ctR * 256, x3R); o.p[LIN_W] = ws.wihT + part * wthird; o.p[LIN_ADD] = part == 0 ? last(d_decin, sD) : Ptr();
+        o.p[LIN_A] = last(ws.DGI16 + (size_t)part * ctR * 256, x3R); o.p[LIN_W] = ws.wihT + part * wthird;
+        o.p[LIN_ADD] = dec ? (part == 2 ? last(ws.DD, sD) : Ptr()) : (part == 0 ? last(d_decin, sD) : Ptr());
         o.p[LIN_ORM] = last(orm[part], sH); o.p[LIN_O16] = last(o16[part], xH);
-        add_desc(bld, K_LIN, ctH, dl.part[part].wg0, dl.part[part].nwg, R, 0, 0, T, o);
+        add_desc(bld, K_LIN, ctH, dl.part[part].wg0, dl.part[part].nwg, R, dec && part == 2 ? DF_ADD_POLLED | DF_ADD_EARLY : 0, 0, T, o);
       }
     } else {
       o.p[LIN_A] = last(ws.DGI16, x3R); o.p[LIN_W] = ws.wihT; o.p[LIN_ADD] = last(d_decin, sD); o.p[LIN_ORM] = last(ws.DPHI[3], sH);
@@ -624,7 +662,9 @@
     }
     Operands gb;
     gb.p[LIN_A] = last(ws.DGH16, x3R); gb.p[LIN_W] = ws.whhT; gb.p[LIN_ADD] = last(ws.GA, sR); gb.ld[LIN_LD_ADD] = R; gb.p[LIN_ORM] = last(ws.GB, sR); gb.ld[LD_OUT] = R;
-    add_desc(bld, K_LIN, ctR, dl.gb.wg0, dl.gb.nwg, 3 * R, DF_ADD_POLLED | DF_RM_SC1 | DF_GENTLE | ((pchain_tune() & 16) ? DF_CANARY : 0), 0, T, gb);
+    if (dec) { gb.p[LIN_ADD2] = last(ws.DD + H, sD); gb.i[LIN_I_LD_ADD2] = ldd; }
+    add_desc(bld, K_LIN, ctR, dl.gb.wg0, dl.gb.nwg, 3 * R,
+             DF_ADD_POLLED | DF_RM_SC1 | DF_GENTLE | ((pchain_tune() & 16) ? DF_CANARY : 0) | (dec ? DF_ADD2_POLLED : 0), 0, T, gb);
     auto blink = [&](const float* W, const float* gate, float* orm, float* o16) { return rev_link(W, gate, orm, o16, T - 1, sH, H, xH); };
     const SeqLink lf[3] = {blink(ws.fT[3], rs.FZ[2], ws.DPHI[2], ws.DPHI16[2]), blink(ws.fT[2], rs.FZ[1], ws.DPHI[1], ws.DPHI16[1]),
                            blink(ws.fT[1], rs.FZ[0], ws.DPHI[0], ws.DPHI16[0])};
@@ -650,6 +690,20 @@
       const SeqLink lq[3] = {blink(ws.qhT, rs.Q[2], ws.DQ[2], ws.DQ16[2]), blink(ws.qT[2], rs.Q[1], ws.DQ[1], ws.DQ16[1]), blink(ws.qT[1], rs.Q[0], ws.DQ[0], ws.DQ16[0])};
       add_linseq(bld, ctH, dl.prior.wg0, dl.prior.nwg, H, false, true, 0, T, last(ws.DPH16, x2Z), 3, lp, -sH, -xH, ctH, 0.f, H, 2 * Z);
       add_linseq(bld, ctH, dl.post.wg0, dl.post.nwg, H, false, true, 0, T, last(ws.DQH16, x2Z), 3, lq, -sH, -xH, ctH, 0.f, H, 2 * Z);
+    }
+    if (dec) {
+      const int L = kBdecAhead, SF = dec->SF;
+      const long sF = (long)B * SF;
+      auto lead = [&](const float* base, long step) { return rev(base, step, T - 1 - L); };
+      Operands b0, b1, b2;
+      b0.p[LIN_A] = lead(dec->dz3, sF); b0.ld[LIN_LD_A] = SF; b0.p[LIN_W] = ws.dT[2]; b0.p[LIN_GATE] = lead(dec->y2, sH); b0.ld[LIN_LD_GATE] = H;
+      b0.p[LIN_ORM] = lead(dec->dy2, sH); b0.ld[LD_OUT] = H; b0.p[LIN_O16] = lead(ws.DY216, xH); b0.n16[N16_OUT] = ctH; b0.f[LIN_F_SLOPE] = dec->slope;
+      add_desc(bld, K_LIN, ctH, dl.bdec[0].wg0, dl.bdec[0].nwg, SF, DF_A_PLAIN | DF_GENTLE, 0, T - L, b0);
+      b1.p[LIN_A] = lead(ws.DY216, xH); b1.p[LIN_W] = ws.dT[1]; b1.p[LIN_GATE] = lead(dec->y1, sH); b1.ld[LIN_LD_GATE] = H;
+      b1.p[LIN_ORM] = lead(dec->dy1, sH); b1.ld[LD_OUT] = H; b1.p[LIN_O16] = lead(ws.DY116, xH); b1.n16[N16_OUT] = ctH; b1.f[LIN_F_SLOPE] = dec->slope;
+      add_desc(bld, K_LIN, ctH, dl.bdec[1].wg0, dl.bdec[1].nwg, H, DF_GENTLE | DF_CANARY, 0, T - L, b1);
+      b2.p[LIN_A] = lead(ws.DY116, xH); b2.p[LIN_W] = ws.dT[0]; b2.p[LIN_ORM] = lead(ws.DD, sD); b2.ld[LD_OUT] = ldd;
+      add_desc(bld, K_LIN, (H + R) / 16, dl.bdec[2].wg0, dl.bdec[2].nwg, H, DF_RM_SC1 | DF_GENTLE | DF_CANARY, 0, T - L, b2);
     }
     ArmPlan plan;
     plan.fill(ws.GA, ws.x16_bytes);
@@ -660,8 +714,18 @@
       for (int i = 0; i < 4; ++i) plan.add(arm_t16(ws.DPHI16[i], H, rt, T, true));
       plan.add(arm_t16(ws.DPH16, 2 * Z, rt, T, true)); plan.add(arm_t16(ws.DQH16, 2 * Z, rt, T, true));
       plan.add(arm_t16(ws.DPHI16b, H, rt, T, true)); plan.add(arm_t16(ws.DPHI16c, H, rt, T, true));
-    }
-    BLVM_TRY(vrnn_launch(bld, false, "vrnn_bwd", s, plan, []() -> int { return BLVM_OK; }));
+      if (dec) { plan.add(arm_t16(ws.DY216, H, rt, T, true)); plan.add(arm_t16(ws.DY116, H, rt, T, true)); plan.add(arm_rm(ws.DD, ldd, B, T, true)); }
+    }
+    auto lead_rows = [&]() -> int {
+      if (!dec) return BLVM_OK;
+      const int L = kBdecAhead, M = L * B, SF = dec->SF;
+      const size_t r0 = (size_t)(T - L) * B;
+      BLVM_TRY(gemm_f32(0, 1, M, H, SF, dec->dz3 + r0 * SF, SF, dec->w[2], H, dec->dy2 + r0 * H, H, nullptr, 0, dec->slope, dec->y2 + r0 * H, H, 0, 1, s));
+      BLVM_TRY(gemm_f32(0, 1, M, H, H, dec->dy2 + r0 * H, H, dec->w[1], H, dec->dy1 + r0 * H, H, nullptr, 0, dec->slope, dec->y1 + r0 * H, H, 0, 1, s));
+      return gemm_f32(0, 1, M, H + R, H, dec->dy1 + r0 * H, H, dec->w[0], H + R, ws.DD + r0 * ldd, ldd, nullptr, 0, 0.f, nullptr, 0, 0, 1, s);
+    };
+    BLVM_TRY(vrnn_launch(bld, false, "vrnn_bwd", s, plan, lead_rows));
+    if (dec) ++g_dec_bwd_folded;
     if (split3) {
       const size_t n4 = n * H / 4;
       hipLaunchKernelGGL(add3_kernel, dim3((unsigned)std::min<size_t>((n4 + 255) / 256, 2048)), dim3(256), 0, s, reinterpret_cast<float4*>(ws.DPHI[3]),
@@ -670,6 +734,7 @@
     return batched();
   }
 
+  BLVM_REQUIRE(!dec, "vrnn_bwd: the decoder leader needs the persistent path");
   launch_dh(-1, Tp - 1);
   for (int t = Tp - 1; t >= 0; --t) {
     const size_t oH = (size_t)t * B * H, oZ = (size_t)t * B * Z, o3R = (size_t)t * B * 3 * R, o2Z = (size_t)t * B * 2 * Z;
@@ -721,3 +786,23 @@
   return vrnn_seq_bwd_impl(w, enc, eps, decin, mu_q, sd_q, mu_p, sd_p, z, reserve, d_decin, x_sl, c_raw, c_fn, stride, fn_floor, Tp, B, X,
                            H, Z, R, residual_posterior, sd_eps, d_enc, d_h0, gr, workspace, static_cast<hipStream_t>(stream_));
 }
+
+extern "C" int blvm_vrnn_seq_bwd_dec(const BlvmVrnnWeights* w, const float* enc, const float* eps, const float* decin,
+                                     const float* mu_q, const float* sd_q, const float* mu_p, const float* sd_p, const float* z,
+                                     const float* reserve, const int32_t* x_sl, const float* c_raw, const float* c_fn, int stride,
+                                     float fn_floor, int Tp, int B, int X, int H, int Z, int R, int residual_posterior, float sd_eps,
+                                     float* d_enc, float* d_h0, const BlvmVrnnGrads* gr, float* workspace, const float* dz3,
+                                     const float* dec_y1, const float* dec_y2, const float* const* dec_w, float* dy2, float* dy1, int DH,
+                                     int SF, float slope, int* folded, void* stream_) {
+  BLVM_REQUIRE(folded != nullptr, "vrnn_bwd_dec: null pointer");
+  *folded = 0;
+  BLVM_TRY(check_dims(Tp, B, X, H, Z, R));
+  if (!vrnn_dec_bwd_folds(Tp, B, H, Z, R, DH, SF)) return BLVM_OK;
+  BLVM_REQUIRE(dz3 && dec_y1 && dec_y2 && dec_w && dec_w[0] && dec_w[1] && dec_w[2] && dy2 && dy1, "vrnn_bwd_dec: null pointer");
+  BLVM_REQUIRE(aligned16(dz3) && aligned16(dy2) && aligned16(dy1), "vrnn_bwd_dec: buffers must be 16-byte aligned");
+  const VrnnDecBwd dec{dz3, dec_y1, dec_y2, {dec_w[0], dec_w[1], dec_w[2]}, dy2, dy1, DH, SF, slope};
+  BLVM_TRY(vrnn_seq_bwd_impl(w, enc, eps, decin, mu_q, sd_q, mu_p, sd_p, z, reserve, nullptr, x_sl, c_raw, c_fn, stride, fn_floor, Tp, B, X,
+                             H, Z, R, residual_posterior, sd_eps, d_enc, d_h0, gr, workspace, static_cast<hipStream_t>(stream_), &dec));
+  *folded = 1;
+  return BLVM_OK;
+}
diff --git a/benchmarking-lvms_amd/csrc/vrnn_static.h b/benchmarking-lvms_amd/csrc/vrnn_static.h
--- a/benchmarking-lvms_amd/csrc/vrnn_static.h
+++ b/benchmarking-lvms_amd/csrc/vrnn_static.h
@@ -41,12 +41,13 @@
   }
   return d;
 }
+constexpr int kBdecAhead = 2;
 struct VrnnBwdDeal {
   int def_n, half, g, spare;
   bool split3;
-  LinkRange grub, part[3], dphi, gb, wide_h, dz, prior, post;
-};
-inline VrnnBwdDeal vrnn_bwd_deal(int ctH, int ctZ, int ctR, int tl, int cus, bool shared, bool allow_split3) {
+  LinkRange grub, part[3], dphi, gb, wide_h, dz, prior, post, bdec[3];
+};
+inline VrnnBwdDeal vrnn_bwd_deal(int ctH, int ctZ, int ctR, int tl, int cus, bool shared, bool allow_split3, int ctD = 0) {
   VrnnBwdDeal d;
   d.def_n = shared ? 0 : range_for(ctR * tl, std::min(cus / 4, 64));
   d.half = range_for(ctH * tl, (cus - d.def_n) / 2);
@@ -64,6 +65,17 @@
   d.dz = LinkRange{ctZ, 0, range_for(ctZ * tl, wide)};
   d.prior = LinkRange{ctH, 0, d.half};
   d.post = LinkRange{ctH, d.half, d.half};
+  for (LinkRange& r : d.bdec) r = LinkRange{0, 0, 0};
+  if (ctD > 0 && d.split3) {
+    const int w0 = d.part[2].wg0, n = d.part[2].nwg;
+    bool fits = n == ctH * tl;
+    for (bool xcd : {false, true})
+      fits = fits && tiles_per_workgroup(tl, ctH, n, xcd) <= 1 && tiles_per_workgroup(tl, ctD, n, xcd) <= kMaxTiles;
+    if (fits) {
+      d.bdec[0] = d.bdec[1] = LinkRange{ctH, w0, n};
+      d.bdec[2] = LinkRange{ctD, w0, n};
+    }
+  }
   return d;
 }
 
@@ -71,6 +83,8 @@
 constexpr std::initializer_list<int> kBwdResident = {0, 1, 2, 3, 5, 6, 7, 8, 9};
 constexpr int kFwdDesc = 6, kFwdDecDesc = 10;
 constexpr std::initializer_list<int> kFwdDecResident = {6, 7, 8};
+constexpr int kBwdDesc = 10, kBwdDecDesc = 13;
+constexpr std::initializer_list<int> kBwdDecResident = {11};
 inline bool one_tile_each(const Program& p, std::initializer_list<int> links, bool xcd) {
   for (int i : links)
     if (tiles_per_workgroup((p.B + 15) / 16, p.d[i].ct, p.d[i].nwg, xcd) > 1) return false;
@@ -176,6 +190,12 @@
     const Desc& d = p.d[i];
     const int slot = arm_operand_slot(d.kind);
     if (slot < 0 || d.p[slot] == nullptr || p.stride[d.sidx[slot]] == 0) return false;
+    if (d.kind == K_LIN && (d.flags & DF_A_PLAIN) != 0) {
+      const Desc& role = p.d[link];
+      for (int w = d.wg0; w < d.wg0 + d.nwg; ++w)
+        if (TileIter(w, d.wg0, d.nwg, rt, d.ct, xcd).valid() && !TileIter(w, role.wg0, role.nwg, rt, role.ct, xcd).valid()) return false;
+      continue;
+    }
     bool inside = false;
     for (int k = 0; k < t.n && !inside; ++k) {
       const ArmEntry& e = t.e[k];
diff --git a/benchmarking-lvms_amd/csrc/vrnn_static.hip b/benchmarking-lvms_amd/csrc/vrnn_static.hip
--- a/benchmarking-lvms_amd/csrc/vrnn_static.hip
+++ b/benchmarking-lvms_amd/csrc/vrnn_static.hip
@@ -24,7 +24,7 @@
 }
 __device__ __forceinline__ int tile_count(int lanes) { return __popcll(__ballot(lanes >= 0)); }
 
-constexpr int kAnatBase = 128, kAnatRole = 512, kAnatSlots = 48;
+constexpr int kAnatBase = 128, kAnatRole = 512, kAnatSlots = 56;
 #ifdef PCHAIN_TPROF
 __device__ __forceinline__ void anat_begin(unsigned* tab) {
   for (int i = threadIdx.x; i < kAnatSlots * 8; i += blockDim.x) tab[i] = 0u;
@@ -212,27 +212,31 @@
 #endif
 typedef PaceK<VRNN_PACE_EARLY, VRNN_PACE_EPI> Paced;
 
-template <int NW, int K, int FLAGS, class PC = PaceOff, bool ROW_ONCE = false, class WS>
-__device__ __forceinline__ void visit_lin(const LinArgs& q, const Deal& d, int s, int tiles, int nt, Walk& wk, const WS& ws) {
+template <int NW, int KT, int FLAGS, class PC = PaceOff, bool ROW_ONCE = false, class WS>
+__device__ __forceinline__ void visit_lin(const LinArgs& q, const Deal& d, int s, int tiles, int nt, Walk& wk, const WS& ws, int kdyn = 0,
+                                          const SPtr& add2 = SPtr{nullptr, 0}, int ldadd2 = 0) {
   if (nt == 0 || s < d.s_begin || s >= d.s_end) return;
-  constexpr bool sum3 = (FLAGS & DF_A_SUM3) != 0;
+  static_assert(KT != 0 || !WS::resident, "resident weights hold a K fixed at compile time");
+  const int K = KT != 0 ? KT : kdyn;
+  constexpr bool sum3 = (FLAGS & DF_A_SUM3) != 0, a_polled = (FLAGS & DF_A_PLAIN) == 0;
   wk.at(d, s, (FLAGS & DF_GENTLE) != 0);
   const float* A = q.a.at(s);
   const float* A2 = sum3 ? q.a2.at(s) : nullptr;
   const float* A3 = sum3 ? q.a3.at(s) : nullptr;
   auto late = [&]() {
     return LinLate{q.bias, q.add.at(s), q.gate.at(s), q.ld1, q.ld2, (FLAGS & DF_ADD_POLLED) != 0, (FLAGS & DF_RELU) != 0, q.slope,
-                   Out{q.orm.at(s), q.ld3, (FLAGS & DF_RM_SC1) != 0, q.o16.at(s), q.n16, q.o16b.at(s), q.n16b}};
+                   Out{q.orm.at(s), q.ld3, (FLAGS & DF_RM_SC1) != 0, q.o16.at(s), q.n16, q.o16b.at(s), q.n16b},
+                   (FLAGS & DF_ADD_EARLY) != 0, (FLAGS & DF_ADD2_POLLED) != 0 ? add2.at(s) : nullptr, ldadd2};
   };
   int seen_r0 = -1;
   for (int tk = 0; tk < (WS::resident ? 1 : nt); ++tk) {
     const int trc = __builtin_amdgcn_readlane(tiles, tk), tr0 = trc & 0xffff, tc0 = (trc >> 16) * 16;
-    if constexpr ((FLAGS & DF_CANARY) != 0) {
+    if constexpr ((FLAGS & DF_CANARY) != 0 && a_polled) {
       if (!ROW_ONCE || tr0 != seen_r0) canary_wait(A, tr0, K, wk.pl, q.ld0);
       seen_r0 = tr0;
     }
     ANAT(anat_arm(wk.pl);)
-    tile_lin_late<NW, OP_F32>(A, q.ld0, true, q.W, K, late, tr0, tc0, wk.B, wk.red(), wk.pl, A2, A3, q.w_width, ws, PC());
+    tile_lin_late<NW, OP_F32>(A, q.ld0, a_polled, q.W, K, late, tr0, tc0, wk.B, wk.red(), wk.pl, A2, A3, q.w_width, ws, PC());
     ANAT(anat_note(wk.anat, 4 * d.idx, wk.pl);)
   }
 }
@@ -460,12 +464,18 @@
   SeqArgs phi;
   DzArgs dz;
   SeqArgs run[2];
-  Deal deal[10];
+  LinArgs bdec[3];
+  Deal deal[kBwdDecDesc];
+  int nbdec;
+  int bdec_k, gb_ldadd2;
+  SPtr gb_add2;
   int B, s0, S, xcd, place;
   Ctl ctl;
   ArmTable arm;
   ANAT(unsigned long long* prof;)
 };
+
+static_assert(sizeof(BwdArgs) <= 4096 && sizeof(FwdArgs) <= 4096, "kernel argument size");
 
 template <int NW, int HALF>
 __device__ __forceinline__ void bwd_half(const BwdArgs& a, int w, int rt, bool xcd, Walk& wk) {
@@ -498,6 +508,46 @@
   ANAT(anat_end(wk.anat, kargs<BwdArgs>().prof, 2 + HALF, w == kargs<BwdArgs>().deal[1 + HALF].wg0);)
 }
 
+constexpr int kGbFlags = DF_ADD_POLLED | DF_RM_SC1 | DF_GENTLE | DF_CANARY;
+constexpr int kPartLeadFlags = DF_ADD_POLLED | DF_ADD_EARLY;
+constexpr int kBdec0Flags = DF_A_PLAIN | DF_GENTLE, kBdec1Flags = DF_GENTLE | DF_CANARY, kBdec2Flags = DF_RM_SC1 | DF_GENTLE | DF_CANARY;
+template <int NW>
+__device__ __forceinline__ void bwd_spare_leader(const BwdArgs& a, int w, int rt, bool xcd, Walk& wk) {
+  const int t = tile_lanes(w, a.deal[3].wg0, a.deal[3].nwg, rt, a.deal[3].ct, xcd), n = tile_count(t);
+  const int t10 = tile_lanes(w, a.deal[10].wg0, a.deal[10].nwg, rt, a.deal[10].ct, xcd), n10 = tile_count(t10);
+  const int t11 = tile_lanes(w, a.deal[11].wg0, a.deal[11].nwg, rt, a.deal[11].ct, xcd), n11 = tile_count(t11);
+  const int t12 = tile_lanes(w, a.deal[12].wg0, a.deal[12].nwg, rt, a.deal[12].ct, xcd), n12 = tile_count(t12);
+  if ((n | n10 | n11 | n12) == 0) return;
+  Res<kR> part;
+  Res<kH> w2;
+  load_lin<NW, kR>(part, kargs<BwdArgs>().part[2].W, kargs<BwdArgs>().part[2].w_width, t, n);
+  load_lin<NW, kH>(w2, kargs<BwdArgs>().bdec[1].W, kH, t11, n11);
+  const Armer armer = arm_rank_dev(w, a.deal[3], a.deal[3].wg0, a.deal[3].nwg, rt, xcd, t, n, a.arm.n);
+#ifdef PCHAIN_TPROF
+  unsigned long long lead = 0, arming = 0;
+  const unsigned long long tb = wall_clock64();
+#endif
+  for (int s = a.s0; s < a.S; ++s) {
+    visit_lin<NW, kR, kPartLeadFlags>(kargs<BwdArgs>().part[2], kargs<BwdArgs>().deal[3], s, t, n, wk, part);
+    ANAT(const unsigned long long t0 = wall_clock64();)
+    visit_lin<NW, 0, kBdec0Flags>(kargs<BwdArgs>().bdec[0], kargs<BwdArgs>().deal[10], s, t10, n10, wk, WMem(), kargs<BwdArgs>().bdec_k);
+    visit_lin<NW, kH, kBdec1Flags>(kargs<BwdArgs>().bdec[1], kargs<BwdArgs>().deal[11], s, t11, n11, wk, w2);
+    visit_lin<NW, kH, kBdec2Flags, PaceOff, true>(kargs<BwdArgs>().bdec[2], kargs<BwdArgs>().deal[12], s, t12, n12, wk, WMem());
+    ANAT(const unsigned long long t1 = wall_clock64();)
+    arm_ahead<NW>(kargs<BwdArgs>().arm, s + kArmAhead, rt, armer);
+    ANAT(const unsigned long long t2 = wall_clock64(); lead += t1 - t0; arming += t2 - t1;)
+  }
+#ifdef PCHAIN_TPROF
+  const unsigned long long whole = wall_clock64() - tb;
+  if (threadIdx.x == 0) {
+    unsigned* q = wk.anat + 13 * 2 * 4;
+    q[0] = (unsigned)(a.S - a.s0); q[2] = (unsigned)lead; q[3] = (unsigned)arming;
+    q[8] = 1u; q[10] = (unsigned)whole;
+  }
+  anat_end(wk.anat, kargs<BwdArgs>().prof, 4, w == kargs<BwdArgs>().deal[3].wg0);
+#endif
+}
+
 template <int NW>
 __global__ __launch_bounds__(NW * 64, 1) void vrnn_static_bwd_kernel(BwdArgs a) {
   extern __shared__ __attribute__((aligned(16))) float lds_red[];
@@ -505,6 +555,10 @@
   const bool xcd = a.place == kPlaceProgram && a.xcd != 0;
   Walk wk{lds_red, lds_red + kBwdProducts * NW * 256, 0, a.B, Poll{a.ctl, 0u, false, 1}};
   ANAT(__shared__ unsigned anat[kAnatSlots * 8]; anat_begin(anat); wk.anat = anat;)
+  if (a.nbdec != 0 && w >= a.deal[3].wg0) {
+    bwd_spare_leader<NW>(a, w, rt, xcd, wk);
+    return;
+  }
   if (w >= a.deal[3].wg0) {
     const int t = tile_lanes(w, a.deal[3].wg0, a.deal[3].nwg, rt, a.deal[3].ct, xcd), n = tile_count(t);
     if (n == 0) return;
@@ -521,8 +575,14 @@
   if (w >= a.deal[4].wg0) {
     const int t = tile_lanes(w, a.deal[4].wg0, a.deal[4].nwg, rt, a.deal[4].ct, xcd), n = tile_count(t);
     if (n == 0) return;
+    if (a.nbdec != 0) {
+      for (int s = a.s0; s < a.S; ++s)
+        visit_lin<NW, 3 * kR, kGbFlags | DF_ADD2_POLLED>(kargs<BwdArgs>().gb, kargs<BwdArgs>().deal[4], s, t, n, wk, WMem(), 0, kargs<BwdArgs>().gb_add2,
+                                                         kargs<BwdArgs>().gb_ldadd2);
+      return;
+    }
     for (int s = a.s0; s < a.S; ++s)
-      visit_lin<NW, 3 * kR, DF_ADD_POLLED | DF_RM_SC1 | DF_GENTLE | DF_CANARY>(kargs<BwdArgs>().gb, kargs<BwdArgs>().deal[4], s, t, n, wk, WMem());
+      visit_lin<NW, 3 * kR, kGbFlags>(kargs<BwdArgs>().gb, kargs<BwdArgs>().deal[4], s, t, n, wk, WMem());
     return;
   }
   if (w < a.deal[2].wg0) bwd_half<NW, 0>(a, w, rt, xcd, wk);
@@ -708,13 +768,14 @@
 
 int vrnn_static_bwd(const Program& p, hipStream_t stream, const ArmPlan& plan, const std::function<int()>& pre) {
   int place = kPlaceProgram;
-  if (vrnn_static_check(p, 10, kBwdProducts, 8, 9, &place)) return 1;
+  const bool lead = p.ndesc == kBwdDecDesc;
+  if (vrnn_static_check(p, lead ? kBwdDecDesc : kBwdDesc, kBwdProducts, 8, 9, &place)) return 1;
   const Desc* d = p.d;
   const int S = p.S;
-  for (int i = 0; i < 10; ++i)
+  for (int i = 0; i < kBwdDesc; ++i)
     if (d[i].s_begin != 0 || d[i].s_end != (i == 0 ? S : S - 1)) return 1;
-  if (!shaped(d[0], K_GRUB, 0, kH) || !shaped(d[1], K_LIN, 0, kR) || !shaped(d[2], K_LIN, 0, kR) || !shaped(d[3], K_LIN, 0, kR) ||
-      !shaped(d[4], K_LIN, DF_ADD_POLLED | DF_RM_SC1 | DF_GENTLE | DF_CANARY, 3 * kR) || !shaped(d[5], K_LIN, DF_A_SUM3, kH) ||
+  if (!shaped(d[0], K_GRUB, 0, kH) || !shaped(d[1], K_LIN, 0, kR) || !shaped(d[2], K_LIN, 0, kR) || !shaped(d[3], K_LIN, lead ? kPartLeadFlags : 0, kR) ||
+      !shaped(d[4], K_LIN, lead ? kGbFlags | DF_ADD2_POLLED : kGbFlags, 3 * kR) || !shaped(d[5], K_LIN, DF_A_SUM3, kH) ||
       !shaped(d[6], K_LINSEQ, DF_SEQ_GATE, kH) || !shaped(d[7], K_DZ, 0, kH) || !shaped(d[8], K_LINSEQ, DF_SEQ_GATE, kH) ||
       !shaped(d[9], K_LINSEQ, DF_SEQ_GATE, kH))
     return 1;
@@ -726,6 +787,16 @@
     return 1;
   for (int i : {0, 5, 6, 7})
     if (!within(d[i], 0, gentle)) return 1;
+  if (lead) {
+    for (int i = kBwdDesc; i < kBwdDecDesc; ++i) {
+      if (d[i].s_begin != 0 || d[i].s_end != S - 1 - kBdecAhead || d[i].wg0 != spare || d[i].nwg != d[3].nwg) return 1;
+      if (d[i].p[LIN_A2] || d[i].p[LIN_A3] || d[i].p[LIN_O16B] || d[i].p[LIN_ADD] || d[i].p[LIN_ADD2] || d[i].p[LIN_BIAS] || d[i].i[LIN_I_W_WIDTH] != 0) return 1;
+    }
+    if (d[10].kind != K_LIN || d[10].flags != kBdec0Flags || d[10].K <= 0 || d[10].K % 16 != 0 || d[10].ld[LIN_LD_A] != d[10].K) return 1;
+    if (!shaped(d[11], K_LIN, kBdec1Flags, kH) || !shaped(d[12], K_LIN, kBdec2Flags, kH) || d[11].ld[LIN_LD_A] != 0 || d[12].ld[LIN_LD_A] != 0) return 1;
+    if (!one_tile_each(p, kBwdDecResident, place_xcd(place, p))) return 1;
+    if (d[3].p[LIN_ADD] == nullptr || d[4].p[LIN_ADD2] == nullptr || d[1].p[LIN_ADD] != nullptr || d[0].p[GRUB_DD] != nullptr) return 1;
+  }
   BwdArgs a{};
   const Desc& g = d[0];
   a.grub = GrubArgs{sp(p, g, GRUB_D0_16), sp(p, g, GRUB_D1_16), sp(p, g, GRUB_G_IN), sp(p, g, GRUB_RG), sp(p, g, GRUB_UG), sp(p, g, GRUB_NG), sp(p, g, GRUB_GH),
@@ -741,8 +812,11 @@
                 sp(p, z, DZ_DPH16), z.p[DZ_WT], z.p[DZ_C_RAW], z.p[DZ_C_FN], reinterpret_cast<const int32_t*>(z.p[DZ_X_SL]), z.ld[DZ_LD_ADD],
                 z.ld[LD_OUT], z.n16[N16_OUT], z.i[DZ_I_Z], z.i[DZ_I_RESIDUAL], z.i[DZ_I_STRIDE], z.i[DZ_I_T0], (int)z.f[DZ_F_GEMM_FROM], z.f[DZ_F_FN_FLOOR],
                 z.f[DZ_F_BETA], z.f[DZ_F_SD_EPS]};
+  a.nbdec = lead ? 3 : 0;
+  if (lead) { a.bdec_k = d[kBwdDesc].K; a.gb_add2 = sp(p, d[4], LIN_ADD2); a.gb_ldadd2 = d[4].i[LIN_I_LD_ADD2]; }
+  for (int k = 0; k < a.nbdec; ++k) a.bdec[k] = lin_args(p, d[kBwdDesc + k]);
   int grid = 0;
-  for (int i = 0; i < 10; ++i) { a.deal[i] = deal_of(d[i], i); grid = std::max(grid, d[i].wg0 + d[i].nwg); }
+  for (int i = 0; i < p.ndesc; ++i) { a.deal[i] = deal_of(d[i], i); grid = std::max(grid, d[i].wg0 + d[i].nwg); }
   a.B = p.B; a.s0 = p.s_first; a.S = S; a.xcd = p.xcd; a.place = place; a.ctl = p.ctl;
   ANAT(a.prof = pchain_profile_buffer();)
   BLVM_TRY(arm_or_fill(p, plan, 3, {}, spare, d[3].nwg, place_xcd(place, p), stream, &a.arm));
diff --git a/include/blvm_hip.h b/include/blvm_hip.h
--- a/include/blvm_hip.h
+++ b/include/blvm_hip.h
@@ -185,6 +185,16 @@
                       int residual_posterior, float sd_eps, float* d_enc, float* d_h0, const BlvmVrnnGrads* grads,
                       float* workspace, void* stream);
 
+size_t blvm_vrnn_bwd_dec_workspace_floats(int Tp, int B, int X, int H, int Z, int R, int DH, int SF);
+int blvm_vrnn_seq_bwd_dec(const BlvmVrnnWeights* w, const float* enc, const float* eps, const float* decin,
+                          const float* mu_q, const float* sd_q, const float* mu_p, const float* sd_p, const float* z,
+                          const float* reserve, const int32_t* x_sl, const float* c_raw, const float* c_fn, int stride,
+                          float fn_floor, int Tp, int B, int X, int H, int Z, int R, int residual_posterior, float sd_eps,
+                          float* d_enc, float* d_h0, const BlvmVrnnGrads* grads, float* workspace, const float* dz3,
+                          const float* dec_y1, const float* dec_y2, const float* const* dec_w, float* dy2, float* dy1, int DH,
+                          int SF, float slope, int* folded, void* stream);
+int blvm_vrnn_dec_bwd_fold(int mode);
+
 size_t blvm_lstm_reserve_floats(int T, int B, int H);
 size_t blvm_lstm_bwd_workspace_floats(int T, int B, int H);
 int blvm_lstm_seq_fwd(const float* Wih, const float* Whh, const float* bih, const float* bhh, const float* in,
```

New measurement: 95.11 million (median of 6 runs). 1.02x the previous value.
